# aniketntnu/WordDiffusion

Hardware: AMD Instinct MI355X
Metric: denoised 64x256 word images/sec (1000-step DDPM), whole job (higher is better)
Workload: dtype bf16x3; 1 GPU; BASELINE configs[1]: batch 64 per GPU of 64x256 crops = [64,4,8,32] latents, 1000-step DDPM (999 executed steps), base unet.py UNetModel (320 ch, mult (1,1), 4 heads, 339 writers), random-init synthetic weights; variant=base, batch_per_gpu=64, noise_steps=1000, executed_steps_per_image=999, precision=split-bf16 MFMA x3, fp32 accumulate (<=1e-4 of the fp32 reference), output_finite=True

## Files before the change

### include/wdiff_hip.h

```cpp
#ifndef WDIFF_HIP_H
#define WDIFF_HIP_H

#include <stdint.h>

#ifdef __cplusplus
extern "C" {
#endif

#define WD_OK 0
#define WD_EINVAL (-1)
#define WD_ELAUNCH (-2)
#define WD_ESTATE (-3)

#define WD_ACT_NONE 0
#define WD_ACT_SILU 1
#define WD_ACT_GEGLU 2

typedef uint16_t wd_bf16;

#define WD_MAX_KSPLIT 64

typedef struct wd_src {
    const wd_bf16* hi;
    const wd_bf16* lo;
    const int32_t* gather;
    int32_t ld;
    int32_t c;
    int32_t ntaps;
    int32_t hw_src;
} wd_src;

typedef struct wd_gemm_args {
    wd_src src[2];
    int32_t nsrc;
    int32_t npass;
    const wd_bf16* w_hi;
    const wd_bf16* w_lo;
    int32_t m, n, ktot;
    int32_t hw_out;
    const float* bias;
    const float* rowvec;
    int32_t rowvec_ld;
    const float* resid;
    int32_t resid_ld;
    const int64_t* resid_rows;
    int32_t act;
    float* out_f32;
    int32_t out_ld;
    wd_bf16* out_hi;
    wd_bf16* out_lo;
    int32_t out_pl_ld;
    int32_t tile;
    int32_t w_layout;
    int32_t slab_rows;
    int32_t ksplit;
    float* ws;
    int64_t ws_floats;
    double* stat_part;
    int32_t stat_cpg;
    int32_t dbg;
    int32_t* tickets;
    int32_t ntickets;
    const float* gn_gamma;
    const float* gn_beta;
    float gn_eps;
    int32_t gn_silu;
    int32_t gn_cpg;
    const float* a32;
    int32_t a32_ld;
    const double* a32_part;
    int32_t a32_nchunk;
    int32_t a32_pcpg;
    int32_t a32_cpg;
    const float* a32_gamma;
    const float* a32_beta;
    float a32_eps;
    int32_t a32_silu;
    const float* ln_gamma;
    const float* ln_beta;
    float ln_eps;
    int32_t w_ngroups;
    int64_t w_group_stride;
} wd_gemm_args;

int wd_gemm(const wd_gemm_args* args, void* stream);

int wd_gemm_check(const wd_gemm_args* args, wd_gemm_args* out);
const char* wd_gemm_check_kernel(const wd_gemm_args* args);

int wd_gemm_pack_w(const wd_bf16* hi, const wd_bf16* lo, int n, int ktot, wd_bf16* out_hi, wd_bf16* out_lo, void* stream);

typedef struct wd_ff_args {
    const wd_bf16* x_hi;
    const wd_bf16* x_lo;
    int32_t x_ld;
    int32_t m, c, inner;
    const wd_bf16* w1_hi;
    const wd_bf16* w1_lo;
    const float* b1;
    const wd_bf16* w2_hi;
    const wd_bf16* w2_lo;
    const float* b2;
    const float* resid;
    int32_t resid_ld;
    float* out_f32;
    int32_t out_ld;
    wd_bf16* out_hi;
    wd_bf16* out_lo;
    int32_t out_pl_ld;
    const wd_bf16* w3_hi;
    const wd_bf16* w3_lo;
    const float* b3;
    const float* resid3;
    int32_t resid3_ld;
    double* stat_part;
    int32_t stat_cpg;
    int32_t hw_out;
    int32_t npass;
    const float* x_in;
    int32_t x_in_ld;
    int32_t hw;
    const double* gn_part;
    int32_t gn_nchunk, gn_pcpg, gn_cpg;
    float gn_eps;
    const float* gn_gamma;
    const float* gn_beta;
    const wd_bf16* pi_hi;
    const wd_bf16* pi_lo;
    const float* pi_b;
    const float* ln2_gamma;
    const float* ln2_beta;
    const wd_bf16* mq_a;
    const wd_bf16* mot_a;
    const float* xb_a;
    const wd_bf16* mq_b;
    const wd_bf16* mot_b;
    const float* xb_b;
    const float* ln3_gamma;
    const float* ln3_beta;
    float ln_eps;
    int32_t heads, L;
    float* tok2;
} wd_ff_args;
int wd_ff_fused(const wd_ff_args* args, void* stream);
int wd_ff_supported(int c, int inner);
int wd_ff_args_bytes(void);

int wd_gemm_auto_ksplit(int m, int n, int ktot, int64_t ws_floats);
int wd_gemm_args_bytes(void);
int wd_gemm_experimental(void);

int wd_gn_nchunk(int hw);
int wd_gn_stats(const float* x, int ld, int batch, int hw, int c, int cpg, double* part, void* stream);
int wd_gn_fold_chunks(const double* part, int batch, int nchunk, int ngroups, double* out, void* stream);

int wd_gn_apply(const float* x, int ld, int batch, int hw, int c, int cpg, const double* part, int nchunk, int part_cpg,
                const float* gamma, const float* beta, float eps, int silu,
                wd_bf16* out_hi, wd_bf16* out_lo, int out_ld, int c_off,
                wd_bf16* raw_hi, wd_bf16* raw_lo, void* stream);

int wd_gn_apply2(const float* xa, int lda, int ca, const double* part_a, int nchunk_a, int part_cpg_a, int c_off_a,
                 const float* xb, int ldb, int cb, const double* part_b, int nchunk_b, int part_cpg_b, int c_off_b,
                 int batch, int hw, int cpg, const float* gamma, const float* beta, float eps, int silu,
                 wd_bf16* out_hi, wd_bf16* out_lo, int out_ld, wd_bf16* raw_hi, wd_bf16* raw_lo, const int32_t* perm_a, void* stream);

int wd_gn_conv3x3_few_supported(int c, int w, int oc);
int wd_gn_conv3x3_few(const float* x, int ld, int batch, int h, int w, int c, int cpg, const double* part, int nchunk, int part_cpg,
                      const float* gamma, const float* beta, float eps, int silu, const float* weight, const float* bias, int oc,
                      float* out, void* stream);

int wd_layernorm(const float* x, int ld, int rows, int c, const float* gamma, const float* beta, float eps,
                 wd_bf16* out_hi, wd_bf16* out_lo, int out_ld, void* stream);

int wd_split(const float* x, int ld, int rows, int c, int silu, wd_bf16* out_hi, wd_bf16* out_lo, int out_ld,
             void* stream);

int wd_attention(const float* q, int ldq, const float* k, int ldk, const float* v, int ldv,
                 int batch, int heads, int nq, int nk, int d, float scale,
                 float* out_f32, wd_bf16* out_hi, wd_bf16* out_lo, int out_ld, int out_rows, int out_row0,
                 void* stream);

int64_t wd_attention_packed_elems(int batch, int heads, int nk, int d);
int wd_attention_pack_kv(const float* k, int ldk, const float* v, int ldv, int batch, int heads, int nk, int d,
                         wd_bf16* img, void* stream);
int wd_attention_packed(const float* q, int ldq, const wd_bf16* img, int batch, int heads, int nq, int nk, int d,
                        float scale, float* out_f32, wd_bf16* out_hi, wd_bf16* out_lo, int out_ld, int out_rows,
                        int out_row0, void* stream);

int wd_timestep_embedding(const int64_t* t, int batch, const float* freqs, int half,
                          wd_bf16* out_hi, wd_bf16* out_lo, int out_ld, void* stream);

int wd_xattn_supported(int c, int heads, int L);
int wd_xattn_fold(const float* k, int ldk, const float* v, int ldv, int batch, int heads, int L, int d, float scale,
                  const float* wq, const float* wo, int c, float* mq, float* mo, wd_bf16* mq_pl, wd_bf16* mot_pl, void* stream);
int wd_xattn_fused(const float* x, int ld, int batch, int hw, int c, const float* gamma, const float* beta, float eps,
                   const float* mq, const float* mo, int heads, int L, const float* bias, float* out, int out_ld,
                   const float* gamma2, const float* beta2, float eps2, wd_bf16* n_hi, wd_bf16* n_lo, int n_ld,
                   const wd_bf16* mq_pl, const wd_bf16* mot_pl, void* stream);

int wd_emb_combine(const float* time, const float* label, const int64_t* y, int num_classes, int T, int B, int ted,
                   wd_bf16* out_hi, wd_bf16* out_lo, int out_ld, void* stream);
int wd_select_rows(const float* table, const int32_t* t_dev, int batch, int64_t row_floats, int chunk, float* out,
                   void* stream);

int wd_emb_combine_mix(const float* time, const float* label, const int32_t* pairs, const float* mix, int num_classes, int T, int B,
                       int ted, wd_bf16* out_hi, wd_bf16* out_lo, int out_ld, void* stream);
int wd_label_mix(const float* label, const int32_t* pairs, const float* mix, int num_classes, int B, int ted, float* out,
                 void* stream);

int wd_xattn_pair(const float* x, int ld, int batch, int hw, int c, float eps, int heads, int L, const float* gamma_a,
                  const float* beta_a, const wd_bf16* mq_pl_a, const wd_bf16* mot_pl_a, const float* bias_a, const float* gamma_b,
                  const float* beta_b, const wd_bf16* mq_pl_b, const wd_bf16* mot_pl_b, const float* bias_b, float* out, int out_ld,
                  const float* gamma2, const float* beta2, float eps2, wd_bf16* n_hi, wd_bf16* n_lo, int n_ld, void* stream);

int wd_embed_tokens(const void* ids, int ids_are_i64, int rows, int seq_len, const float* table, int vocab, int c,
                    const float* pe, wd_bf16* out_hi, wd_bf16* out_lo, int out_ld, void* stream);

int wd_im2col3x3(const float* x, int batch, int cin, int h, int w, wd_bf16* out_hi, wd_bf16* out_lo, int kpad,
                 void* stream);

int wd_conv3x3_in_supported(int cin, int h, int w, int cout);
int wd_conv3x3_in_nchunk(int hw);
int wd_conv3x3_in(const float* x, int batch, int cin, int h, int w, const float* weight, const float* bias, int cout, float* out,
                  int ld, double* part, int stat_cpg, void* stream);

int wd_nchw_to_tokens(const float* x, int batch, int c, int hw, float* out, int ld, void* stream);
int wd_tokens_to_nchw(const float* x, int ld, int batch, int c, int hw, float* out, void* stream);

int wd_ddpm_step(float* x, const float* eps, int batch, int n_per_sample, const float* ca, const float* cb,
                 const float* cs, const int32_t* t_dev, const float* noise, uint64_t seed, uint64_t sample_offset,
                 void* stream);

int wd_ddpm_step_cfg(float* x, const float* first, const float* second, float scale, float* eps_out, int batch, int n_per_sample,
                     const float* ca, const float* cb, const float* cs, const int32_t* t_dev, const float* noise, uint64_t seed,
                     uint64_t sample_offset, void* stream);

int wd_advance_timestep(int32_t* t_dev, int delta, int64_t* t64, int batch, void* stream);

int wd_ddim_step(float* x, const float* eps, const float* second, float scale, float* eps_out, int batch, int n_per_sample,
                 const float* c1, const float* c2, const float* c3, const float* c4, const float* c5, const int32_t* k_dev,
                 const int32_t* t_dev, const float* noise, uint64_t seed, uint64_t sample_offset, void* stream);

int wd_next_timestep(int32_t* k_dev, const int32_t* tau, int S, int32_t* t_dev, int64_t* t64, int batch, void* stream);

int wd_randn(float* out, int batch, int n_per_sample, uint64_t seed, uint64_t sample_offset, uint32_t stream_id,
             void* stream);

#define WD_VAE_MAX_LATENT 8
#define WD_STREAM_VAE_POSTERIOR 3
#define WD_STREAM_DROPOUT0 0x100
int wd_vae_posterior(const float* moments_tok, int ld, const float* w, const float* bias, int batch, int L, int hw, float* mean,
                     float* logvar, float* sample, float scale, const float* noise, uint64_t seed, uint64_t sample_offset,
                     void* stream);

int wd_posterior_sample(const float* mean, const float* logvar, int batch, int n_per_sample, float* sample, float scale,
                        const float* noise, uint64_t seed, uint64_t sample_offset, void* stream);

int wd_noise_images(const float* x, const float* eps, const int64_t* t, const float* sqrt_ah, const float* sqrt_1m_ah,
                    int batch, int n_per_sample, float* out, void* stream);

int wd_copy2d(void* dst, int64_t dst_pitch, const void* src, int64_t src_pitch, int64_t width_bytes, int64_t rows,
              void* stream);

int wd_ema_update(float* ema, const float* p, int64_t n, double beta, void* stream);

int wd_adamw_table_entry_bytes(void);
int wd_adamw_chunk(void);
int wd_adamw_multi(const void* table, int ntensor, int64_t total_chunks, double lr, double beta1, double beta2, double eps,
                   double weight_decay, int64_t step, int ema_mode, double ema_beta, void* stream);

int wd_repack_entry_bytes(void);
int wd_repack_tile(void);
int wd_repack_vchunk(void);
int wd_repack_multi(const void* table, int nentries, int64_t total_chunks, void* stream);

int wd_mse_loss(const float* pred, const float* target, int64_t n, float* grad, float* loss, double* scratch,
                int scratch_len, void* stream);


int wd_transpose_planes(const void* in_hi, const void* in_lo, int in_is_f32, int ld, int c, const int32_t* gather, int ntaps,
                        int hw_out, int hw_src, int m, int mpad, int tap_minor, wd_bf16* out_hi, wd_bf16* out_lo,
                        void* stream);

typedef struct wd_dw_item {
    const wd_bf16* d_hi;
    const wd_bf16* d_lo;
    const wd_bf16* x_hi;
    const wd_bf16* x_lo;
    float* grad;
    int32_t d_ld, x_ld, grad_ld, accumulate;
} wd_dw_item;
typedef struct wd_dw_args {
    const wd_bf16* d_hi;
    const wd_bf16* d_lo;
    const wd_bf16* x_hi;
    const wd_bf16* x_lo;
    const int32_t* gather;
    float* grad;
    float* ws;
    int64_t ws_floats;
    int32_t d_ld, x_ld, grad_ld;
    int32_t ntaps, hw_out, hw_src;
    int32_t m, n, c;
    int32_t npass;
    int32_t accumulate;
    int32_t nslice;
    int32_t dbg;
    int32_t reserved;
    void* stamps;
    const wd_dw_item* items;
    int32_t nitems;
    int32_t reserved2;
} wd_dw_args;
int wd_dw(const wd_dw_args* a, void* stream);
int wd_dw_group(const wd_dw_args* a, const wd_dw_item* items_host, const wd_dw_item* items_dev, int nitems, void* stream);
int wd_dw_group_slices(int m, int n, int c, int ntaps, int nitems);
int wd_dw_item_bytes(void);
int wd_dw_supported(int m, int n, int c, int ntaps, int hw_out);
int wd_dw_slices(int m, int n, int c, int ntaps);
int wd_dw_args_bytes(void);

int wd_colsum(const float* x, int ld, int rows, int c, int seg, float* out, int out_ld, int accumulate, float scale,
              float* scratch, int64_t scratch_floats, void* stream);

int wd_gn_bwd_nchunk(int hw);
int wd_gn_bwd_stats(const float* x, int ld, const float* dz, int dz_ld, int dz_off, int batch, int hw, int c, int cpg,
                    const double* part, int nchunk_f, int part_cpg, const float* gamma, const float* beta, int c_off, float eps,
                    int silu, float* sums, void* stream);
int wd_gn_bwd_apply(const float* x, int ld, const float* dz, int dz_ld, int dz_off, int batch, int hw, int c, int cpg,
                    const double* part, int nchunk_f, int part_cpg, const float* gamma, const float* beta, int c_off, float eps,
                    int silu, const float* sums, float* dx, int dx_ld, int accumulate, void* stream);

int wd_gn_bwd_fused_supported(int hw, int c, int cpg);
int wd_gn_bwd_fused(const float* x, int ld, const float* dz, int dz_ld, int dz_off, int batch, int hw, int c, int cpg,
                    const double* part, int nchunk_f, int part_cpg, const float* gamma, const float* beta, int c_off, float eps,
                    int silu, float* sums, float* dx, int dx_ld, int accumulate, void* stream);

typedef struct {
    uint64_t seed;
    uint64_t row_base;
    const uint64_t* row_base_dev;
    uint32_t tag, thr;
    float scale;
} wd_dropout;
int wd_gn_apply_dropout(const float* x, int ld, int batch, int hw, int c, int cpg, const double* part, int nchunk, int part_cpg,
                        const float* gamma, const float* beta, float eps, int silu,
                        wd_bf16* out_hi, wd_bf16* out_lo, int out_ld, int c_off,
                        wd_bf16* raw_hi, wd_bf16* raw_lo, const wd_dropout* d, void* stream);
int wd_gn_bwd_stats_dropout(const float* x, int ld, const float* dz, int dz_ld, int dz_off, int batch, int hw, int c, int cpg,
                            const double* part, int nchunk_f, int part_cpg, const float* gamma, const float* beta, int c_off, float eps,
                            int silu, float* sums, const wd_dropout* d, void* stream);
int wd_gn_bwd_apply_dropout(const float* x, int ld, const float* dz, int dz_ld, int dz_off, int batch, int hw, int c, int cpg,
                            const double* part, int nchunk_f, int part_cpg, const float* gamma, const float* beta, int c_off, float eps,
                            int silu, const float* sums, float* dx, int dx_ld, int accumulate, const wd_dropout* d, void* stream);
int wd_gn_bwd_fused_dropout(const float* x, int ld, const float* dz, int dz_ld, int dz_off, int batch, int hw, int c, int cpg,
                            const double* part, int nchunk_f, int part_cpg, const float* gamma, const float* beta, int c_off, float eps,
                            int silu, float* sums, float* dx, int dx_ld, int accumulate, const wd_dropout* d, void* stream);

int wd_layernorm_bwd_nblk(int rows);
int wd_layernorm_bwd(const float* x, int ld, const float* dy, int dy_ld, int rows, int c, const float* gamma, float eps,
                     float* dx, int dx_ld, int accumulate, float* colpart, void* stream);

int wd_attention_bwd_small_nwg(int heads, int nq, int nk, int d);
int wd_attention_bwd_small(const float* q, int ldq, const float* k, int ldk, const float* v, int ldv, const float* dout,
                           int ldo, int batch, int heads, int nq, int nk, int d, float scale, float* dq, int lddq,
                           float* dkv_part, int* nwg_out, void* stream);
// ... 46 lines not shown
```

### worddiffusion_amd/_native.py

```python
from __future__ import annotations

import ctypes as C
import os
import re

_HERE = os.path.dirname(os.path.abspath(__file__))
LIB_PATH = os.environ.get("WDIFF_LIB") or os.path.join(_HERE, "libwdiff_hip.so")
HEADER_PATH = os.path.join(os.path.dirname(_HERE), "include", "wdiff_hip.h")

WD_OK, WD_EINVAL, WD_ELAUNCH, WD_ESTATE = 0, -1, -2, -3
ACT_NONE, ACT_SILU, ACT_GEGLU = 0, 1, 2
VAE_MAX_LATENT, STREAM_VAE_POSTERIOR = 8, 3
NCLASS = 13
CLASS_NAMES = ("gemm", "gn_stats", "gn_apply", "layernorm", "attention", "other", "gemm_other_tiles", "gemm_splitk_reduce",
               "gemm_two_per_cu", "gemm_weights_to_registers", "feed_forward_fused", "weight_gradient", "gemm_small_maps_whole_k")

_vp = C.c_void_p
_i = C.c_int
_f = C.c_float
_u64 = C.c_uint64


class WdSrc(C.Structure):
    _fields_ = [("hi", _vp), ("lo", _vp), ("gather", _vp), ("ld", C.c_int32), ("c", C.c_int32),
                ("ntaps", C.c_int32), ("hw_src", C.c_int32)]


class WdGemmArgs(C.Structure):
    _fields_ = [("src", WdSrc * 2), ("nsrc", C.c_int32), ("npass", C.c_int32), ("w_hi", _vp), ("w_lo", _vp),
                ("m", C.c_int32), ("n", C.c_int32), ("ktot", C.c_int32), ("hw_out", C.c_int32),
                ("bias", _vp), ("rowvec", _vp), ("rowvec_ld", C.c_int32), ("resid", _vp), ("resid_ld", C.c_int32),
                ("resid_rows", _vp), ("act", C.c_int32), ("out_f32", _vp), ("out_ld", C.c_int32),
                ("out_hi", _vp), ("out_lo", _vp), ("out_pl_ld", C.c_int32), ("tile", C.c_int32),
                ("w_layout", C.c_int32), ("slab_rows", C.c_int32), ("ksplit", C.c_int32), ("ws", _vp),
                ("ws_floats", C.c_int64), ("stat_part", _vp), ("stat_cpg", C.c_int32), ("dbg", C.c_int32),
                ("tickets", _vp), ("ntickets", C.c_int32), ("gn_gamma", _vp), ("gn_beta", _vp), ("gn_eps", C.c_float),
                ("gn_silu", C.c_int32), ("gn_cpg", C.c_int32), ("a32", _vp), ("a32_ld", C.c_int32), ("a32_part", _vp),
                ("a32_nchunk", C.c_int32), ("a32_pcpg", C.c_int32), ("a32_cpg", C.c_int32), ("a32_gamma", _vp), ("a32_beta", _vp),
                ("a32_eps", C.c_float), ("a32_silu", C.c_int32), ("ln_gamma", _vp), ("ln_beta", _vp), ("ln_eps", C.c_float),
                ("w_ngroups", C.c_int32), ("w_group_stride", C.c_int64)]


class WdFfArgs(C.Structure):
    _fields_ = [("x_hi", _vp), ("x_lo", _vp), ("x_ld", C.c_int32), ("m", C.c_int32), ("c", C.c_int32), ("inner", C.c_int32),
                ("w1_hi", _vp), ("w1_lo", _vp), ("b1", _vp), ("w2_hi", _vp), ("w2_lo", _vp), ("b2", _vp), ("resid", _vp),
                ("resid_ld", C.c_int32), ("out_f32", _vp), ("out_ld", C.c_int32), ("out_hi", _vp), ("out_lo", _vp),
                ("out_pl_ld", C.c_int32), ("w3_hi", _vp), ("w3_lo", _vp), ("b3", _vp), ("resid3", _vp), ("resid3_ld", C.c_int32),
                ("stat_part", _vp), ("stat_cpg", C.c_int32), ("hw_out", C.c_int32), ("npass", C.c_int32),
                ("x_in", _vp), ("x_in_ld", C.c_int32), ("hw", C.c_int32), ("gn_part", _vp), ("gn_nchunk", C.c_int32),
                ("gn_pcpg", C.c_int32), ("gn_cpg", C.c_int32), ("gn_eps", C.c_float), ("gn_gamma", _vp), ("gn_beta", _vp),
                ("pi_hi", _vp), ("pi_lo", _vp), ("pi_b", _vp), ("ln2_gamma", _vp), ("ln2_beta", _vp), ("mq_a", _vp), ("mot_a", _vp),
                ("xb_a", _vp), ("mq_b", _vp), ("mot_b", _vp), ("xb_b", _vp), ("ln3_gamma", _vp), ("ln3_beta", _vp),
                ("ln_eps", C.c_float), ("heads", C.c_int32), ("L", C.c_int32), ("tok2", _vp)]


class WdDwArgs(C.Structure):
    _fields_ = [("d_hi", _vp), ("d_lo", _vp), ("x_hi", _vp), ("x_lo", _vp), ("gather", _vp), ("grad", _vp), ("ws", _vp),
                ("ws_floats", C.c_int64), ("d_ld", C.c_int32), ("x_ld", C.c_int32), ("grad_ld", C.c_int32), ("ntaps", C.c_int32),
                ("hw_out", C.c_int32), ("hw_src", C.c_int32), ("m", C.c_int32), ("n", C.c_int32), ("c", C.c_int32),
                ("npass", C.c_int32), ("accumulate", C.c_int32), ("nslice", C.c_int32), ("dbg", C.c_int32), ("reserved", C.c_int32),
                ("stamps", _vp), ("items", _vp), ("nitems", C.c_int32), ("reserved2", C.c_int32)]


class WdDwItem(C.Structure):
    _fields_ = [("d_hi", _vp), ("d_lo", _vp), ("x_hi", _vp), ("x_lo", _vp), ("grad", _vp), ("d_ld", C.c_int32), ("x_ld", C.c_int32),
                ("grad_ld", C.c_int32), ("accumulate", C.c_int32)]


_SIGS = {
    "wd_gemm": (_i, [C.POINTER(WdGemmArgs), _vp]),
    "wd_gemm_check": (_i, [C.POINTER(WdGemmArgs), C.POINTER(WdGemmArgs)]),
    "wd_gemm_check_kernel": (C.c_char_p, [C.POINTER(WdGemmArgs)]),
    "wd_dw": (_i, [C.POINTER(WdDwArgs), _vp]),
    "wd_dw_supported": (_i, [_i, _i, _i, _i, _i]),
    "wd_dw_slices": (_i, [_i, _i, _i, _i]),
    "wd_dw_args_bytes": (_i, []),
    "wd_dw_group": (_i, [C.POINTER(WdDwArgs), _vp, _vp, _i, _vp]),
    "wd_dw_group_slices": (_i, [_i, _i, _i, _i, _i]),
    "wd_dw_item_bytes": (_i, []),
    "wd_gemm_auto_ksplit": (_i, [_i, _i, _i, C.c_int64]),
    "wd_gemm_pack_w": (_i, [_vp, _vp, _i, _i, _vp, _vp, _vp]),
    "wd_ff_fused": (_i, [C.POINTER(WdFfArgs), _vp]),
    "wd_ff_supported": (_i, [_i, _i]),
    "wd_ff_args_bytes": (_i, []),
    "wd_gemm_args_bytes": (_i, []),
    "wd_gemm_experimental": (_i, []),
    "wd_gn_nchunk": (_i, [_i]),
    "wd_gn_stats": (_i, [_vp, _i, _i, _i, _i, _i, _vp, _vp]),
    "wd_gn_fold_chunks": (_i, [_vp, _i, _i, _i, _vp, _vp]),
    "wd_gn_conv3x3_few_supported": (_i, [_i, _i, _i]),
    "wd_gn_conv3x3_few": (_i, [_vp, _i, _i, _i, _i, _i, _i, _vp, _i, _i, _vp, _vp, _f, _i, _vp, _vp, _i, _vp, _vp]),
    "wd_gn_apply": (_i, [_vp, _i, _i, _i, _i, _i, _vp, _i, _i, _vp, _vp, _f, _i, _vp, _vp, _i, _i, _vp, _vp, _vp]),
    "wd_gn_apply_dropout": (_i, [_vp, _i, _i, _i, _i, _i, _vp, _i, _i, _vp, _vp, _f, _i, _vp, _vp, _i, _i, _vp, _vp, _vp, _vp]),
    "wd_gn_apply2": (_i, [_vp, _i, _i, _vp, _i, _i, _i, _vp, _i, _i, _vp, _i, _i, _i, _i, _i, _i, _vp, _vp, _f, _i, _vp, _vp, _i, _vp,
                          _vp, _vp, _vp]),
    "wd_layernorm": (_i, [_vp, _i, _i, _i, _vp, _vp, _f, _vp, _vp, _i, _vp]),
    "wd_split": (_i, [_vp, _i, _i, _i, _i, _vp, _vp, _i, _vp]),
    "wd_attention": (_i, [_vp, _i, _vp, _i, _vp, _i, _i, _i, _i, _i, _i, _f, _vp, _vp, _vp, _i, _i, _i, _vp]),
    "wd_attention_packed_elems": (C.c_int64, [_i, _i, _i, _i]),
    "wd_attention_pack_kv": (_i, [_vp, _i, _vp, _i, _i, _i, _i, _i, _vp, _vp]),
    "wd_attention_packed": (_i, [_vp, _i, _vp, _i, _i, _i, _i, _i, _f, _vp, _vp, _vp, _i, _i, _i, _vp]),
    "wd_timestep_embedding": (_i, [_vp, _i, _vp, _i, _vp, _vp, _i, _vp]),
    "wd_embed_tokens": (_i, [_vp, _i, _i, _i, _vp, _i, _i, _vp, _vp, _vp, _i, _vp]),
    "wd_im2col3x3": (_i, [_vp, _i, _i, _i, _i, _vp, _vp, _i, _vp]),
    "wd_conv3x3_in_supported": (_i, [_i, _i, _i, _i]),
    "wd_conv3x3_in_nchunk": (_i, [_i]),
    "wd_conv3x3_in": (_i, [_vp, _i, _i, _i, _i, _vp, _vp, _i, _vp, _i, _vp, _i, _vp]),
    "wd_nchw_to_tokens": (_i, [_vp, _i, _i, _i, _vp, _i, _vp]),
    "wd_tokens_to_nchw": (_i, [_vp, _i, _i, _i, _i, _vp, _vp]),
    "wd_ddpm_step": (_i, [_vp, _vp, _i, _i, _vp, _vp, _vp, _vp, _vp, _u64, _u64, _vp]),
    "wd_advance_timestep": (_i, [_vp, _i, _vp, _i, _vp]),
    "wd_randn": (_i, [_vp, _i, _i, _u64, _u64, C.c_uint32, _vp]),
    "wd_vae_posterior": (_i, [_vp, _i, _vp, _vp, _i, _i, _i, _vp, _vp, _vp, _f, _vp, _u64, _u64, _vp]),
    "wd_posterior_sample": (_i, [_vp, _vp, _i, _i, _vp, _f, _vp, _u64, _u64, _vp]),
    "wd_noise_images": (_i, [_vp, _vp, _vp, _vp, _vp, _i, _i, _vp, _vp]),
    "wd_copy2d": (_i, [_vp, C.c_int64, _vp, C.c_int64, C.c_int64, C.c_int64, _vp]),
    "wd_ema_update": (_i, [_vp, _vp, C.c_int64, C.c_double, _vp]),
    "wd_adamw_table_entry_bytes": (_i, []),
    "wd_adamw_chunk": (_i, []),
    "wd_adamw_multi": (_i, [_vp, _i, C.c_int64, C.c_double, C.c_double, C.c_double, C.c_double, C.c_double, C.c_int64, _i,
                           C.c_double, _vp]),
    "wd_mse_loss": (_i, [_vp, _vp, C.c_int64, _vp, _vp, _vp, _i, _vp]),
    "wd_transpose_planes": (_i, [_vp, _vp, _i, _i, _i, _vp, _i, _i, _i, _i, _i, _i, _vp, _vp, _vp]),
    "wd_repack_entry_bytes": (_i, []),
    "wd_repack_tile": (_i, []),
    "wd_repack_vchunk": (_i, []),
    "wd_repack_multi": (_i, [_vp, _i, C.c_int64, _vp]),
    "wd_attention_bwd_scratch_floats": (C.c_int64, [_i, _i, _i, _i]),
    "wd_attention_bwd": (_i, [_vp, _i, _vp, _i, _vp, _i, _vp, _i, _i, _i, _i, _i, _i, _f, _vp, _i, _vp, _i, _vp, _i, _vp, C.c_int64, _vp]),
    "wd_xattn_supported": (_i, [_i, _i, _i]),
    "wd_xattn_fold": (_i, [_vp, _i, _vp, _i, _i, _i, _i, _i, _f, _vp, _vp, _i, _vp, _vp, _vp, _vp, _vp]),
    "wd_xattn_fused": (_i, [_vp, _i, _i, _i, _i, _vp, _vp, _f, _vp, _vp, _i, _i, _vp, _vp, _i, _vp, _vp, _f, _vp, _vp, _i, _vp, _vp, _vp]),
    "wd_dout_prep_rows": (_i, []),
    "wd_dout_prep": (_i, [_vp, _i, _i, _i, _i, _i, _vp, _vp, _vp, _vp, _vp, _vp]),
    "wd_dout_prep_geglu": (_i, [_vp, _i, _vp, _i, _i, _i, _i, _vp, _vp, _vp, _vp, _vp, _vp]),
    "wd_colsum_finish": (_i, [_vp, _i, _i, _i, _vp, _i, _i, _f, _vp]),
    "wd_colsum_entry_bytes": (_i, []),
    "wd_colsum_finish_multi": (_i, [_vp, _i, _i, _vp]),
    "wd_emb_combine": (_i, [_vp, _vp, _vp, _i, _i, _i, _i, _vp, _vp, _i, _vp]),
    "wd_select_rows": (_i, [_vp, _vp, _i, C.c_int64, _i, _vp, _vp]),
    "wd_emb_combine_mix": (_i, [_vp, _vp, _vp, _vp, _i, _i, _i, _i, _vp, _vp, _i, _vp]),
    "wd_label_mix": (_i, [_vp, _vp, _vp, _i, _i, _i, _vp, _vp]),
    "wd_ddpm_step_cfg": (_i, [_vp, _vp, _vp, _f, _vp, _i, _i, _vp, _vp, _vp, _vp, _vp, _u64, _u64, _vp]),
    "wd_ddim_step": (_i, [_vp, _vp, _vp, _f, _vp, _i, _i, _vp, _vp, _vp, _vp, _vp, _vp, _vp, _vp, _u64, _u64, _vp]),
    "wd_next_timestep": (_i, [_vp, _vp, _i, _vp, _vp, _i, _vp]),
    "wd_xattn_pair": (_i, [_vp, _i, _i, _i, _i, _f, _i, _i, _vp, _vp, _vp, _vp, _vp, _vp, _vp, _vp, _vp, _vp, _vp, _i, _vp, _vp, _f,
                           _vp, _vp, _i, _vp]),
    "wd_add": (_i, [_vp, _vp, C.c_int64, _vp]),
    "wd_permute_dw": (_i, [_vp, _i, _i, _i, _i, _vp, _vp]),
    "wd_colsum": (_i, [_vp, _i, _i, _i, _i, _vp, _i, _i, _f, _vp, C.c_int64, _vp]),
    "wd_gn_bwd_nchunk": (_i, [_i]),
    "wd_gn_bwd_stats": (_i, [_vp, _i, _vp, _i, _i, _i, _i, _i, _i, _vp, _i, _i, _vp, _vp, _i, _f, _i, _vp, _vp]),
    "wd_gn_bwd_apply": (_i, [_vp, _i, _vp, _i, _i, _i, _i, _i, _i, _vp, _i, _i, _vp, _vp, _i, _f, _i, _vp, _vp, _i, _i, _vp]),
    "wd_gn_bwd_fused_supported": (_i, [_i, _i, _i]),
    "wd_gn_bwd_fused": (_i, [_vp, _i, _vp, _i, _i, _i, _i, _i, _i, _vp, _i, _i, _vp, _vp, _i, _f, _i, _vp, _vp, _i, _i, _vp]),
    "wd_gn_bwd_stats_dropout": (_i, [_vp, _i, _vp, _i, _i, _i, _i, _i, _i, _vp, _i, _i, _vp, _vp, _i, _f, _i, _vp, _vp, _vp]),
    "wd_gn_bwd_apply_dropout": (_i, [_vp, _i, _vp, _i, _i, _i, _i, _i, _i, _vp, _i, _i, _vp, _vp, _i, _f, _i, _vp, _vp, _i, _i, _vp, _vp]),
    "wd_gn_bwd_fused_dropout": (_i, [_vp, _i, _vp, _i, _i, _i, _i, _i, _i, _vp, _i, _i, _vp, _vp, _i, _f, _i, _vp, _vp, _i, _i, _vp, _vp]),
    "wd_layernorm_bwd_nblk": (_i, [_i]),
    "wd_layernorm_bwd": (_i, [_vp, _i, _vp, _i, _i, _i, _vp, _f, _vp, _i, _i, _vp, _vp]),
    "wd_attention_bwd_small_nwg": (_i, [_i, _i, _i, _i]),
    "wd_attention_bwd_small": (_i, [_vp, _i, _vp, _i, _vp, _i, _vp, _i, _i, _i, _i, _i, _i, _f, _vp, _i, _vp,
                                   C.POINTER(_i), _vp]),
    "wd_geglu_fwd": (_i, [_vp, _i, C.c_int64, _i, _vp, _vp, _i, _vp]),
    "wd_geglu_bwd": (_i, [_vp, _i, _vp, _i, C.c_int64, _i, _vp, _i, _vp]),
    "wd_silu_bwd": (_i, [_vp, _vp, C.c_int64, _vp, _vp]),
    "wd_pool2x2_sum": (_i, [_vp, _i, _i, _i, _i, _vp, _vp]),
    "wd_embedding_bwd": (_i, [_vp, _i, _i, _vp, _i, _i, _i, _vp, _i, _vp]),
    "wd_graph_begin": (_i, [_vp]),
    "wd_graph_end": (_i, [_vp, C.POINTER(_vp)]),
    "wd_graph_launch": (_i, [_vp, _vp]),
    "wd_graph_destroy": (_i, [_vp]),
    "wd_prof_enable": (_i, [_i]),
    "wd_prof_collect": (_i, [C.POINTER(C.c_double), C.POINTER(C.c_int64), C.POINTER(C.c_double)]),
    "wd_prof_collect_flops": (_i, [C.POINTER(C.c_double), C.POINTER(C.c_int64), C.POINTER(C.c_double)]),
    "wd_version": (C.c_char_p, []),
    "wd_device_info": (_i, [C.POINTER(_i), C.POINTER(_i), C.c_char_p, _i]),
}


def header_symbols() -> list:
    txt = open(HEADER_PATH).read()
    txt = re.sub(r"/\*.*?\*/", "", txt, flags=re.S)
    return sorted(set(re.findall(r"\b(wd_[a-z0-9_]+)\s*\(", txt)))


class NativeError(RuntimeError):
    pass


_lib = None


def lib() -> C.CDLL:
    global _lib
    if _lib is not None:
        return _lib
    if not os.path.exists(LIB_PATH):
        raise NativeError(f"{LIB_PATH} is missing: build it with `python -m worddiffusion_amd.build` "
                          "(hipcc --offload-arch=gfx950); worddiffusion_amd has no CPU/eager fallback")
    l = C.CDLL(LIB_PATH)
    for name, (res, args) in _SIGS.items():
        fn = getattr(l, name)
        fn.restype = res
        fn.argtypes = args
    if l.wd_gemm_args_bytes() != C.sizeof(WdGemmArgs):
        raise NativeError(f"{LIB_PATH}: wd_gemm_args is {l.wd_gemm_args_bytes()} bytes in the library, {C.sizeof(WdGemmArgs)} in "
                          "worddiffusion_amd/_native.py - rebuild with `python -m worddiffusion_amd.build`")
    if l.wd_ff_args_bytes() != C.sizeof(WdFfArgs):
        raise NativeError(f"{LIB_PATH}: wd_ff_args is {l.wd_ff_args_bytes()} bytes in the library, {C.sizeof(WdFfArgs)} in "
                          "worddiffusion_amd/_native.py - rebuild with `python -m worddiffusion_amd.build`")
    if l.wd_dw_item_bytes() != C.sizeof(WdDwItem):
        raise NativeError(f"{LIB_PATH}: wd_dw_item is {l.wd_dw_item_bytes()} bytes in the library, {C.sizeof(WdDwItem)} in "
                          "worddiffusion_amd/_native.py - rebuild with `python -m worddiffusion_amd.build`")
    if l.wd_dw_args_bytes() != C.sizeof(WdDwArgs):
        raise NativeError(f"{LIB_PATH}: wd_dw_args is {l.wd_dw_args_bytes()} bytes in the library, {C.sizeof(WdDwArgs)} in "
                          "worddiffusion_amd/_native.py - rebuild with `python -m worddiffusion_amd.build`")
    _lib = l
    return l


_ERR = {WD_EINVAL: "invalid argument", WD_ELAUNCH: "HIP launch/runtime error", WD_ESTATE: "bad call order"}


def check(rc: int, what: str) -> None:
    if rc != WD_OK:
        raise NativeError(f"{what} failed: {_ERR.get(rc, rc)}")
```

### worddiffusion_amd/csrc/wd_ff.hip

```cpp
#include "wd_gemm_epi.h"

namespace {

constexpr int FNT = 512;
constexpr int FBM = 64;
constexpr int FC = 320;
constexpr int FCH = 128;
constexpr int FRING = 6;
constexpr int F_MAX_INNER = 2048;
constexpr int FGRP = 30;
constexpr uint32_t F_OOB = 0x80000000u;

typedef __attribute__((ext_vector_type(4))) unsigned f_u32x4;

__device__ __forceinline__ int f_lds_off(int row, int ch) { return row * 128 + ((ch ^ ((row >> 1) & 7)) << 4); }

template <int NPASS, bool PROJ, bool FRONT>
__global__ void __launch_bounds__(FNT, 1) wd_ff_kernel(const wd_ff_args a) {
#if defined(__HIP_DEVICE_COMPILE__)
    static_assert(!FRONT || (NPASS == 3 && PROJ), "the transformer front needs split-bf16 operands and the proj_out tail");
    constexpr int NPL = (NPASS == 1) ? 1 : 2;
    constexpr int SLAB = 2 * FBM * 128;
    constexpr int A_BYTES = 5 * SLAB;
    constexpr int H_BYTES = 2 * SLAB;
    extern __shared__ __attribute__((aligned(16))) char smem[];
    char* s_a = smem;
    char* s_h = smem + A_BYTES;
    float* s_b1 = reinterpret_cast<float*>(smem + A_BYTES + 2 * H_BYTES);

    const int m0 = blockIdx.x * FBM;
    const int tid = threadIdx.x;
    const int lane = tid & 63;
    const int wave = __builtin_amdgcn_readfirstlane(tid >> 6);
    const int kh = wave >> 2, cg = wave & 3;
    const int l15 = lane & 15, lq = lane >> 4;
    const int nchunk = a.inner / FCH;

    auto make_srd = [](const wd_bf16* p) {
        return __builtin_amdgcn_make_buffer_rsrc(const_cast<wd_bf16*>(p), 0, 0x7FFFFFF0, 0x00020000);
    };
    const __amdgpu_buffer_rsrc_t srd1_hi = make_srd(a.w1_hi), srd1_lo = make_srd(a.w1_lo ? a.w1_lo : a.w1_hi);
    const __amdgpu_buffer_rsrc_t srd2_hi = make_srd(a.w2_hi), srd2_lo = make_srd(a.w2_lo ? a.w2_lo : a.w2_hi);
    const __amdgpu_buffer_rsrc_t srd3_hi = make_srd(PROJ ? a.w3_hi : a.w2_hi), srd3_lo = make_srd(PROJ ? (a.w3_lo ? a.w3_lo : a.w3_hi) : a.w2_hi);
    const uint32_t lane16 = lane * 16;
    const int nct1 = (2 * a.inner) >> 4;

    bf16x8 ring[FRING][NPL];
    auto issue = [&](const int slot, const int g, const int j) {
        const bool live = j < nchunk;
        const uint32_t vo = live ? lane16 : F_OOB;
        if (PROJ && g < FRING) {
            const uint32_t so3 = (uint32_t)(((2 * (g / 5) + kh) * (FC / 16) + 5 * cg + g % 5) * 1024);
            const uint32_t so1 = (uint32_t)(((g >> 1) * nct1 + 2 * (j * 8 + wave) + (g & 1)) * 1024);
            const uint32_t so = live ? so1 : so3;
#pragma unroll
            for (int p = 0; p < NPL; ++p) {
                const __amdgpu_buffer_rsrc_t srd = live ? (p ? srd1_lo : srd1_hi) : (p ? srd3_lo : srd3_hi);
                ring[slot][p] = __builtin_bit_cast(bf16x8, __builtin_amdgcn_raw_buffer_load_b128(srd, lane16, so, 0));
            }
        } else if (g < 20) {
            const uint32_t so = (uint32_t)(((g >> 1) * nct1 + 2 * (j * 8 + wave) + (g & 1)) * 1024);
#pragma unroll
            for (int p = 0; p < NPL; ++p)
                ring[slot][p] = __builtin_bit_cast(bf16x8, __builtin_amdgcn_raw_buffer_load_b128(p ? srd1_lo : srd1_hi, vo, live ? so : 0u, 0));
        } else {
            const int q = (g - 20) / 5, t = (g - 20) % 5;
            const uint32_t so = (uint32_t)(((4 * j + 2 * kh + q) * (FC / 16) + 5 * cg + t) * 1024);
#pragma unroll
            for (int p = 0; p < NPL; ++p)
                ring[slot][p] = __builtin_bit_cast(bf16x8, __builtin_amdgcn_raw_buffer_load_b128(p ? srd2_lo : srd2_hi, vo, live ? so : 0u, 0));
        }
    };
    f32x4 acc2[4][5];
    bf16x8 xa[4][NPL];
    auto read_frags = [&](const char* slab_base, const int half) {
        const int ch = half * 4 + lq;
#pragma unroll
        for (int i = 0; i < 4; ++i) {
            const int ao = f_lds_off(i * 16 + l15, ch);
#pragma unroll
            for (int p = 0; p < NPL; ++p) xa[i][p] = *reinterpret_cast<const bf16x8*>(slab_base + p * (FBM * 128) + ao);
        }
    };
    auto mfma12 = [&](f32x4 (&acc)[4], const bf16x8 (&w)[NPL]) {
#pragma unroll
        for (int i = 0; i < 4; ++i) {
            if (NPL == 2) {
                acc[i] = __builtin_amdgcn_mfma_f32_16x16x32_bf16(xa[i][NPL - 1], w[0], acc[i], 0, 0, 0);
                acc[i] = __builtin_amdgcn_mfma_f32_16x16x32_bf16(xa[i][0], w[NPL - 1], acc[i], 0, 0, 0);
            }
            acc[i] = __builtin_amdgcn_mfma_f32_16x16x32_bf16(xa[i][0], w[0], acc[i], 0, 0, 0);
        }
    };
    constexpr int LDE = FC + 4;
    float* ep = reinterpret_cast<float*>(smem);
    auto ksum_to_image = [&]() {
        for (int hh = 0; hh < 2; ++hh) {
            if (kh == hh) {
#pragma unroll
                for (int i = 0; i < 4; ++i)
#pragma unroll
                    for (int t = 0; t < 5; ++t)
#pragma unroll
                        for (int r = 0; r < 4; ++r) {
                            float* pe = ep + (i * 16 + 4 * lq + r) * LDE + cg * 80 + t * 16 + l15;
                            *pe = (hh == 0) ? acc2[i][t][r] : *pe + acc2[i][t][r];
                        }
            }
            __syncthreads();
        }
    };

    if constexpr (FRONT) {
        constexpr int SP = 65, PP = 72, KS32 = FC / 32;
        const int b = m0 / a.hw;
        const int HJ = a.heads * a.L;
        char* fr = s_h + 4096;
        float* s_aff = reinterpret_cast<float*>(fr);
        float* sS = reinterpret_cast<float*>(fr);
        wd_bf16* sP = reinterpret_cast<wd_bf16*>(fr + FBM * SP * 4);
        float* s_vec = reinterpret_cast<float*>(s_h + 40960);
        const float* s_pib = s_vec;
        const float* s_ln2g = s_vec + FC, * s_ln2b = s_vec + 2 * FC, * s_ln3g = s_vec + 3 * FC, * s_ln3b = s_vec + 4 * FC;
        const float* s_xba = s_vec + 5 * FC, * s_xbb = s_vec + 6 * FC;
        const int arow = tid >> 3, ach = tid & 7;
        float4 xv[5][2];
        {
            const float* xrow = a.x_in + (long)(m0 + arow) * a.x_in_ld + ach * 8;
#pragma unroll
            for (int sl = 0; sl < 5; ++sl) {
                xv[sl][0] = *reinterpret_cast<const float4*>(xrow + sl * 64);
                xv[sl][1] = *reinterpret_cast<const float4*>(xrow + sl * 64 + 4);
            }
        }
        const __amdgpu_buffer_rsrc_t srdp_hi = make_srd(a.pi_hi), srdp_lo = make_srd(a.pi_lo);
        auto issue_pi = [&](const int slot, const int g) {
            const uint32_t so = (uint32_t)(((2 * (g / 5) + kh) * (FC / 16) + 5 * cg + g % 5) * 1024);
#pragma unroll
            for (int p = 0; p < NPL; ++p)
                ring[slot][p] = __builtin_bit_cast(bf16x8, __builtin_amdgcn_raw_buffer_load_b128(p ? srdp_lo : srdp_hi, lane16, so, 0));
        };
#pragma unroll
        for (int g = 0; g < FRING; ++g) issue_pi(g, g);
        const int sv = wave < 7 ? wave : 6;
        const float* vsrc = sv == 0 ? a.pi_b : sv == 1 ? a.ln2_gamma : sv == 2 ? a.ln2_beta : sv == 3 ? a.ln3_gamma : sv == 4 ? a.ln3_beta
                            : sv == 5 ? a.xb_a : a.xb_b;
        const float4 vst0 = *reinterpret_cast<const float4*>(vsrc + lane * 4);
        const float4 vst1 = *reinterpret_cast<const float4*>(vsrc + (64 + l15) * 4);
        constexpr int NB1 = 2 * F_MAX_INNER / FNT;
        float b1v[NB1];
        {
            const __amdgpu_buffer_rsrc_t sb1 = __builtin_amdgcn_make_buffer_rsrc(const_cast<float*>(a.b1), 0, a.b1 ? 2 * a.inner * 4 : 0, 0x00020000);
#pragma unroll
            for (int k = 0; k < NB1; ++k)
                b1v[k] = __builtin_bit_cast(float, __builtin_amdgcn_raw_buffer_load_b32(sb1, (uint32_t)(tid + k * FNT) * 4u, 0, 0));
        }
        __builtin_amdgcn_sched_barrier(0);
        for (int e = tid; e < FBM * PP; e += FNT) reinterpret_cast<uint32_t*>(sP)[e] = 0u;
        {
            const int ngp = FC / a.gn_pcpg, ratio = a.gn_cpg / a.gn_pcpg;
            for (int c = tid; c < FC; c += FNT) {
                const int g = c / a.gn_cpg;
                const float gam = a.gn_gamma[c], bet = a.gn_beta[c];
                double su = 0.0, sq = 0.0;
                const int nterm = ratio * a.gn_nchunk;
                int k = 0, ck = 0;
                for (int t0 = 0; t0 < nterm; t0 += 8) {
                    const int k0 = k, ck0 = ck;
                    double2 pv[8];
#pragma unroll
                    for (int u = 0; u < 8; ++u) {
                        const bool live = t0 + u < nterm;
                        const int kk = live ? k : k0, cc = live ? ck : ck0;
                        pv[u] = *reinterpret_cast<const double2*>(a.gn_part + (((long)b * a.gn_nchunk + cc) * ngp + g * ratio + kk) * 2);
                        if (++ck == a.gn_nchunk) {
                            ck = 0;
                            ++k;
                        }
                    }
#pragma unroll
                    for (int u = 0; u < 8; ++u)
                        if (t0 + u < nterm) {
                            su += pv[u].x;
                            sq += pv[u].y;
                        }
                }
                const double n = (double)a.hw * a.gn_cpg;
                const double mu = su / n;
                double var = sq / n - mu * mu;
                if (var < 0.0) var = 0.0;
                const float rstd = (float)(1.0 / sqrt(var + (double)a.gn_eps));
                const float sc = rstd * gam;
                s_aff[2 * c] = sc;
                s_aff[2 * c + 1] = bet - (float)mu * sc;
            }
        }
        __builtin_amdgcn_sched_barrier(0);
        if (wave < 7) {
            *reinterpret_cast<float4*>(s_vec + sv * FC + lane * 4) = vst0;
            *reinterpret_cast<float4*>(s_vec + sv * FC + (64 + l15) * 4) = vst1;
        }
#pragma unroll
        for (int k = 0; k < NB1; ++k)
            if (tid + k * FNT < 2 * a.inner) s_b1[tid + k * FNT] = b1v[k];
        __syncthreads();
#pragma unroll
        for (int sl = 0; sl < 5; ++sl) {
            const float4* tab = reinterpret_cast<const float4*>(s_aff + 2 * (sl * 64 + ach * 8));
            const float4 t0 = tab[0], t1 = tab[1], t2 = tab[2], t3 = tab[3];
            const float4 x0 = xv[sl][0], x1 = xv[sl][1];
            float4 y0, y1;
            y0.x = x0.x * t0.x + t0.y; y0.y = x0.y * t0.z + t0.w; y0.z = x0.z * t1.x + t1.y; y0.w = x0.w * t1.z + t1.w;
            y1.x = x1.x * t2.x + t2.y; y1.y = x1.y * t2.z + t2.w; y1.z = x1.z * t3.x + t3.y; y1.w = x1.w * t3.z + t3.w;
            uint2 h0, l0, h1, l1;
            wd_split4(y0, h0, l0);
            wd_split4(y1, h1, l1);
            char* dst = s_a + sl * SLAB + f_lds_off(arow, ach);
            *reinterpret_cast<f_u32x4*>(dst) = f_u32x4{h0.x, h0.y, h1.x, h1.y};
            *reinterpret_cast<f_u32x4*>(dst + FBM * 128) = f_u32x4{l0.x, l0.y, l1.x, l1.y};
        }
        __syncthreads();
#pragma unroll
        for (int i = 0; i < 4; ++i)
#pragma unroll
            for (int t = 0; t < 5; ++t)
#pragma unroll
                for (int r = 0; r < 4; ++r) acc2[i][t][r] = 0.0f;
#pragma unroll
        for (int g = 0; g < 25; ++g) {
            const int q = g / 5, t = g % 5;
            if (t == 0) read_frags(s_a + q * SLAB, kh);
            {
                f32x4 col[4] = {acc2[0][t], acc2[1][t], acc2[2][t], acc2[3][t]};
                mfma12(col, ring[g % FRING]);
#pragma unroll
                for (int i = 0; i < 4; ++i) acc2[i][t] = col[i];
            }
            if (g + FRING < 25) issue_pi(g % FRING, g + FRING);
            __builtin_amdgcn_sched_barrier(0);
        }
        __syncthreads();
        ksum_to_image();
        float4 xr[2][5];
#pragma unroll
        for (int pp = 0; pp < 2; ++pp)
#pragma unroll
            for (int i = 0; i < 5; ++i) {
                const int n = (l15 + 16 * i) * 4, row = wave * 8 + pp * 4 + lq;
                const float4 v = *reinterpret_cast<const float4*>(ep + row * LDE + n);
                const float4 bx = *reinterpret_cast<const float4*>(s_pib + n);
                xr[pp][i] = make_float4(v.x + bx.x, v.y + bx.y, v.z + bx.z, v.w + bx.w);
            }
        __syncthreads();
        auto ln_rows = [&](const float* gamma, const float* beta) {
#pragma unroll
            for (int pp = 0; pp < 2; ++pp) {
                const int row = wave * 8 + pp * 4 + lq;
                float s = 0.f;
#pragma unroll
                for (int i = 0; i < 5; ++i) s += (xr[pp][i].x + xr[pp][i].y) + (xr[pp][i].z + xr[pp][i].w);
                const float mean = wd_row16_sum(s) / (float)FC;
                float q = 0.f;
#pragma unroll
                for (int i = 0; i < 5; ++i) {
                    const float a0 = xr[pp][i].x - mean, a1 = xr[pp][i].y - mean, a2 = xr[pp][i].z - mean, a3 = xr[pp][i].w - mean;
                    q += (a0 * a0 + a1 * a1) + (a2 * a2 + a3 * a3);
                }
                const float rstd = 1.0f / sqrtf(wd_row16_sum(q) / (float)FC + a.ln_eps);
#pragma unroll
                for (int i = 0; i < 5; ++i) {
                    const int n = (l15 + 16 * i) * 4;
                    const float4 ga = *reinterpret_cast<const float4*>(gamma + n);
                    const float4 be = *reinterpret_cast<const float4*>(beta + n);
                    const float4 x = xr[pp][i];
                    float4 o;
                    o.x = (x.x - mean) * rstd * ga.x + be.x; o.y = (x.y - mean) * rstd * ga.y + be.y;
                    o.z = (x.z - mean) * rstd * ga.z + be.z; o.w = (x.w - mean) * rstd * ga.w + be.w;
                    uint2 hi, lo;
                    wd_split4(o, hi, lo);
                    char* d = s_a + (n >> 6) * SLAB + f_lds_off(row, (n & 63) >> 3) + (n & 7) * 2;
                    *reinterpret_cast<uint2*>(d) = hi;
                    *reinterpret_cast<uint2*>(d + FBM * 128) = lo;
                }
            }
        };
        const int ht = wave & 3, rp = wave >> 2;
        const long pq = 64L * FC;
        bf16x8 bh[KS32], bl[KS32];
        auto issue_mq = [&](const wd_bf16* mq) {
            const __amdgpu_buffer_rsrc_t rq = __builtin_amdgcn_make_buffer_rsrc(const_cast<wd_bf16*>(mq + (long)b * 2 * pq), 0,
                                                                                (int)(2 * pq * 2), 0x00020000);
            const uint32_t vo = ht * 16 + l15 < HJ ? lane16 : F_OOB;
#pragma unroll
            for (int ks = 0; ks < KS32; ++ks) {
                bh[ks] = __builtin_bit_cast(bf16x8, __builtin_amdgcn_raw_buffer_load_b128(rq, vo, (uint32_t)((ht * KS32 + ks) << 10), 0));
                bl[ks] = __builtin_bit_cast(bf16x8, __builtin_amdgcn_raw_buffer_load_b128(rq, vo, (uint32_t)(((ht * KS32 + ks) << 10) + pq * 2), 0));
            }
            __builtin_amdgcn_sched_barrier(0);
        };
        issue_mq(a.mq_a);
#pragma unroll
        for (int ps = 0; ps < 2; ++ps) {
            const wd_bf16* mot = ps == 0 ? a.mot_a : a.mot_b;
            const float* xb = ps == 0 ? s_xba : s_xbb;
            ln_rows(s_ln2g, s_ln2b);
            __syncthreads();
            if (ht * 16 < HJ) {
                f32x4 a_lh[2], a_hl[2], a_hh[2];
#pragma unroll
                for (int ri = 0; ri < 2; ++ri)
#pragma unroll
                    for (int r = 0; r < 4; ++r) a_lh[ri][r] = a_hl[ri][r] = a_hh[ri][r] = 0.f;
#pragma unroll
                for (int ks = 0; ks < KS32; ++ks)
#pragma unroll
                    for (int ri = 0; ri < 2; ++ri) {
                        const char* ap = s_a + (ks >> 1) * SLAB + f_lds_off((2 * rp + ri) * 16 + l15, (ks & 1) * 4 + lq);
                        const bf16x8 ah = *reinterpret_cast<const bf16x8*>(ap);
                        const bf16x8 al = *reinterpret_cast<const bf16x8*>(ap + FBM * 128);
                        a_lh[ri] = __builtin_amdgcn_mfma_f32_16x16x32_bf16(al, bh[ks], a_lh[ri], 0, 0, 0);
                        a_hl[ri] = __builtin_amdgcn_mfma_f32_16x16x32_bf16(ah, bl[ks], a_hl[ri], 0, 0, 0);
                        a_hh[ri] = __builtin_amdgcn_mfma_f32_16x16x32_bf16(ah, bh[ks], a_hh[ri], 0, 0, 0);
                    }
#pragma unroll
                for (int ri = 0; ri < 2; ++ri)
#pragma unroll
                    for (int r = 0; r < 4; ++r)
                        sS[((2 * rp + ri) * 16 + 4 * lq + r) * SP + ht * 16 + l15] = (a_lh[ri][r] + a_hl[ri][r]) + a_hh[ri][r];
            }
            __builtin_amdgcn_sched_barrier(0);
            bf16x8 mh[2][5], ml[2][5];
            {
                const __amdgpu_buffer_rsrc_t rm = __builtin_amdgcn_make_buffer_rsrc(const_cast<wd_bf16*>(mot + (long)b * 2 * pq), 0,
                                                                                    (int)(2 * pq * 2), 0x00020000);
#pragma unroll
                for (int ks = 0; ks < 2; ++ks) {
                    const uint32_t vo = ks * 32 + lq * 8 < HJ ? lane16 : F_OOB;
#pragma unroll
                    for (int t = 0; t < 5; ++t) {
                        const uint32_t so = (uint32_t)((((5 * cg + t) * 2 + ks) << 10));
                        mh[ks][t] = __builtin_bit_cast(bf16x8, __builtin_amdgcn_raw_buffer_load_b128(rm, vo, so, 0));
                        ml[ks][t] = __builtin_bit_cast(bf16x8, __builtin_amdgcn_raw_buffer_load_b128(rm, vo, so + (uint32_t)(pq * 2), 0));
                    }
                }
            }
            __syncthreads();
            for (int idx = tid; idx < FBM * a.heads; idx += FNT) {
                const int t = idx / a.heads, h = idx - t * a.heads;
                const float* pr = sS + t * SP + h * a.L;
                wd_bf16* ph = sP + t * PP + h * a.L;
                float ex[10];
#pragma unroll
                for (int j = 0; j < 10; ++j) ex[j] = pr[j < a.L ? j : a.L - 1];
                float mx = -3.4e38f;
#pragma unroll
                for (int j = 0; j < 10; ++j) mx = fmaxf(mx, ex[j]);
                for (int j = 10; j < a.L; ++j) mx = fmaxf(mx, pr[j]);
                float sum = 0.f;
#pragma unroll
                for (int j = 0; j < 10; ++j) {
                    ex[j] = __expf(ex[j] - mx);
                    sum += j < a.L ? ex[j] : 0.f;
                }
                for (int j = 10; j < a.L; ++j) sum += __expf(pr[j] - mx);
                const float inv = __fdividef(1.f, sum);
#pragma unroll
                for (int j = 0; j < 10; ++j)
                    if (j < a.L) {
                        uint32_t hi, lo;
                        wd_split1(ex[j] * inv, hi, lo);
                        ph[j] = (wd_bf16)hi;
                        ph[FBM * PP + j] = (wd_bf16)lo;
                    }
                for (int j = 10; j < a.L; ++j) {
                    uint32_t hi, lo;
                    wd_split1(__expf(pr[j] - mx) * inv, hi, lo);
                    ph[j] = (wd_bf16)hi;
                    ph[FBM * PP + j] = (wd_bf16)lo;
                }
            }
            __syncthreads();
            {
                f32x4 o[2][5];
#pragma unroll
                for (int ri = 0; ri < 2; ++ri)
#pragma unroll
                    for (int t = 0; t < 5; ++t)
#pragma unroll
                        for (int r = 0; r < 4; ++r) o[ri][t][r] = 0.f;
#pragma unroll
                for (int ks = 0; ks < 2; ++ks)
#pragma unroll
                    for (int ri = 0; ri < 2; ++ri) {
                        const wd_bf16* ap = sP + ((2 * rp + ri) * 16 + l15) * PP + lq * 8 + ks * 32;
                        const bf16x8 ah = *reinterpret_cast<const bf16x8*>(ap);
                        const bf16x8 al = *reinterpret_cast<const bf16x8*>(ap + FBM * PP);
#pragma unroll
                        for (int t = 0; t < 5; ++t) o[ri][t] = __builtin_amdgcn_mfma_f32_16x16x32_bf16(al, mh[ks][t], o[ri][t], 0, 0, 0);
#pragma unroll
                        for (int t = 0; t < 5; ++t) o[ri][t] = __builtin_amdgcn_mfma_f32_16x16x32_bf16(ah, ml[ks][t], o[ri][t], 0, 0, 0);
#pragma unroll
                        for (int t = 0; t < 5; ++t) o[ri][t] = __builtin_amdgcn_mfma_f32_16x16x32_bf16(ah, mh[ks][t], o[ri][t], 0, 0, 0);
                    }
#pragma unroll
                for (int ri = 0; ri < 2; ++ri)
#pragma unroll
                    for (int t = 0; t < 5; ++t)
#pragma unroll
                        for (int r = 0; r < 4; ++r) ep[((2 * rp + ri) * 16 + 4 * lq + r) * LDE + (5 * cg + t) * 16 + l15] = o[ri][t][r];
            }
            if (ps == 0) {
                issue_mq(a.mq_b);
            } else {
#pragma unroll
                for (int g = 0; g < FRING; ++g) issue(g, g, 0);
                __builtin_amdgcn_sched_barrier(0);
            }
            __syncthreads();
#pragma unroll
            for (int pp = 0; pp < 2; ++pp)
#pragma unroll
                for (int i = 0; i < 5; ++i) {
                    const int n = (l15 + 16 * i) * 4, row = wave * 8 + pp * 4 + lq;
                    const float4 bi = *reinterpret_cast<const float4*>(xb + n);
                    const float4 at = *reinterpret_cast<const float4*>(ep + row * LDE + n);
                    const float4 x = xr[pp][i];
                    xr[pp][i] = make_float4(at.x + bi.x + x.x, at.y + bi.y + x.y, at.z + bi.z + x.z, at.w + bi.w + x.w);
                }
            __syncthreads();
        }
#pragma unroll
        for (int pp = 0; pp < 2; ++pp)
#pragma unroll
            for (int i = 0; i < 5; ++i)
                *reinterpret_cast<float4*>(a.tok2 + (long)(m0 + wave * 8 + pp * 4 + lq) * FC + (l15 + 16 * i) * 4) = xr[pp][i];
        ln_rows(s_ln3g, s_ln3b);
    } else {
#pragma unroll
    for (int g = 0; g < FRING; ++g) issue(g, g, 0);

    {
        const __amdgpu_buffer_rsrc_t sx_hi = make_srd(a.x_hi), sx_lo = make_srd(a.x_lo ? a.x_lo : a.x_hi);
        const int arow = tid >> 3, ach = tid & 7;
        const uint32_t vo = (m0 + arow < a.m) ? (uint32_t)(m0 + arow) * (uint32_t)(a.x_ld * 2) + (uint32_t)(ach * 16) : F_OOB;
        f_u32x4 v[5][NPL];
#pragma unroll
        for (int sl = 0; sl < 5; ++sl)
#pragma unroll
            for (int p = 0; p < NPL; ++p) v[sl][p] = __builtin_amdgcn_raw_buffer_load_b128(p ? sx_lo : sx_hi, vo, sl * 128, 0);
        const int dst = f_lds_off(arow, ach);
#pragma unroll
        for (int sl = 0; sl < 5; ++sl)
#pragma unroll
            for (int p = 0; p < NPL; ++p) *reinterpret_cast<f_u32x4*>(s_a + sl * SLAB + p * (FBM * 128) + dst) = v[sl][p];
        for (int i = tid; i < 2 * a.inner; i += FNT) s_b1[i] = a.b1 ? a.b1[i] : 0.0f;
    }
    }
    __syncthreads();

#pragma unroll
    for (int i = 0; i < 4; ++i)
#pragma unroll
        for (int t = 0; t < 5; ++t)
#pragma unroll
            for (int r = 0; r < 4; ++r) acc2[i][t][r] = 0.0f;

    for (int j = 0; j < nchunk; ++j) {
        char* hbuf = s_h + (j & 1) * H_BYTES;
        f32x4 ax[4], ag[4];
#pragma unroll
        for (int i = 0; i < 4; ++i)
#pragma unroll
            for (int r = 0; r < 4; ++r) {
                ax[i][r] = 0.0f;
                ag[i][r] = 0.0f;
            }
#pragma unroll
        for (int g = 0; g < 20; ++g) {
            if ((g & 1) == 0) read_frags(s_a + (g >> 2) * SLAB, (g >> 1) & 1);
            if (g & 1) mfma12(ag, ring[g % FRING]);
            else mfma12(ax, ring[g % FRING]);
            if (g + FRING < FGRP) issue(g % FRING, g + FRING, j);
            else issue(g % FRING, g + FRING - FGRP, j + 1);
            __builtin_amdgcn_sched_barrier(0);
        }
        {
            const int hcol = (j * 8 + wave) * 32 + l15;
            const float bx = s_b1[hcol], bg = s_b1[hcol + 16];
            const int slab = wave >> 2, ch = (wave & 3) * 2 + (l15 >> 3), e = (l15 & 7) * 2;
#pragma unroll
            for (int i = 0; i < 4; ++i)
#pragma unroll
                for (int r = 0; r < 4; ++r) {
                    const float h = (ax[i][r] + bx) * wd_gelu_erf(ag[i][r] + bg);
                    uint32_t hb, lb;
                    wd_split1(h, hb, lb);
                    char* p = hbuf + slab * SLAB + f_lds_off(i * 16 + lq * 4 + r, ch) + e;
                    *reinterpret_cast<unsigned short*>(p) = (unsigned short)hb;
                    if (NPL == 2) *reinterpret_cast<unsigned short*>(p + FBM * 128) = (unsigned short)lb;
                }
        }
        __syncthreads();
#pragma unroll
        for (int g = 20; g < FGRP; ++g) {
            const int q = (g - 20) / 5, t = (g - 20) % 5;
            if (t == 0) read_frags(hbuf + kh * SLAB, q);
            {
                f32x4 col[4] = {acc2[0][t], acc2[1][t], acc2[2][t], acc2[3][t]};
                mfma12(col, ring[g % FRING]);
#pragma unroll
                for (int i = 0; i < 4; ++i) acc2[i][t] = col[i];
            }
            if (g + FRING < FGRP) issue(g % FRING, g + FRING, j);
            else issue(g % FRING, g + FRING - FGRP, j + 1);
            __builtin_amdgcn_sched_barrier(0);
        }
    }

    __syncthreads();
    ksum_to_image();
    wd_gemm_args e = {};
    e.m = a.m;
    e.n = FC;
    e.hw_out = a.hw_out > 0 ? a.hw_out : 1;
    e.act = WD_ACT_NONE;
    e.out_f32 = a.out_f32;
    e.out_ld = a.out_ld;
    e.out_hi = a.out_hi;
    e.out_lo = a.out_lo;
    e.out_pl_ld = a.out_pl_ld;
    e.ksplit = 1;
    e.stat_part = a.stat_part;
    e.stat_cpg = a.stat_cpg;
    if constexpr (!PROJ) {
        e.bias = a.b2;
        e.resid = a.resid;
        e.resid_ld = a.resid_ld;
        wd_epilogue_from_image<FBM, FC, FNT>(e, ep, m0, 0, tid);
    } else {
        constexpr int ROWB = LDE * 4;
        const float* resid = FRONT ? a.tok2 : a.resid;
        const int resid_ld = FRONT ? FC : a.resid_ld;
        if (FRONT) asm volatile("s_waitcnt vmcnt(0)" ::: "memory");
        {
            float4 v[10];
#pragma unroll
            for (int it = 0; it < 10; ++it) {
                const int idx = it * 64 + lane, row = wave * 8 + idx / 80, c = (idx % 80) * 4;
                const int m = m0 + row;
                float4 x = *reinterpret_cast<const float4*>(ep + row * LDE + c);
                if (a.b2) {
                    const float4 q = *reinterpret_cast<const float4*>(a.b2 + c);
                    x.x += q.x; x.y += q.y; x.z += q.z; x.w += q.w;
                }
                if (resid && m < a.m) {
                    const float4 q = *reinterpret_cast<const float4*>(resid + (long)m * resid_ld + c);
                    x.x += q.x; x.y += q.y; x.z += q.z; x.w += q.w;
                }
                v[it] = x;
            }
            asm volatile("s_waitcnt lgkmcnt(0)" ::: "memory");
            __builtin_amdgcn_sched_barrier(0);
#pragma unroll
            for (int it = 0; it < 10; ++it) {
                const int idx = it * 64 + lane, row = wave * 8 + idx / 80, c = (idx % 80) * 4;
                uint2 hh, ll;
                wd_split4(v[it], hh, ll);
                char* rowp = reinterpret_cast<char*>(ep) + row * ROWB;
                *reinterpret_cast<uint2*>(rowp + c * 2) = hh;
                if (NPL == 2) *reinterpret_cast<uint2*>(rowp + 640 + c * 2) = ll;
            }
        }
        __syncthreads();
#pragma unroll
        for (int i = 0; i < 4; ++i)
#pragma unroll
            for (int t = 0; t < 5; ++t)
#pragma unroll
                for (int r = 0; r < 4; ++r) acc2[i][t][r] = 0.0f;
#pragma unroll
        for (int g = 0; g < 25; ++g) {
            const int q = g / 5, t = g % 5;
            if (t == 0) {
                const int ks = 2 * q + kh;
#pragma unroll
                for (int i = 0; i < 4; ++i) {
                    const char* rp = reinterpret_cast<const char*>(ep) + (i * 16 + l15) * ROWB + (ks * 4 + lq) * 16;
#pragma unroll
                    for (int p = 0; p < NPL; ++p) xa[i][p] = *reinterpret_cast<const bf16x8*>(rp + p * 640);
                }
            }
            {
                f32x4 col[4] = {acc2[0][t], acc2[1][t], acc2[2][t], acc2[3][t]};
                mfma12(col, ring[g % FRING]);
#pragma unroll
                for (int i = 0; i < 4; ++i) acc2[i][t] = col[i];
            }
            if (g + FRING < 25) {
                const int g2 = g + FRING;
                const uint32_t so3 = (uint32_t)(((2 * (g2 / 5) + kh) * (FC / 16) + 5 * cg + g2 % 5) * 1024);
#pragma unroll
                for (int p = 0; p < NPL; ++p)
                    ring[g % FRING][p] = __builtin_bit_cast(bf16x8, __builtin_amdgcn_raw_buffer_load_b128(p ? srd3_lo : srd3_hi, lane16, so3, 0));
            }
            __builtin_amdgcn_sched_barrier(0);
        }
        __syncthreads();
        ksum_to_image();
        e.bias = a.b3;
        e.resid = a.resid3;
        e.resid_ld = a.resid3_ld;
        wd_epilogue_from_image<FBM, FC, FNT>(e, ep, m0, 0, tid);
    }
#endif
}

template <int NPASS, bool PROJ, bool FRONT = false>
int launch_ff(const wd_ff_args& a, hipStream_t st) {
    constexpr int max_smem = 5 * 2 * FBM * 128 + 2 * 2 * 2 * FBM * 128 + 2 * F_MAX_INNER * 4;
    constexpr int red_smem = FBM * (FC + 4) * 4 + WD_STAT_SCRATCH;
    static_assert(max_smem <= 160 * 1024 && red_smem <= max_smem, "LDS budget");
    const int loop_smem = max_smem - 2 * (F_MAX_INNER - a.inner) * 4;
    const int smem = loop_smem > red_smem ? loop_smem : red_smem;
    static bool attr_done = false;
    if (!attr_done) {
        if (hipFuncSetAttribute(reinterpret_cast<const void*>(&wd_ff_kernel<NPASS, PROJ, FRONT>), hipFuncAttributeMaxDynamicSharedMemorySize,
                                max_smem) != hipSuccess)
            return WD_ELAUNCH;
        attr_done = true;
    }
    const int nb = (a.m + FBM - 1) / FBM;
    const double fl = 2.0 * (double)a.m * (3.0 * (double)a.inner * FC + (PROJ ? (double)FC * FC : 0.0) +
                                           (FRONT ? (double)FC * FC + 4.0 * a.heads * a.L * FC : 0.0));
    WdLaunchScope scope(WD_CLS_FF, st, fl);
    hipLaunchKernelGGL((wd_ff_kernel<NPASS, PROJ, FRONT>), dim3(nb), dim3(FNT), smem, st, a);
    return wd_check_launch();
}

}

extern "C" int wd_ff_args_bytes(void) { return (int)sizeof(wd_ff_args); }

extern "C" int wd_ff_supported(int c, int inner) { return (c == FC && inner > 0 && inner % FCH == 0 && inner <= F_MAX_INNER) ? 1 : 0; }

extern "C" int wd_ff_fused(const wd_ff_args* pa, void* stream) {
    if (!pa) return WD_EINVAL;
    const wd_ff_args& a = *pa;
    if (!wd_ff_supported(a.c, a.inner) || a.m <= 0 || (a.npass != 1 && a.npass != 3)) return WD_EINVAL;
    const bool front = a.x_in != nullptr;
    if (!a.w1_hi || !a.w2_hi || (a.npass == 3 && (!a.w1_lo || !a.w2_lo))) return WD_EINVAL;
    if (!front && (!a.x_hi || (a.npass == 3 && !a.x_lo) || a.x_ld % 8 || a.x_ld < a.c)) return WD_EINVAL;
    if (!a.out_f32 && !a.out_hi) return WD_EINVAL;
    if ((a.out_ld | a.resid_ld | a.out_pl_ld) & 3) return WD_EINVAL;
    if (a.resid && a.resid_ld <= 0) return WD_EINVAL;
    if ((long)a.m * a.x_ld * 2 >= 0x7FFFFFF0L || (long)2 * a.inner * a.c * 2 >= 0x7FFFFFF0L) return WD_EINVAL;
    const bool proj = a.w3_hi != nullptr;
    if (proj && ((a.npass == 3 && !a.w3_lo) || (a.resid3 && (a.resid3_ld <= 0 || (a.resid3_ld & 3))))) return WD_EINVAL;
    if (a.stat_part && (a.stat_cpg <= 0 || FC % a.stat_cpg || a.hw_out <= 0 || !(a.hw_out % FBM == 0 || FBM % a.hw_out == 0) ||
                        (FBM > a.hw_out && FBM / a.hw_out > WD_STAT_MAXNS)))
        return WD_EINVAL;
    if (front) {
        if (a.npass != 3 || !proj || a.x_in_ld < a.c || a.x_in_ld % 4 || a.hw <= 0 || a.hw % FBM || a.m % a.hw) return WD_EINVAL;
        if (!a.gn_part || a.gn_nchunk <= 0 || a.gn_pcpg <= 0 || a.gn_cpg <= 0 || a.gn_cpg % a.gn_pcpg || FC % a.gn_cpg ||
            !a.gn_gamma || !a.gn_beta)
            return WD_EINVAL;
        if (!a.pi_hi || !a.pi_lo || !a.pi_b || !a.ln2_gamma || !a.ln2_beta || !a.ln3_gamma || !a.ln3_beta || !a.tok2) return WD_EINVAL;
        if (!a.mq_a || !a.mot_a || !a.xb_a || !a.mq_b || !a.mot_b || !a.xb_b || !wd_xattn_supported(a.c, a.heads, a.L)) return WD_EINVAL;
    }
    hipStream_t st = reinterpret_cast<hipStream_t>(stream);
    if (front) return launch_ff<3, true, true>(a, st);
    if (proj) return a.npass == 3 ? launch_ff<3, true>(a, st) : launch_ff<1, true>(a, st);
    return a.npass == 3 ? launch_ff<3, false>(a, st) : launch_ff<1, false>(a, st);
}
```

### worddiffusion_amd/csrc/wd_pack.hip

```cpp
#include "wd_common.h"

namespace {

struct PackRef {
    const float* src0;
    const float* src1;
    void* dst_hi;
    void* dst_lo;
    int32_t N, C, T, mode;
    int32_t npad, ld, g, ntile_c;
    int64_t chunk0;
    int32_t row_off, col_off;
};

constexpr int PT = 32;
constexpr int VCHUNK = 8192;

__device__ __forceinline__ int geglu_perm(int n, int N, int g) {
    if (g <= 0) return n;
    const int inner = N >> 1;
    const int half = n >= inner;
    const int m = half ? n - inner : n;
    return (m / g) * 2 * g + half * g + (m % g);
}

template <int T>
__device__ __forceinline__ void repack_full_tile(const PackRef& e, float* s, const int n0, const int c0, const int tid) {
    constexpr int ROW = PT * T + 1;
    const int C = e.C, N = e.N;
    for (int idx = tid; idx < PT * PT * T; idx += 256) {
        const int nl = idx / (PT * T), rem = idx - nl * (PT * T);
        const int n = n0 + nl;
        s[nl * ROW + rem] = n < N ? e.src0[((int64_t)n * C + c0) * T + rem] : 0.f;
    }
    __syncthreads();
    uint32_t* dh = reinterpret_cast<uint32_t*>(e.dst_hi);
    uint32_t* dl = reinterpret_cast<uint32_t*>(e.dst_lo);
    const int pr = tid & 15, r0 = tid >> 4;
    if (e.mode == 3) {
        const int nct = e.ld >> 4;
        for (int r = r0; r < PT * T; r += 16) {
            const int nl = r / T, t = r - nl * T;
            const int n = n0 + nl;
            if (n >= N) continue;
            uint32_t h0, l0, h1, l1;
            wd_split1(s[nl * ROW + (2 * pr) * T + t], h0, l0);
            wd_split1(s[nl * ROW + (2 * pr + 1) * T + t], h1, l1);
            const int row = geglu_perm(n, N, e.g) + e.row_off;
            const int k = e.col_off + t * C + c0 + 2 * pr;
            const int64_t o = ((((int64_t)(k >> 5) * nct + (row >> 4)) * 64 + (row & 15) + 16 * ((k >> 3) & 3)) * 8 + (k & 7)) >> 1;
            dh[o] = h0 | (h1 << 16);
            if (dl) dl[o] = l0 | (l1 << 16);
        }
    } else if (e.mode == 0) {
        for (int r = r0; r < PT * T; r += 16) {
            const int nl = r / T, t = r - nl * T;
            const int n = n0 + nl;
            if (n >= N) continue;
            uint32_t h0, l0, h1, l1;
            wd_split1(s[nl * ROW + (2 * pr) * T + t], h0, l0);
            wd_split1(s[nl * ROW + (2 * pr + 1) * T + t], h1, l1);
            const int64_t o = ((int64_t)geglu_perm(n, N, e.g) * e.ld + (int64_t)t * C + c0 + 2 * pr) >> 1;
            dh[o] = h0 | (h1 << 16);
            if (dl) dl[o] = l0 | (l1 << 16);
        }
    } else {
        for (int r = r0; r < PT * T; r += 16) {
            const int cl = r / T, t = r - cl * T;
            uint32_t h0, l0, h1, l1;
            wd_split1(s[(2 * pr) * ROW + cl * T + t], h0, l0);
            wd_split1(s[(2 * pr + 1) * ROW + cl * T + t], h1, l1);
            const int64_t o = ((int64_t)(c0 + cl) * e.ld + (int64_t)t * e.npad + n0 + 2 * pr) >> 1;
            dh[o] = h0 | (h1 << 16);
            if (dl) dl[o] = l0 | (l1 << 16);
        }
    }
}

__global__ void __launch_bounds__(256) repack_multi_kernel(const PackRef* __restrict__ tab, int nentries) {
    __shared__ float s[PT * (PT * 9 + 1)];
    int lo = 0, hi = nentries - 1;
    const int64_t ch = blockIdx.x;
    while (lo < hi) {
        const int mid = (lo + hi + 1) >> 1;
        if (tab[mid].chunk0 <= ch) lo = mid;
        else hi = mid - 1;
    }
    const PackRef e = tab[lo];
    const int64_t lc = ch - e.chunk0;
    const int tid = threadIdx.x;
    if (e.mode == 2) {
        float* dst = reinterpret_cast<float*>(e.dst_hi);
        const int64_t base = lc * VCHUNK, end = base + VCHUNK < e.N ? base + VCHUNK : e.N;
        for (int64_t i = base + tid; i < end; i += 256) {
            float v = e.src0[i];
            if (e.src1) v += e.src1[i];
            dst[geglu_perm((int)i, e.N, e.g)] = v;
        }
        return;
    }
    const int T = e.T, C = e.C, N = e.N;
    const int n0 = (int)(lc / e.ntile_c) * PT, c0 = (int)(lc % e.ntile_c) * PT;
    const int nc = min(PT, C - c0);
    const int row = PT * T + 1;
    if (nc == PT && (T == 9 || T == 1) && (e.mode != 1 || e.npad - n0 >= PT) && (C & 1) == 0 && (e.ld & 1) == 0 &&
        (e.npad & 1) == 0 && ((reinterpret_cast<uintptr_t>(e.dst_hi) | reinterpret_cast<uintptr_t>(e.dst_lo)) & 3) == 0) {
        if (T == 9) repack_full_tile<9>(e, s, n0, c0, tid);
        else repack_full_tile<1>(e, s, n0, c0, tid);
        return;
    }
    if (e.mode == 3) return;
    for (int idx = tid; idx < PT * nc * T; idx += 256) {
        const int nl = idx / (nc * T), rem = idx - nl * (nc * T);
        const int n = n0 + nl;
        s[nl * row + rem] = n < N ? e.src0[((int64_t)n * C + c0) * T + rem] : 0.f;
    }
    __syncthreads();
    wd_bf16* dh = reinterpret_cast<wd_bf16*>(e.dst_hi);
    wd_bf16* dl = reinterpret_cast<wd_bf16*>(e.dst_lo);
    if (e.mode == 0) {
        for (int idx = tid; idx < PT * T * nc; idx += 256) {
            const int cl = idx % nc, t = (idx / nc) % T, nl = idx / (nc * T);
            const int n = n0 + nl;
            if (n >= N) continue;
            uint32_t h, l;
            wd_split1(s[nl * row + cl * T + t], h, l);
            const int64_t o = (int64_t)geglu_perm(n, N, e.g) * e.ld + (int64_t)t * C + c0 + cl;
            dh[o] = (wd_bf16)h;
            if (dl) dl[o] = (wd_bf16)l;
        }
    } else {
        const int nn = min(PT, e.npad - n0);
        for (int idx = tid; idx < nc * T * nn; idx += 256) {
            const int nl = idx % nn, t = (idx / nn) % T, cl = idx / (nn * T);
            uint32_t h, l;
            wd_split1(s[nl * row + cl * T + t], h, l);
            const int64_t o = (int64_t)(c0 + cl) * e.ld + (int64_t)t * e.npad + n0 + nl;
            dh[o] = (wd_bf16)h;
            if (dl) dl[o] = (wd_bf16)l;
        }
    }
}

}

extern "C" int wd_repack_entry_bytes(void) { return (int)sizeof(PackRef); }
extern "C" int wd_repack_tile(void) { return PT; }
extern "C" int wd_repack_vchunk(void) { return VCHUNK; }

extern "C" int wd_repack_multi(const void* table, int nentries, int64_t total_chunks, void* stream) {
    if (!table || nentries <= 0 || total_chunks <= 0 || total_chunks > 0x7fffffffLL) return WD_EINVAL;
    hipStream_t st = reinterpret_cast<hipStream_t>(stream);
    WdLaunchScope scope(WD_CLS_OTHER, st);
    hipLaunchKernelGGL(repack_multi_kernel, dim3((unsigned)total_chunks), dim3(256), 0, st,
                       reinterpret_cast<const PackRef*>(table), nentries);
    return wd_check_launch();
}
```

### worddiffusion_amd/csrc/wd_xattn.hip

```cpp
#include "wd_common.h"
#include <stdlib.h>
#include <type_traits>

namespace {

constexpr int XHJ = 64;

__device__ __forceinline__ long xa_mq_index(int hj, int n, int c) {
    return ((long)((hj >> 4) * (c >> 5) + (n >> 5)) << 9) + ((((n >> 3) & 3) * 16 + (hj & 15)) << 3) + (n & 7);
}
__device__ __forceinline__ long xa_mo16_index(int n, int hj) {
    return ((long)((n >> 4) * 2 + (hj >> 5)) << 9) + ((((hj >> 3) & 3) * 16 + (n & 15)) << 3) + (hj & 7);
}

__global__ void __launch_bounds__(256) xattn_fold_kernel(const float* __restrict__ k, int ldk, const float* __restrict__ v,
                                                         int ldv, int heads, int L, int d, float scale,
                                                         const float* __restrict__ wq, const float* __restrict__ wo, int c,
                                                         float* __restrict__ mq, float* __restrict__ mo,
                                                         wd_bf16* __restrict__ mq_pl, wd_bf16* __restrict__ mot_pl) {
    extern __shared__ float s_kv[];
    const int j = blockIdx.x, h = blockIdx.y, b = blockIdx.z;
    const int inner = heads * d;
    const float* kr = k + ((long)b * L + j) * ldk + h * d;
    const float* vr = v + ((long)b * L + j) * ldv + h * d;
// ... 93 lines not shown
        *reinterpret_cast<float4*>(s_m + r * CP + f * 4) = m4;
    }
    __syncthreads();

    const int tp = tid >> 3, g = tid & 7;
    {
        float acc[2][NH];
#pragma unroll
        for (int i = 0; i < NH; ++i) acc[0][i] = acc[1][i] = 0.f;
        const float* xa = s_x + (2 * tp) * CP;
        const float* xb = xa + CP;
        for (int f = 0; f < ((dbg & 2) ? 1 : C4); ++f) {
            const float4 a = *reinterpret_cast<const float4*>(xa + f * 4), c4 = *reinterpret_cast<const float4*>(xb + f * 4);
#pragma unroll
            for (int i = 0; i < NH; ++i) {
                const float4 m4 = *reinterpret_cast<const float4*>(s_m + (g + 8 * i) * CP + f * 4);
                acc[0][i] += (a.x * m4.x + a.y * m4.y) + (a.z * m4.z + a.w * m4.w);
                acc[1][i] += (c4.x * m4.x + c4.y * m4.y) + (c4.z * m4.z + c4.w * m4.w);
            }
        }
#pragma unroll
        for (int i = 0; i < NH; ++i) {
            s_p[(2 * tp) * (HJP + 1) + g + 8 * i] = acc[0][i];
            s_p[(2 * tp + 1) * (HJP + 1) + g + 8 * i] = acc[1][i];
        }
    }
    __syncthreads();
    for (int idx = tid; idx < XT * heads; idx += 256) {
        const int t = idx / heads, h = idx - t * heads;
        float* pr = s_p + t * (HJP + 1) + h * L;
        float mx = -3.4e38f;
        for (int j = 0; j < L; ++j) mx = fmaxf(mx, pr[j]);
        float sum = 0.f;
        for (int j = 0; j < L; ++j) {
            const float e = expf(pr[j] - mx);
            pr[j] = e;
            sum += e;
        }
        const float inv = 1.f / sum;
        for (int j = 0; j < L; ++j) pr[j] *= inv;
    }
    for (int e = tid; e < HJ * C4; e += 256) {
        const int r = e / C4, f = e - r * C4;
        *reinterpret_cast<float4*>(s_m + r * CP + f * 4) = *reinterpret_cast<const float4*>(mob + (long)r * C + f * 4);
    }
    __syncthreads();

    float4 o[2][NI];
#pragma unroll
    for (int i = 0; i < NI; ++i) o[0][i] = o[1][i] = make_float4(0.f, 0.f, 0.f, 0.f);
    {
        const float* pa = s_p + (2 * tp) * (HJP + 1);
        const float* pb = pa + (HJP + 1);
        for (int hj = 0; hj < ((dbg & 4) ? 1 : HJ); ++hj) {
            const float wa = pa[hj], wb = pb[hj];
            const float* mr = s_m + hj * CP + g * 4;
#pragma unroll
            for (int i = 0; i < NI; ++i) {
                const float4 m4 = *reinterpret_cast<const float4*>(mr + i * 32);
                o[0][i].x += wa * m4.x; o[0][i].y += wa * m4.y; o[0][i].z += wa * m4.z; o[0][i].w += wa * m4.w;
                o[1][i].x += wb * m4.x; o[1][i].y += wb * m4.y; o[1][i].z += wb * m4.z; o[1][i].w += wb * m4.w;
            }
        }
    }
#pragma unroll
    for (int u = 0; u < 2; ++u) {
        const int t = 2 * tp + u;
        const bool ok = t < ntok;
        float s = 0.f;
#pragma unroll
        for (int i = 0; i < NI; ++i) {
            const int n = (g + 8 * i) * 4;
            const float4 bi = *reinterpret_cast<const float4*>(bias + n);
            float4 xr = make_float4(0.f, 0.f, 0.f, 0.f);
            if (ok) xr = *reinterpret_cast<const float4*>(x + (row0 + t) * ld + n);
            o[u][i].x += bi.x + xr.x; o[u][i].y += bi.y + xr.y; o[u][i].z += bi.z + xr.z; o[u][i].w += bi.w + xr.w;
            if (ok) *reinterpret_cast<float4*>(out + (row0 + t) * out_ld + n) = o[u][i];
            s += (o[u][i].x + o[u][i].y) + (o[u][i].z + o[u][i].w);
        }
        if (n_hi) {
            s += __shfl_xor(s, 1, 64); s += __shfl_xor(s, 2, 64); s += __shfl_xor(s, 4, 64);
            const float mean = s / (float)C;
            float q = 0.f;
#pragma unroll
            for (int i = 0; i < NI; ++i) {
                const float a0 = o[u][i].x - mean, a1 = o[u][i].y - mean, a2 = o[u][i].z - mean, a3 = o[u][i].w - mean;
                q += (a0 * a0 + a1 * a1) + (a2 * a2 + a3 * a3);
            }
            q += __shfl_xor(q, 1, 64); q += __shfl_xor(q, 2, 64); q += __shfl_xor(q, 4, 64);
            const float rstd = 1.0f / sqrtf(q / (float)C + eps2);
            if (ok) {
#pragma unroll
                for (int i = 0; i < NI; ++i) {
                    const int n = (g + 8 * i) * 4;
                    const float4 ga = *reinterpret_cast<const float4*>(gamma2 + n);
                    const float4 be = *reinterpret_cast<const float4*>(beta2 + n);
                    float4 y;
                    y.x = (o[u][i].x - mean) * rstd * ga.x + be.x; y.y = (o[u][i].y - mean) * rstd * ga.y + be.y;
                    y.z = (o[u][i].z - mean) * rstd * ga.z + be.z; y.w = (o[u][i].w - mean) * rstd * ga.w + be.w;
                    uint2 hi, lo;
                    wd_split4(y, hi, lo);
                    *reinterpret_cast<uint2*>(n_hi + (row0 + t) * n_ld + n) = hi;
                    if (n_lo) *reinterpret_cast<uint2*>(n_lo + (row0 + t) * n_ld + n) = lo;
                }
            }
        }
    }
}

template <int NI, int NH>
int launch_fused(const float* x, int ld, int batch, int hw, const float* gamma, const float* beta, float eps, const float* mq,
                 const float* mo, int heads, int L, const float* bias, float* out, int out_ld, const float* gamma2,
                 const float* beta2, float eps2, wd_bf16* n_hi, wd_bf16* n_lo, int n_ld, hipStream_t st) {
    constexpr int C = NI * 32, CP = C + 4, HJP = NH * 8;
    constexpr size_t smem = (size_t)(XT * CP + HJP * CP + XT * (HJP + 1)) * sizeof(float);
    static_assert(smem <= 160 * 1024, "tile does not fit LDS");
    static bool attr = false;
    if (!attr) {
        if (hipFuncSetAttribute(reinterpret_cast<const void*>(&xattn_fused_kernel<NI, NH>),
                                hipFuncAttributeMaxDynamicSharedMemorySize, (int)smem) != hipSuccess)
            return WD_ELAUNCH;
        attr = true;
    }
    WdLaunchScope scope(WD_CLS_ATTN, st);
    hipLaunchKernelGGL((xattn_fused_kernel<NI, NH>), dim3((hw + XT - 1) / XT, batch), dim3(256), smem, st, x, ld, hw, gamma, beta,
                       eps, mq, mo, heads, L, bias, out, out_ld, gamma2, beta2, eps2, n_hi, n_lo, n_ld,
                       getenv("WDIFF_XATTN_DBG") ? atoi(getenv("WDIFF_XATTN_DBG")) : 0);
    return wd_check_launch();
}


typedef __attribute__((ext_vector_type(8))) __bf16 xa_bf16x8;

struct XaLayer {
    const float* gamma;
    const float* beta;
    const wd_bf16* mq_pl;
    const wd_bf16* mot_pl;
    const float* bias;
};

typedef __attribute__((ext_vector_type(4))) float xa_f32x4;

typedef __attribute__((ext_vector_type(4))) unsigned xa_u32x4;
__device__ __forceinline__ xa_bf16x8 xa_bload(__amdgpu_buffer_rsrc_t r, unsigned voff, unsigned soff) {
    return __builtin_bit_cast(xa_bf16x8, (xa_u32x4)__builtin_amdgcn_raw_buffer_load_b128(r, voff, soff, 0));
}

template <int NI, int NP, int LL>
__global__ void __launch_bounds__(256, 3) xattn16_kernel(const float* __restrict__ x, int ld, int hw, const XaLayer la,
                                                      const XaLayer lb, float eps, int heads, int L, float* __restrict__ out,
                                                      int out_ld, const float* __restrict__ gamma2,
                                                      const float* __restrict__ beta2, float eps2, wd_bf16* __restrict__ n_hi,
                                                      wd_bf16* __restrict__ n_lo, int n_ld) {
    constexpr int XT = 16, NTH = 256;
    constexpr int C = NI * 32, XP = C + 8, OP = C + 4, SP = 65, PP = 72, NT = NI / 2, KS32 = C / 32;
    static_assert(NI % 2 == 0, "column tiles per wave");
    extern __shared__ __attribute__((aligned(16))) char smem[];
    wd_bf16* sX = reinterpret_cast<wd_bf16*>(smem);
    float* sO = reinterpret_cast<float*>(smem);
    constexpr size_t XBYTES = (size_t)2 * XT * XP * 2 > (size_t)XT * OP * 4 ? (size_t)2 * XT * XP * 2 : (size_t)XT * OP * 4;
    float* sS = reinterpret_cast<float*>(smem + XBYTES);
    wd_bf16* sP = reinterpret_cast<wd_bf16*>(smem + XBYTES + (size_t)XT * SP * 4);
    float* sV = reinterpret_cast<float*>(smem + XBYTES + (size_t)XT * SP * 4 + (size_t)2 * XT * PP * 2);
    const int b = blockIdx.x, t0 = blockIdx.y * XT;
    const int tid = threadIdx.x, lane = tid & 63;
    const int wave = __builtin_amdgcn_readfirstlane(tid >> 6);
    const int HJ = heads * L;
    const long row0 = (long)b * hw + t0;
    const int ntok = min(XT, hw - t0);
    constexpr int FI = NI / 2;
    const int qd = lane >> 4, l15 = lane & 15;
    const int trow = wave * 4 + qd;
    const bool ok = trow < ntok;
    float4 xr[FI];
#pragma unroll
    for (int i = 0; i < FI; ++i) {
        xr[i] = make_float4(0.f, 0.f, 0.f, 0.f);
        if (ok) xr[i] = *reinterpret_cast<const float4*>(x + (row0 + trow) * ld + (l15 + 16 * i) * 4);
    }
    const bool row_live = wave * 16 + l15 < HJ;
    const long pq = (long)XHJ * C;
    xa_bf16x8 bh[KS32], bl[KS32];
    auto request_scores = [&](const XaLayer& ly) {
        const __amdgpu_buffer_rsrc_t rq = __builtin_amdgcn_make_buffer_rsrc(const_cast<wd_bf16*>(ly.mq_pl + (long)b * 2 * pq), 0,
                                                                            (int)(2 * pq * 2), 0x00020000);
        const unsigned vo = row_live ? lane * 16u : 0x80000000u;
#pragma unroll
        for (int ks = 0; ks < KS32; ++ks) {
            bh[ks] = xa_bload(rq, vo, (unsigned)((wave * KS32 + ks) << 10));
            bl[ks] = xa_bload(rq, vo, (unsigned)(((wave * KS32 + ks) << 10) + pq * 2));
        }
    };
    for (int e = tid; e < 2 * XT * PP / 2; e += NTH) reinterpret_cast<uint32_t*>(sP)[e] = 0u;
    for (int e = tid; e < 6 * (C / 4); e += NTH) {
        const int v = e / (C / 4), i = e - v * (C / 4);
        const float* src = v == 0 ? la.bias : v == 1 ? lb.gamma : v == 2 ? lb.beta : v == 3 ? lb.bias : v == 4 ? gamma2 : beta2;
        if (src) reinterpret_cast<float4*>(sV)[e] = reinterpret_cast<const float4*>(src)[i];
    }
#pragma unroll
    for (int ps = 0; ps < NP; ++ps) {
    const XaLayer& ly = ps == 0 ? la : lb;
    const float* gamma = ps == 0 ? la.gamma : sV + C;
    const float* beta = ps == 0 ? la.beta : sV + 2 * C;
    const float* bias = ps == 0 ? sV : sV + 3 * C;
    const bool last = ps == NP - 1;
    {
        float s = 0.f;
#pragma unroll
        for (int i = 0; i < FI; ++i) s += (xr[i].x + xr[i].y) + (xr[i].z + xr[i].w);
        const float mean = wd_row16_sum(s) / (float)C;
        float q = 0.f;
#pragma unroll
        for (int i = 0; i < FI; ++i) {
            const float a0 = xr[i].x - mean, a1 = xr[i].y - mean, a2 = xr[i].z - mean, a3 = xr[i].w - mean;
            q += (a0 * a0 + a1 * a1) + (a2 * a2 + a3 * a3);
        }
        const float rstd = 1.0f / sqrtf(wd_row16_sum(q) / (float)C + eps);
#pragma unroll
        for (int i = 0; i < FI; ++i) {
            const float4 ga = *reinterpret_cast<const float4*>(gamma + (l15 + 16 * i) * 4);
            const float4 be = *reinterpret_cast<const float4*>(beta + (l15 + 16 * i) * 4);
            float4 o;
            o.x = (xr[i].x - mean) * rstd * ga.x + be.x; o.y = (xr[i].y - mean) * rstd * ga.y + be.y;
            o.z = (xr[i].z - mean) * rstd * ga.z + be.z; o.w = (xr[i].w - mean) * rstd * ga.w + be.w;
            uint2 hi, lo;
            wd_split4(o, hi, lo);
            *reinterpret_cast<uint2*>(sX + (long)trow * XP + (l15 + 16 * i) * 4) = hi;
            *reinterpret_cast<uint2*>(sX + (long)(XT + trow) * XP + (l15 + 16 * i) * 4) = lo;
        }
    }
    __builtin_amdgcn_sched_barrier(0);
    request_scores(ly);
    __syncthreads();

    if (wave * 16 < HJ) {
        xa_f32x4 a_lh = {0.f, 0.f, 0.f, 0.f}, a_hl = a_lh, a_hh = a_lh;
        const wd_bf16* ax = sX + (long)l15 * XP + qd * 8;
#pragma unroll
        for (int ks = 0; ks < KS32; ++ks) {
            const xa_bf16x8 ah = *reinterpret_cast<const xa_bf16x8*>(ax + ks * 32);
            const xa_bf16x8 al = *reinterpret_cast<const xa_bf16x8*>(ax + (long)XT * XP + ks * 32);
            a_lh = __builtin_amdgcn_mfma_f32_16x16x32_bf16(al, bh[ks], a_lh, 0, 0, 0);
            a_hl = __builtin_amdgcn_mfma_f32_16x16x32_bf16(ah, bl[ks], a_hl, 0, 0, 0);
            a_hh = __builtin_amdgcn_mfma_f32_16x16x32_bf16(ah, bh[ks], a_hh, 0, 0, 0);
        }
#pragma unroll
        for (int r = 0; r < 4; ++r) sS[(4 * qd + r) * SP + wave * 16 + l15] = (a_lh[r] + a_hl[r]) + a_hh[r];
    }
    __builtin_amdgcn_sched_barrier(0);
    xa_bf16x8 mh[2][NT], ml[2][NT];
    {
        const __amdgpu_buffer_rsrc_t rm = __builtin_amdgcn_make_buffer_rsrc(const_cast<wd_bf16*>(ly.mot_pl + (long)b * 2 * pq), 0,
                                                                            (int)(2 * pq * 2), 0x00020000);
#pragma unroll
        for (int ks = 0; ks < 2; ++ks) {
            const unsigned vo = ks * 32 + qd * 8 < HJ ? lane * 16u : 0x80000000u;
#pragma unroll
            for (int t = 0; t < NT; ++t) {
                mh[ks][t] = xa_bload(rm, vo, (unsigned)((((wave * NT + t) * 2 + ks) << 10)));
                ml[ks][t] = xa_bload(rm, vo, (unsigned)((((wave * NT + t) * 2 + ks) << 10) + pq * 2));
            }
        }
    }
    __syncthreads();
    for (int idx = tid; idx < XT * heads; idx += NTH) {
        const int t = idx / heads, h = idx - t * heads;
        const float* pr = sS + t * SP + h * L;
        wd_bf16* ph = sP + (long)t * PP + h * L;
        if (LL > 0) {
            constexpr int LN_ = LL > 0 ? LL : 1;
            float v[LN_];
#pragma unroll
            for (int j = 0; j < LN_; ++j) v[j] = pr[j];
            float mx = v[0];
#pragma unroll
            for (int j = 1; j < LN_; ++j) mx = fmaxf(mx, v[j]);
            float sum = 0.f;
#pragma unroll
            for (int j = 0; j < LN_; ++j) {
                v[j] = __expf(v[j] - mx);
                sum += v[j];
            }
            const float inv = __fdividef(1.f, sum);
#pragma unroll
            for (int j = 0; j < LN_; ++j) {
                uint32_t hi, lo;
                wd_split1(v[j] * inv, hi, lo);
                ph[j] = (wd_bf16)hi;
                ph[(long)XT * PP + j] = (wd_bf16)lo;
            }
        } else {
            float mx = -3.4e38f;
            for (int j = 0; j < L; ++j) mx = fmaxf(mx, pr[j]);
            float sum = 0.f;
            for (int j = 0; j < L; ++j) sum += __expf(pr[j] - mx);
            const float inv = __fdividef(1.f, sum);
            for (int j = 0; j < L; ++j) {
                uint32_t hi, lo;
                wd_split1(__expf(pr[j] - mx) * inv, hi, lo);
                ph[j] = (wd_bf16)hi;
                ph[(long)XT * PP + j] = (wd_bf16)lo;
            }
        }
    }
    __syncthreads();
    {
        xa_f32x4 o[NT];
#pragma unroll
        for (int t = 0; t < NT; ++t) o[t] = xa_f32x4{0.f, 0.f, 0.f, 0.f};
        const wd_bf16* ap = sP + (long)l15 * PP + qd * 8;
#pragma unroll
        for (int ks = 0; ks < 2; ++ks) {
            const xa_bf16x8 ah = *reinterpret_cast<const xa_bf16x8*>(ap + ks * 32);
            const xa_bf16x8 al = *reinterpret_cast<const xa_bf16x8*>(ap + (long)XT * PP + ks * 32);
#pragma unroll
            for (int t = 0; t < NT; ++t) o[t] = __builtin_amdgcn_mfma_f32_16x16x32_bf16(al, mh[ks][t], o[t], 0, 0, 0);
#pragma unroll
            for (int t = 0; t < NT; ++t) o[t] = __builtin_amdgcn_mfma_f32_16x16x32_bf16(ah, ml[ks][t], o[t], 0, 0, 0);
#pragma unroll
            for (int t = 0; t < NT; ++t) o[t] = __builtin_amdgcn_mfma_f32_16x16x32_bf16(ah, mh[ks][t], o[t], 0, 0, 0);
        }
#pragma unroll
        for (int t = 0; t < NT; ++t)
#pragma unroll
            for (int r = 0; r < 4; ++r) sO[(4 * qd + r) * OP + (wave * NT + t) * 16 + l15] = o[t][r];
    }
    __syncthreads();
    {
        float s = 0.f;
#pragma unroll
        for (int i = 0; i < FI; ++i) {
            const int n = (l15 + 16 * i) * 4;
            const float4 bi = *reinterpret_cast<const float4*>(bias + n);
            const float4 at = *reinterpret_cast<const float4*>(sO + trow * OP + n);
            xr[i] = make_float4(at.x + bi.x + xr[i].x, at.y + bi.y + xr[i].y, at.z + bi.z + xr[i].z, at.w + bi.w + xr[i].w);
            if (ok && last) *reinterpret_cast<float4*>(out + (row0 + trow) * out_ld + n) = xr[i];
            s += (xr[i].x + xr[i].y) + (xr[i].z + xr[i].w);
        }
        if (n_hi && last) {
            const float mean = wd_row16_sum(s) / (float)C;
            float q = 0.f;
#pragma unroll
            for (int i = 0; i < FI; ++i) {
                const float a0 = xr[i].x - mean, a1 = xr[i].y - mean, a2 = xr[i].z - mean, a3 = xr[i].w - mean;
                q += (a0 * a0 + a1 * a1) + (a2 * a2 + a3 * a3);
            }
            const float rstd = 1.0f / sqrtf(wd_row16_sum(q) / (float)C + eps2);
            if (ok) {
#pragma unroll
                for (int i = 0; i < FI; ++i) {
                    const int n = (l15 + 16 * i) * 4;
                    const float4 g2 = *reinterpret_cast<const float4*>(sV + 4 * C + n);
                    const float4 b2 = *reinterpret_cast<const float4*>(sV + 5 * C + n);
                    float4 y;
                    y.x = (xr[i].x - mean) * rstd * g2.x + b2.x; y.y = (xr[i].y - mean) * rstd * g2.y + b2.y;
                    y.z = (xr[i].z - mean) * rstd * g2.z + b2.z; y.w = (xr[i].w - mean) * rstd * g2.w + b2.w;
                    uint2 hi, lo;
                    wd_split4(y, hi, lo);
                    *reinterpret_cast<uint2*>(n_hi + (row0 + trow) * n_ld + n) = hi;
                    if (n_lo) *reinterpret_cast<uint2*>(n_lo + (row0 + trow) * n_ld + n) = lo;
                }
            }
        }
    }
    if (!last) __syncthreads();
    }
}

template <int NI, int NP>
int launch16(const float* x, int ld, int batch, int hw, const XaLayer& la, const XaLayer& lb, float eps, int heads, int L,
             float* out, int out_ld, const float* gamma2, const float* beta2, float eps2, wd_bf16* n_hi, wd_bf16* n_lo, int n_ld,
             hipStream_t st) {
    constexpr int C = NI * 32, XTM = 16;
    constexpr size_t xb = (size_t)2 * XTM * (C + 8) * 2 > (size_t)XTM * (C + 4) * 4 ? (size_t)2 * XTM * (C + 8) * 2 : (size_t)XTM * (C + 4) * 4;
    constexpr size_t smem = xb + (size_t)XTM * 65 * 4 + (size_t)2 * XTM * 72 * 2 + (size_t)6 * C * 4;
    static_assert(smem <= 48 * 1024, "static LDS limit");
    WdLaunchScope scope(WD_CLS_ATTN, st);
    const dim3 grid(batch, (hw + XTM - 1) / XTM);
    if (L == 10)
        hipLaunchKernelGGL((xattn16_kernel<NI, NP, 10>), grid, dim3(256), smem, st, x, ld, hw, la, lb, eps, heads, L, out, out_ld,
                           gamma2, beta2, eps2, n_hi, n_lo, n_ld);
    else
        hipLaunchKernelGGL((xattn16_kernel<NI, NP, 0>), grid, dim3(256), smem, st, x, ld, hw, la, lb, eps, heads, L, out, out_ld,
                           gamma2, beta2, eps2, n_hi, n_lo, n_ld);
    return wd_check_launch();
}

}

extern "C" int wd_xattn_supported(int c, int heads, int L) {
    return (c == 64 || c == 320) && heads > 0 && L > 0 && heads * L <= 40 && c % heads == 0;
}

extern "C" int wd_xattn_fold(const float* k, int ldk, const float* v, int ldv, int batch, int heads, int L, int d, float scale,
                             const float* wq, const float* wo, int c, float* mq, float* mo, wd_bf16* mq_pl, wd_bf16* mot_pl,
                             void* stream) {
    if (!k || !v || !wq || !wo || !mq || !mo || batch <= 0 || heads <= 0 || L <= 0 || d <= 0 || c <= 0) return WD_EINVAL;
    if ((mq_pl != nullptr) != (mot_pl != nullptr) || (mq_pl && heads * L > XHJ)) return WD_EINVAL;
    hipStream_t st = reinterpret_cast<hipStream_t>(stream);
    WdLaunchScope scope(WD_CLS_OTHER, st);
    hipLaunchKernelGGL(xattn_fold_kernel, dim3(L, heads, batch), dim3(256), 2 * d * sizeof(float), st, k, ldk, v, ldv, heads, L, d,
                       scale, wq, wo, c, mq, mo, mq_pl, mot_pl);
    return wd_check_launch();
}

extern "C" int wd_xattn_fused(const float* x, int ld, int batch, int hw, int c, const float* gamma, const float* beta, float eps,
                              const float* mq, const float* mo, int heads, int L, const float* bias, float* out, int out_ld,
                              const float* gamma2, const float* beta2, float eps2, wd_bf16* n_hi, wd_bf16* n_lo, int n_ld,
                              const wd_bf16* mq_pl, const wd_bf16* mot_pl, void* stream) {
    if (!x || !gamma || !beta || !mq || !mo || !bias || !out || batch <= 0 || hw <= 0) return WD_EINVAL;
    if (!wd_xattn_supported(c, heads, L) || ld % 4 || out_ld % 4 || (n_hi && (n_ld % 4 || !gamma2 || !beta2))) return WD_EINVAL;
    hipStream_t st = reinterpret_cast<hipStream_t>(stream);
    if (mq_pl && mot_pl && !getenv("WDIFF_XATTN_VALU")) {
        const XaLayer la = {gamma, beta, mq_pl, mot_pl, bias};
        if (c == 320)
            return launch16<10, 1>(x, ld, batch, hw, la, la, eps, heads, L, out, out_ld, gamma2, beta2, eps2, n_hi, n_lo, n_ld, st);
        return launch16<2, 1>(x, ld, batch, hw, la, la, eps, heads, L, out, out_ld, gamma2, beta2, eps2, n_hi, n_lo, n_ld, st);
    }
    const int nh = (heads * L + 7) / 8;
#define WD_XA(NI_, NH_)                                                                                                     \
    return launch_fused<NI_, NH_>(x, ld, batch, hw, gamma, beta, eps, mq, mo, heads, L, bias, out, out_ld, gamma2, beta2, eps2, \
                                  n_hi, n_lo, n_ld, st)
    if (c == 320) {
        switch (nh) {
            case 1: WD_XA(10, 1);
            case 2: WD_XA(10, 2);
            case 3: WD_XA(10, 3);
            case 4: WD_XA(10, 4);
            case 5: WD_XA(10, 5);
        }
    } else {
        switch (nh) {
            case 1: WD_XA(2, 1);
            case 2: WD_XA(2, 2);
            case 3: WD_XA(2, 3);
            case 4: WD_XA(2, 4);
            case 5: WD_XA(2, 5);
        }
    }
#undef WD_XA
    return WD_EINVAL;
}

extern "C" int wd_xattn_pair(const float* x, int ld, int batch, int hw, int c, float eps, int heads, int L, const float* gamma_a,
                             const float* beta_a, const wd_bf16* mq_pl_a, const wd_bf16* mot_pl_a, const float* bias_a,
                             const float* gamma_b, const float* beta_b, const wd_bf16* mq_pl_b, const wd_bf16* mot_pl_b,
                             const float* bias_b, float* out, int out_ld, const float* gamma2, const float* beta2, float eps2,
                             wd_bf16* n_hi, wd_bf16* n_lo, int n_ld, void* stream) {
    if (!x || !out || !gamma_a || !beta_a || !mq_pl_a || !mot_pl_a || !bias_a || !gamma_b || !beta_b || !mq_pl_b || !mot_pl_b ||
        !bias_b || batch <= 0 || hw <= 0)
        return WD_EINVAL;
    if (!wd_xattn_supported(c, heads, L) || ld % 4 || out_ld % 4 || (n_hi && (n_ld % 4 || !gamma2 || !beta2))) return WD_EINVAL;
    hipStream_t st = reinterpret_cast<hipStream_t>(stream);
    const XaLayer la = {gamma_a, beta_a, mq_pl_a, mot_pl_a, bias_a}, lb = {gamma_b, beta_b, mq_pl_b, mot_pl_b, bias_b};
    if (c == 320)
        return launch16<10, 2>(x, ld, batch, hw, la, lb, eps, heads, L, out, out_ld, gamma2, beta2, eps2, n_hi, n_lo, n_ld, st);
    return launch16<2, 2>(x, ld, batch, hw, la, lb, eps, heads, L, out, out_ld, gamma2, beta2, eps2, n_hi, n_lo, n_ld, st);
}
```

### worddiffusion_amd/engine.py

```python
from __future__ import annotations

import ctypes as C
import math
import os
from typing import Dict, List, Optional, Tuple

import numpy as np
import torch

from . import _native as N
from .layers import (DownsampleParams, ResBlockParams, SpatialTransformerParams, UpsampleParams)


def conv_gather_table(h: int, w: int, mode: str) -> Tuple[np.ndarray, int, int]:
    if mode == "same":
        ho, wo = h, w
    elif mode == "down":
        ho, wo = (h + 2 - 3) // 2 + 1, (w + 2 - 3) // 2 + 1
    elif mode == "up":
        ho, wo = 2 * h, 2 * w
    elif mode == "down_rb":
        ho, wo = (h - 2) // 2 + 1, (w - 2) // 2 + 1
    else:
        raise ValueError(mode)
# ... 114 lines not shown
    def __init__(self, name, planes, rows=0, cols=0, shape=None):
        self.name, self.planes, self.rows, self.cols, self.shape, self.pieces = name, planes, rows, cols, shape, []

    @staticmethod
    def _nct(w):
        return w.shape[0], w.shape[1], (w.shape[2] * w.shape[3] if w.dim() == 4 else 1)

    def fwd(self, w, row_off=0, col_off=0, g=0):
        n, c, t = self._nct(w)
        assert row_off + n <= self.rows and col_off + t * c <= self.cols, self.name
        self.pieces.append((0, w, None, n, c, t, row_off, col_off, 0, g))
        return self

    def bwd(self, w, col_off=0, npad=None):
        n, c, t = self._nct(w)
        npad = n if npad is None else npad
        assert c <= self.rows and col_off + t * npad <= self.cols, self.name
        self.pieces.append((1, w, None, n, c, t, 0, col_off, npad, 0))
        return self

    def vec(self, p, p2=None, off=0, g=0):
        self.pieces.append((2, p, p2, p.numel(), 1, 1, 0, off, 0, g))
        return self

    def host(self) -> torch.Tensor:
        first = self.pieces[0][1]
        out = torch.zeros((self.rows, self.cols) if self.planes else (int(torch.tensor(self.shape).prod()),),
                          dtype=torch.float32, device=first.device)
        for (mode, p, p2, n, c, t, row_off, col_off, npad, g) in self.pieces:
            src = p.detach().float()
            if mode == 2:
                v = src.reshape(-1) + (p2.detach().float().reshape(-1) if p2 is not None else 0)
                out[col_off:col_off + n] = geglu_interleave(v, g) if g else v
                continue
            w3 = src.reshape(n, c, t)
            if mode == 0:
                blk = w3.permute(0, 2, 1).reshape(n, t * c)
                out[row_off:row_off + n, col_off:col_off + t * c] = geglu_interleave(blk, g) if g else blk
            else:
                blk = torch.zeros(c, t, npad, dtype=torch.float32, device=first.device)
                blk[:, :, :n] = w3.permute(1, 2, 0)
                out[:c, col_off:col_off + t * npad] = blk.reshape(c, t * npad)
        return out if self.planes else out.reshape(self.shape)


class RecipeBook(dict):

    def matrix(self, name, rows, cols) -> _Recipe:
        self[name] = _Recipe(name, True, rows, cols)
        return self[name]

    def vector(self, name, p, p2=None, g=0) -> _Recipe:
        self[name] = _Recipe(name, False, shape=tuple(p.shape)).vec(p, p2, 0, g)
        return self[name]

    def vector_cat(self, name, ps) -> _Recipe:
        r = _Recipe(name, False, shape=(sum(p.numel() for p in ps),))
        off = 0
        for p in ps:
            r.vec(p, None, off)
            off += p.numel()
        self[name] = r
        return r

    def linear(self, name, lin):
        self.matrix(name + ".w", lin.weight.shape[0], lin.weight.shape[1]).fwd(lin.weight)
        if lin.bias is not None:
            self.vector(name + ".b", lin.bias)

    @staticmethod
    def frag_ok(r) -> bool:
        return r.planes and r.rows % 16 == 0 and r.cols % 32 == 0 and all(
            mode == 0 and c % 32 == 0 and t in (1, 9) and col_off % 2 == 0 and row_off >= 0
            for (mode, p, p2, n, c, t, row_off, col_off, npad, g) in r.pieces)

    def device_table(self, lib, dst: Dict[str, torch.Tensor], dev, frag: Optional[Dict[str, torch.Tensor]] = None):
        import struct
        assert lib.wd_repack_entry_bytes() == 80
        tile, vchunk = lib.wd_repack_tile(), lib.wd_repack_vchunk()
        recs, c0 = [], 0
        for name, r in self.items():
            d = dst[name]
            for (mode, p, p2, n, c, t, row_off, col_off, npad, g) in r.pieces:
                assert p.is_cuda and p.dtype == torch.float32 and p.is_contiguous(), name
                if mode == 2:
                    hi, lo, ld, ntc = d.data_ptr() + 4 * col_off, 0, 0, 1
                    nch = (n + vchunk - 1) // vchunk
                else:
                    ld = r.cols
                    o = 2 * (row_off * ld + col_off)
                    hi, lo = d[0].data_ptr() + o, d[1].data_ptr() + o
                    ntc = (c + tile - 1) // tile
                    nch = (((npad if mode == 1 else n) + tile - 1) // tile) * ntc
                recs.append(struct.pack("<QQQQiiiiiiiiqii", p.data_ptr(), p2.data_ptr() if p2 is not None else 0, hi, lo, n, c, t,
                                        mode, npad, ld, g, ntc, c0, 0, 0))
                c0 += nch
                if frag is not None and name in frag and self.frag_ok(r):
                    f = frag[name]
                    recs.append(struct.pack("<QQQQiiiiiiiiqii", p.data_ptr(), 0, f[0].data_ptr(), f[1].data_ptr(), n, c, t, 3, 0,
                                            r.rows, g, ntc, c0, row_off, col_off))
                    c0 += nch
        raw = torch.frombuffer(bytearray(b"".join(recs)), dtype=torch.uint8).to(dev)
        return raw, c0, len(recs)


class Act:
    __slots__ = ("t", "c", "h", "w", "stats", "prod", "perm")

    def __init__(self, t, c, h, w, stats=None, prod=None, perm=None):
        self.t, self.c, self.h, self.w = t, c, h, w
        self.perm = perm
        self.stats = stats
        self.prod = prod


class Plan:
    def __init__(self):
        self.cond: List[tuple] = []
        self.step: List[tuple] = []
        self.keep: List[object] = []
        self.out: Optional[torch.Tensor] = None

    @staticmethod
    def _run(ops, stream):
        for fn, args, what in ops:
            rc = fn(*args, stream)
            if rc != 0:
                N.check(rc, what)

    def run_cond(self, stream):
        self._run(self.cond, stream)

    def run_film(self, stream):
        self._run(getattr(self, "film", []), stream)
        self.film_loaded = -1

    @staticmethod
    def film_prepare(t, stream):
        return False

    def run_step(self, stream):
        self._run(self.step, stream)

    def run_step1(self, stream):
        self._run(self.step1, stream)


def _ptr(t: Optional[torch.Tensor], byte_off: int = 0):
    return None if t is None else t.data_ptr() + byte_off


class UNetEngine:

    def __init__(self, model, variant: str):
        self.model = model
        self.variant = variant
        self.lib = N.lib()
        self.npass = 3
        self._sig = None
        self._ps, self._ps_gen = None, -1
        self._pack = None
        self._w: Dict[str, torch.Tensor] = {}
        self._w3: Dict[str, torch.Tensor] = {}
        self._w3_meta: Dict[str, tuple] = {}
        self._wf: Dict[str, torch.Tensor] = {}
        self.use_wdirect = os.environ.get("WDIFF_GEMM_WDIRECT", "1") != "0"
        self.use_up_phases = os.environ.get("WDIFF_UPSAMPLE_PHASES", "1") != "0"
        self._derived: Dict[str, tuple] = {}
        self.use_smallmap = os.environ.get("WDIFF_GEMM_SMALLMAP", "1") != "0"
        self.fuse_ff = os.environ.get("WDIFF_FUSE_FF", "1") != "0"
        self.fuse_proj = os.environ.get("WDIFF_FUSE_PROJ", "1") != "0"
        self.fuse_ln = os.environ.get("WDIFF_FUSE_LN", "1") != "0"
        self.fuse_gn_in = int(os.environ.get("WDIFF_FUSE_GN_IN", "1"))
        self.use_slab = os.environ.get("WDIFF_SLAB", "0") != "0"
        self.fuse_stats = os.environ.get("WDIFF_FUSE_STATS", "1") != "0"
        self.fuse_xattn = os.environ.get("WDIFF_FUSE_XATTN", "1") != "0"
        self.use_conv3 = os.environ.get("WDIFF_CONV3", "0") != "0"
        if (self.use_slab or self.use_conv3) and not self.lib.wd_gemm_experimental():
            raise N.NativeError("WDIFF_SLAB / WDIFF_CONV3 need a library built with WDIFF_EXPERIMENTAL=1 "
                                "(python -m worddiffusion_amd.build --force)")
        self.fuse_xattn_pair = os.environ.get("WDIFF_FUSE_XATTN_PAIR", "1") != "0"
        self.fuse_st = os.environ.get("WDIFF_FUSE_ST", "1") != "0"
        self.fuse_out = os.environ.get("WDIFF_FUSE_OUT", "1") != "0"
        self.fuse_in = os.environ.get("WDIFF_FUSE_IN", "1") != "0"
        self.pack_kv = os.environ.get("WDIFF_PACK_KV", "1") != "0"
        self.fuse_gn2 = os.environ.get("WDIFF_FUSE_GN2", "1") != "0"
        self.fuse_gn = os.environ.get("WDIFF_FUSE_GN", "1") != "0"
        self.fuse_split = os.environ.get("WDIFF_FUSE_SPLIT", "1") != "0"
        self._plans: Dict[tuple, Plan] = {}
        self._tabs: Dict[tuple, torch.Tensor] = {}
        self._tab_np: Dict[int, np.ndarray] = {}
        self._same_w: Dict[int, int] = {}
        self._down_w: Dict[int, int] = {}
        self._ws = None
        self.device = None

    def set_precision(self, mode: str):
        npass = {"bf16x3": 3, "fp32": 3, "bf16": 1}[mode]
        if npass != self.npass:
            self.npass = npass
            self._plans.clear()

    def _recipes(self) -> "RecipeBook":
        m = self.model
        R = RecipeBook()
        film_w = []
        self.film_off = {}
        off = 0
        cin_conv = m.input_blocks[0][0]
        self.kpad_in = ((9 * cin_conv.in_channels + 31) // 32) * 32
        R.matrix("in.w", cin_conv.out_channels, self.kpad_in).fwd(cin_conv.weight)
        R.vector("in.b", cin_conv.bias)
        R.vector("in.w.f32", cin_conv.weight)
        R.linear("te0", m.time_embed[0])
        R.linear("te2", m.time_embed[2])
        if m.num_classes is not None:
            R.vector("label", m.label_emb.weight)
        we = m.word_emb
        cd = we.embedding.weight.shape[1]
        R.vector("we.table", we.embedding.weight)
        qkv = (we.attention.linear_query, we.attention.linear_key, we.attention.linear_value)
        R.matrix("we.qkv.w", 3 * cd, cd)
        R.vector_cat("we.qkv.b", [l.bias for l in qkv])
        for i, l in enumerate(qkv):
            R["we.qkv.w"].fwd(l.weight, row_off=i * cd)
        kv_w = []
        self.kv_off = {}
        kvo = 0
        for name, mod in self._walk():
            if isinstance(mod, ResBlockParams):
                R.vector(name + ".gn1.g", mod.in_layers[0].weight)
                R.vector(name + ".gn1.b", mod.in_layers[0].bias)
                R.matrix(name + ".c1.w", mod.cout, 9 * mod.cin).fwd(mod.in_layers[2].weight)
                R.vector(name + ".c1.b", mod.in_layers[2].bias)
                R.vector(name + ".gn2.g", mod.out_layers[0].weight)
                R.vector(name + ".gn2.b", mod.out_layers[0].bias)
                if mod.cin != mod.cout:
                    R.matrix(name + ".c2.w", mod.cout, 9 * mod.cout + mod.cin).fwd(mod.out_layers[3].weight) \
                        .fwd(mod.skip_connection.weight, col_off=9 * mod.cout)
                    R.vector(name + ".c2.b", mod.out_layers[3].bias, mod.skip_connection.bias)
                else:
                    R.matrix(name + ".c2.w", mod.cout, 9 * mod.cout).fwd(mod.out_layers[3].weight)
                    R.vector(name + ".c2.b", mod.out_layers[3].bias)
                film_w.append(mod.emb_layers[1])
                self.film_off[name] = off
                off += mod.cout
            elif isinstance(mod, (DownsampleParams, UpsampleParams)):
                conv = mod.op if isinstance(mod, DownsampleParams) else mod.conv
                R.matrix(name + ".w", mod.cout, 9 * mod.cin).fwd(conv.weight)
                R.vector(name + ".b", conv.bias)
                if isinstance(mod, UpsampleParams) and self._up_phases_ok(mod):
                    key = name + ".wph"
                    if key not in self._derived or self._derived[key][0].device != conv.weight.device:
                        self._derived[key] = (torch.empty((4, 4, mod.cout, mod.cin), dtype=torch.float32, device=conv.weight.device),
                                              (lambda cv=conv: upsample_phase_weights(cv.weight)))
                    wph = self._derived[key][0]
                    for ph in range(4):
                        r = R.matrix(f"{name}.wph{ph}", mod.cout, 4 * mod.cin)
                        for t in range(4):
                            r.fwd(wph[ph, t], col_off=t * mod.cin)
            elif isinstance(mod, SpatialTransformerParams):
                inner = mod.heads * mod.d_head
                R.vector(name + ".gn.g", mod.norm.weight)
                R.vector(name + ".gn.b", mod.norm.bias)
                R.matrix(name + ".pi.w", inner, mod.ch).fwd(mod.proj_in.weight)
                R.vector(name + ".pi.b", mod.proj_in.bias)
                R.matrix(name + ".po.w", mod.ch, inner).fwd(mod.proj_out.weight)
                R.vector(name + ".po.b", mod.proj_out.bias)
                for d, tb in enumerate(mod.transformer_blocks):
                    p = f"{name}.tb{d}"
                    for ln in ("norm1", "norm2", "norm3"):
                        R.vector(f"{p}.{ln}.g", getattr(tb, ln).weight)
                        R.vector(f"{p}.{ln}.b", getattr(tb, ln).bias)
                    if self.variant == "phosc":
                        R.matrix(p + ".a1.qkv.w", 3 * inner, inner)
                        for i, l in enumerate((tb.attn1.to_q, tb.attn1.to_k, tb.attn1.to_v)):
                            R[p + ".a1.qkv.w"].fwd(l.weight, row_off=i * inner)
                        cross = [("a2", tb.attn2)]
                    else:
                        R.matrix(p + ".a1.q.w", inner, inner).fwd(tb.attn1.to_q.weight)
                        cross = [("a1", tb.attn1), ("a2", tb.attn2)]
                    R.matrix(p + ".a2.q.w", inner, inner).fwd(tb.attn2.to_q.weight)
                    for tag, at in cross:
                        kv_w.append(at)
                        self.kv_off[f"{p}.{tag}"] = kvo
                        kvo += 2 * at.to_k.weight.shape[0]
                        R.vector(f"{p}.{tag}.q.f32", at.to_q.weight)
                        R.vector(f"{p}.{tag}.o.f32", at.to_out[0].weight)
                    for tag, at in (("a1", tb.attn1), ("a2", tb.attn2)):
                        R.linear(f"{p}.{tag}.o", at.to_out[0])
                    ffi = tb.ff.net[2].in_features
                    g = geglu_tile(ffi) % 1000 // 2
                    R.matrix(p + ".ff1.w", 2 * ffi, inner).fwd(tb.ff.net[0].proj.weight, g=g)
                    R.vector(p + ".ff1.b", tb.ff.net[0].proj.bias, g=g)
                    R.linear(p + ".ff2", tb.ff.net[2])
                    if N.lib().wd_ff_supported(inner, ffi):
                        R.matrix(p + ".ff1f.w", 2 * ffi, inner).fwd(tb.ff.net[0].proj.weight, g=16)
                        R.vector(p + ".ff1f.b", tb.ff.net[0].proj.bias, g=16)
        self.film_total = off
        self.kv_total = kvo
        ted = m.time_embed[2].out_features
        R.matrix("film.w", off, ted)
        R.vector_cat("film.b", [l.bias for l in film_w])
        r0 = 0
        for l in film_w:
            R["film.w"].fwd(l.weight, row_off=r0)
            r0 += l.weight.shape[0]
        if kv_w:
            R.matrix("kv.w", kvo, kv_w[0].to_k.weight.shape[1])
            r0 = 0
            for at in kv_w:
                for l in (at.to_k, at.to_v):
                    R["kv.w"].fwd(l.weight, row_off=r0)
                    r0 += l.weight.shape[0]
        self._film_mods, self._kv_mods = film_w, kv_w
        R.vector("out.gn.g", m.out[0].weight)
        R.vector("out.gn.b", m.out[0].bias)
        R.matrix("out.w", m.out[2].out_channels, 9 * m.out[2].in_channels).fwd(m.out[2].weight)
        R.vector("out.b", m.out[2].bias)
        R.vector("out.w.f32", m.out[2].weight)
        return R

    def _walk(self):
        m = self.model
        for i, blk in enumerate(m.input_blocks):
            for j, mod in enumerate(blk):
                yield f"in{i}.{j}", mod
        for j, mod in enumerate(m.middle_block):
            yield f"mid.{j}", mod
        for i, blk in enumerate(m.output_blocks):
            for j, mod in enumerate(blk):
                yield f"out{i}.{j}", mod

    def _signature(self):
        if self._ps is None or self._ps_gen != _PARAM_GEN[0]:
            self._ps, self._ps_gen = list(self.model.parameters()), _PARAM_GEN[0]
        ps = self._ps
        return (sum(p._version for p in ps) + (_NATIVE_WRITES[0] << 32), hash(tuple(p.data_ptr() for p in ps)), str(ps[0].device))

    def refresh_weights(self, force: bool = False):
        sig = self._signature()
        if not force and sig == self._sig:
            return
        dev = next(self.model.parameters()).device
        if dev.type != "cuda":
            raise N.NativeError("worddiffusion_amd runs on an MI355X only: move the model to cuda "
                                "(there is no CPU / eager fallback)")
        if self.device is not None and dev != self.device:
            self._w.clear()
            self._w3.clear()
            self._wf.clear()
            self._w3_meta.clear()
            self._plans.clear()
            self._tabs.clear()
            self._tab_np.clear()
            self._ws = None
            self._pack = None
        self.device = dev
        if self._pack is None or self._pack[0] != sig[1:]:
            book = self._recipes()
            for p in self.model.parameters():
                if p.dtype != torch.float32 or not p.is_contiguous():
                    raise N.NativeError("parameters must be contiguous fp32 (the reference never retypes them, unet.py:415)")
            for name, r in book.items():
                if name not in self._w:
                    self._w[name] = (torch.zeros((2, r.rows, r.cols), dtype=torch.bfloat16, device=dev) if r.planes
                                     else torch.zeros(r.shape, dtype=torch.float32, device=dev))
            table, chunks, n = book.device_table(self.lib, self._w, dev, self._wf)
            self._pack = (sig[1:], table, chunks, n, [k for k in self._wf if k not in book or not book.frag_ok(book[k])])
        _, table, chunks, n, wf_left = self._pack
        stream = torch.cuda.current_stream(dev).cuda_stream
        with torch.no_grad():
            for buf, fn in self._derived.values():
                buf.copy_(fn())
        N.check(self.lib.wd_repack_multi(table.data_ptr(), n, chunks, stream), "wd_repack_multi")
        for name in wf_left:
            self._pack_wf(name, self._wf[name], stream)
        with torch.no_grad():
            for name, meta in self._w3_meta.items():
                self._w3[name].copy_(slab_order(self._w[name], *meta))
            if "freqs" not in self._w and hasattr(self.model, "word_emb"):
                half = self.model.model_channels // 2
                freqs = torch.exp(-math.log(10000) * torch.arange(0, half, dtype=torch.float32) / half)
                self._w["freqs"] = freqs.to(dev)
                self._w["pe"] = self.model.word_emb.positional_encoding.to(dev).contiguous()
        self._sig = sig

    def _pack_wf(self, name, wf, stream):
        wp = self._w[name]
        N.check(self.lib.wd_gemm_pack_w(wp[0].data_ptr(), wp[1].data_ptr(), wp.shape[1], wp.shape[2], wf[0].data_ptr(),
                                        wf[1].data_ptr(), stream), "wd_gemm_pack_w")

    def _table(self, h, w, mode):
        key = (h, w, mode)
        if key not in self._tabs:
            tab, ho, wo = conv_gather_table(h, w, mode)
            dt = torch.from_numpy(tab).to(self.device)
            self._tabs[key] = (dt, ho, wo)
            self._tab_np[dt.data_ptr()] = tab
            if mode == "down":
                self._down_w[dt.data_ptr()] = wo
            if mode == "same":
                self._same_w[dt.data_ptr()] = w
        return self._tabs[key]

    def _f32(self, P: Plan, *shape):
        t = torch.empty(shape, dtype=torch.float32, device=self.device)
        P.keep.append(t)
        return t

    def _planes(self, P: Plan, rows, ld):
        t = torch.zeros((2, rows, ld), dtype=torch.bfloat16, device=self.device)
        P.keep.append(t)
        return t

    def _hilo(self, planes: Optional[torch.Tensor], byte_off: int = 0):
        if planes is None:
            return None, None
        return planes[0].data_ptr() + byte_off, (planes[1].data_ptr() + byte_off if self.npass == 3 else None)

    def _src(self, planes: torch.Tensor, c: int, ntaps: int = 1, gather: Optional[torch.Tensor] = None,
             hw_src: int = 0, col_off: int = 0) -> N.WdSrc:
        s = N.WdSrc()
        s._tab_np = self._tab_np.get(gather.data_ptr()) if gather is not None else None
        s._same_w = self._same_w.get(gather.data_ptr(), 0) if gather is not None else 0
        s._down_w = self._down_w.get(gather.data_ptr(), 0) if gather is not None else 0
        ld = planes.shape[2]
        s.hi = planes[0].data_ptr() + 2 * col_off
        s.lo = planes[1].data_ptr() + 2 * col_off
        s.gather = _ptr(gather)
        s.ld, s.c, s.ntaps, s.hw_src = ld, c, ntaps, hw_src
        return s

    def _gemm(self, ops, what, srcs, wname, m, hw_out, bias=None, rowvec=None, rowvec_ld=0, resid=None,
              resid_ld=0, resid_rows=None, act=N.ACT_NONE, out_f32=None, out_ld=0, out_pl=None, n=None, tile=0,
              w_row_off=0, want_stats=False, a32=None, ln=None, w_groups=None):
        a = N.WdGemmArgs()
        for i, s in enumerate(srcs):
            a.src[i] = s
        a.nsrc = len(srcs)
        a.npass = self.npass
        wp = self._w[wname]
        ktot = wp.shape[2]
        assert ktot == sum(s.ntaps * s.c for s in srcs), (what, ktot, [(s.ntaps, s.c) for s in srcs])
        nrows = wp.shape[1] if n is None else n
        a.w_hi = wp[0].data_ptr() + 2 * w_row_off * ktot
        a.w_lo = wp[1].data_ptr() + 2 * w_row_off * ktot
        a.m, a.n, a.ktot, a.hw_out = m, nrows, ktot, hw_out
        a.bias = _ptr(bias)
        a.rowvec, a.rowvec_ld = rowvec, rowvec_ld
        a.resid, a.resid_ld, a.resid_rows = resid, resid_ld, resid_rows
        a.act = act
        a.out_f32, a.out_ld = _ptr(out_f32), out_ld
        if out_pl is not None:
            a.out_hi, a.out_lo, a.out_pl_ld = out_pl[0].data_ptr(), out_pl[1].data_ptr(), out_pl.shape[2]
        if a32 is not None:
            self._set_a32(a, *a32)
        if w_groups is not None:
            a.w_ngroups, a.w_group_stride = w_groups
        a.tile = tile
        if self._ws is None:
            self._ws = torch.empty(128 * 128 * 160 * 8, dtype=torch.float32, device=self.device)
        a.ksplit, a.ws, a.ws_floats = 0, self._ws.data_ptr(), self._ws.numel()
        self._give_tickets(a, m, nrows)
        span = 0
        if self.use_slab and w_row_off == 0 and (len(srcs) == 1 or (srcs[1].ntaps == 1 and not srcs[1].gather)):
            tabnp = getattr(srcs[0], "_tab_np", None)
            span = slab_span(tabnp, hw_out, srcs[0].hw_src, m)
            if span > 192 or ((m + 127) // 128) * max(1, nrows // 160) < 96:
                span = 0
        s0 = srcs[0]
        frag = not span and not self.use_conv3 and w_row_off == 0 and n is None and act == N.ACT_NONE and tile == 0
        width = (getattr(s0, "_down_w", 0) or getattr(s0, "_same_w", 0)) if s0.ntaps == 9 else 0
        wdirect = (frag and self.use_wdirect and wdirect_fills_chip(m, nrows) and
                   self._legal(a, w_layout=3, tile=64320, slab_rows=getattr(s0, "_same_w", 0) if s0.ntaps == 9 else 0))
        smallmap = (frag and not wdirect and self.use_smallmap and hw_out == 64 and 128 <= (m // 64) * (nrows // 80) <= 512 and
                    self._legal(a, w_layout=3, tile=64080, slab_rows=width))
        assert (a32 is None and w_groups is None) or wdirect, what
        if wdirect or smallmap:
            wf = self._wfrag(wname)
            a.w_hi, a.w_lo = wf[0].data_ptr(), wf[1].data_ptr()
        elif span:
            meta = (srcs[0].ntaps, srcs[0].c, srcs[1].c if len(srcs) > 1 else 0)
            if wname not in self._w3:
                self._w3[wname] = slab_order(wp, *meta)
                self._w3_meta[wname] = meta
            assert self._w3_meta[wname] == meta, wname
            w3 = self._w3[wname]
            a.w_hi, a.w_lo = w3[0].data_ptr(), w3[1].data_ptr()
            a.w_layout, a.slab_rows = 1, span
        else:
            same_w = getattr(srcs[0], "_same_w", 0)
            if (same_w and srcs[0].ntaps == 9 and srcs[0].c % 64 == 0 and act == N.ACT_NONE and tile == 0 and
                    (len(srcs) == 1 or (srcs[1].ntaps == 1 and not srcs[1].gather and srcs[1].c % 64 == 0))):
                a.w_layout, a.slab_rows = 2, same_w
        a._ln_pl = None
        if ln is not None and self.fuse_ln and not self.use_slab:
            pl = torch.zeros((2, m, nrows), dtype=torch.bfloat16, device=self.device)
            if self._legal(a, out_hi=pl[0].data_ptr(), out_lo=pl[1].data_ptr(), out_pl_ld=nrows, ln_gamma=self._w[ln + ".g"].data_ptr(),
                           ln_beta=self._w[ln + ".b"].data_ptr(), ln_eps=1e-5):
                self._cur_plan.keep.append(pl)
                a._ln_pl = pl
        stats = None
        if want_stats and self.fuse_stats and nrows % 32 == 0 and (hw_out % 128 == 0 or hw_out == 64) and not span:
            cpg = nrows // 32
            r = self._resolved(a, stat_part=a.ws, stat_cpg=cpg)
            if r is not None:
                nchunk = max(1, hw_out // (r.tile // 1000))
                part = torch.zeros((m // hw_out, nchunk, 32, 2), dtype=torch.float64, device=self.device)
                self._cur_plan.keep.append(part)
                a.stat_part, a.stat_cpg = part.data_ptr(), cpg
                stats = (part, nchunk, cpg)
        a._stats = stats
        self._cur_plan.keep.append(a)
        ops.append((self.lib.wd_gemm, (C.byref(a),), what))
        return a

    def _resolved(self, a, **fields) -> Optional[N.WdGemmArgs]:
        b = N.WdGemmArgs.from_buffer_copy(a)
        for k, v in fields.items():
            setattr(b, k, v)
        out = N.WdGemmArgs()
        return out if self.lib.wd_gemm_check(C.byref(b), C.byref(out)) == N.WD_OK else None

    def _legal(self, a, apply=True, **fields) -> bool:
        if self._resolved(a, **fields) is None:
            return False
# ... 123 lines not shown
        s.hi, s.lo, s.gather = None, None, _ptr(gather)
        s.ld, s.c, s.ntaps, s.hw_src = x.c, x.c, ntaps, hw_src
        return s

    def _gn_in_combine(self, s: Act, raw, gam, bet, eps, silu, cpg, pl, coff) -> bool:
        pr = s.prod
        if pr is None or not isinstance(pr, N.WdGemmArgs) or not self.fuse_gn or raw is not None or self.use_conv3:
            return False
        if pr.out_f32 != s.t.data_ptr() or pr.out_hi or pr.gn_gamma or pr.n != s.c:
            return False
        hi, lo = self._hilo(pl, 2 * coff)
        return self._legal(pr, gn_gamma=gam.data_ptr() + 4 * coff, gn_beta=bet.data_ptr() + 4 * coff, gn_eps=float(eps),
                           gn_silu=int(silu), gn_cpg=cpg, out_hi=hi, out_lo=lo, out_pl_ld=pl.shape[2])

    def _ln(self, P, ops, what, x: torch.Tensor, rows, c, name):
        pl = self._planes(P, rows, c)
        ops.append((self.lib.wd_layernorm,
                    (x.data_ptr(), c, rows, c, self._w[name + ".g"].data_ptr(), self._w[name + ".b"].data_ptr(), 1e-5,
                     *self._hilo(pl), c), what))
        return pl

    def _resblock(self, P, name, mod: ResBlockParams, srcs: List[Act]) -> Act:
        ops = P.step
        B = self._B
        h, w = srcs[0].h, srcs[0].w
        hw, M = h * w, B * h * w
        cin, cout = mod.cin, mod.cout
        assert cin == sum(s.c for s in srcs)
        tab, _, _ = self._table(h, w, "same")
        need_raw = cin != cout
        h1 = self._f32(P, M, cout)
        if self._gn_in_consumer(P, ops, name + ".gn1", srcs, need_raw, M, hw, cout, taps=9, gather=tab):
            s1, in1 = self._src32(srcs[0], 9, tab, hw), (srcs[0], name + ".gn1", 1e-5, True)
            raw = None
        else:
            a1, raw = self._gn(P, ops, name + ".gn1", srcs, name + ".gn1", 1e-5, True, want_raw=need_raw)
            s1, in1 = self._src(a1, cin, 9, tab, hw), None
        g1 = self._gemm(ops, name + ".conv1", [s1], name + ".c1.w", M, hw,
                        bias=self._w[name + ".c1.b"], rowvec=self._film.data_ptr() + 4 * self.film_off[name],
                        rowvec_ld=self.film_total, out_f32=h1, out_ld=cout, want_stats=True, a32=in1)
        h1a = Act(h1, cout, h, w, g1._stats, prod=g1)
        if self._gn_in_consumer(P, ops, name + ".gn2", [h1a], False, M, hw, cout, taps=9, gather=tab):
            s2, in2 = self._src32(h1a, 9, tab, hw), (h1a, name + ".gn2", 1e-5, True)
        else:
            a2, _ = self._gn(P, ops, name + ".gn2", [h1a], name + ".gn2", 1e-5, True)
            s2, in2 = self._src(a2, cout, 9, tab, hw), None
        out = self._f32(P, M, cout)
        if need_raw:
            g2 = self._gemm(ops, name + ".conv2+skip", [s2, self._src(raw, cin)],
                            name + ".c2.w", M, hw, bias=self._w[name + ".c2.b"], out_f32=out, out_ld=cout,
                            want_stats=True, a32=in2)
        else:
            g2 = self._gemm(ops, name + ".conv2", [s2], name + ".c2.w", M, hw,
                            bias=self._w[name + ".c2.b"], resid=srcs[0].t.data_ptr(), resid_ld=cout, out_f32=out,
                            out_ld=cout, want_stats=True, a32=in2)
        return Act(out, cout, h, w, g2._stats, prod=g2)

    def _up_phases_ok(self, mod) -> bool:
        return (getattr(self, "use_up_phases", False) and self.use_wdirect and self.fuse_gn2 and self.npass == 3 and not self.use_slab and
                not self.use_conv3)

    def _resample(self, P, name, mod, x: Act, mode: str, tile: int = 0) -> Act:
        ops = P.step
        B = self._B
        assert x.perm is None, name
        tab, ho, wo = self._table(x.h, x.w, mode)
        pl = self._planes(P, B * x.h * x.w, x.c)
        pr = x.prod
        if (pr is not None and self.fuse_split and not pr.out_hi and pr.out_f32 == x.t.data_ptr() and
                (pr.n if isinstance(pr, N.WdGemmArgs) else pr.c) == x.c):
            pr.out_hi, pr.out_lo = self._hilo(pl)
            pr.out_pl_ld = x.c
        else:
            ops.append((self.lib.wd_split, (x.t.data_ptr(), x.c, B * x.h * x.w, x.c, 0, *self._hilo(pl), x.c), name + ":split"))
        out = self._f32(P, B * ho * wo, mod.cout)
        hw = x.h * x.w
        src4 = None
        if mode == "up" and tile == 0 and (name + ".wph0") in self._w and self._up_phases_ok(mod) and wdirect_fills_chip(B * 4 * hw, mod.cout):
            key = (x.h, x.w, "up4")
            if key not in self._tabs:
                t4, pm = upsample_phase_tables(x.h, x.w)
                dt, dp = torch.from_numpy(t4).to(self.device), torch.from_numpy(pm).to(self.device)
                self._tabs[key] = (dt, dp)
                self._tab_np[dt.data_ptr()] = t4
            tab4, perm = self._tabs[key]
            src4 = self._src(pl, x.c, 4, tab4, hw)
            groups = (4, mod.cout * 4 * x.c)
            if not self._wdirect_ok([src4], B * 4 * hw, mod.cout, 4 * hw, w_ngroups=groups[0], w_group_stride=groups[1]):
                src4 = None
        if src4 is not None:
            if (name + ".wph0") not in self._wf:
                grp = torch.empty((2, 4, mod.cout, 4 * x.c), dtype=torch.bfloat16, device=self.device)
                st = torch.cuda.current_stream(self.device).cuda_stream
                for ph in range(4):
                    self._wf[f"{name}.wph{ph}"] = grp[:, ph]
                    self._pack_wf(f"{name}.wph{ph}", grp[:, ph], st)
                self._pack = None
            gg = self._gemm(ops, name + ".conv (4 phases)", [src4], name + ".wph0", B * 4 * hw, 4 * hw,
                            bias=self._w[name + ".b"], out_f32=out, out_ld=mod.cout, want_stats=True, w_groups=groups)
            return Act(out, mod.cout, ho, wo, gg._stats, prod=None, perm=perm)
        gg = self._gemm(ops, name + ".conv", [self._src(pl, x.c, 9, tab, x.h * x.w)], name + ".w", B * ho * wo, ho * wo,
                        bias=self._w[name + ".b"], out_f32=out, out_ld=mod.cout, want_stats=True, tile=tile)
        return Act(out, mod.cout, ho, wo, gg._stats, prod=gg)

    def _attention(self, ops, what, q, ldq, k, ldk, v, ldv, heads, nq, nk, d, scale, out_pl, out_f32=None,
                   out_rows=None, out_row0=0):
        B = self._B
        ops.append((self.lib.wd_attention,
                    (q, ldq, k, ldk, v, ldv, B, heads, nq, nk, d, float(scale), _ptr(out_f32), *self._hilo(out_pl),
                     out_pl.shape[2] if out_pl is not None else out_f32.shape[-1],
                     nq if out_rows is None else out_rows, out_row0), what))

    def _xattn_fold(self, P, at, heads, d):
        B, L, inner = self._B, self._ctx_len, heads * d
        ko = self.kv_off[at]
        mq = self._f32(P, B, heads * L, inner)
        mo = self._f32(P, B, heads * L, inner)
        mq_pl = torch.zeros((B, 2, 64, inner), dtype=torch.bfloat16, device=self.device)
        mot_pl = torch.zeros((B, 2, inner, 64), dtype=torch.bfloat16, device=self.device)
        P.keep += [mq_pl, mot_pl]
        P.cond.append((self.lib.wd_xattn_fold,
                       (self._kv.data_ptr() + 4 * ko, self.kv_total, self._kv.data_ptr() + 4 * (ko + inner), self.kv_total, B,
                        heads, L, d, float(d ** -0.5), self._w[at + ".q.f32"].data_ptr(), self._w[at + ".o.f32"].data_ptr(), inner,
                        mq.data_ptr(), mo.data_ptr(), mq_pl.data_ptr(), mot_pl.data_ptr()), at + ":fold"))
        return mq, mo, mq_pl, mot_pl

    def _transformer(self, P, name, mod: SpatialTransformerParams, x: Act) -> Act:
        ops = P.step
        B = self._B
        h, w, c = x.h, x.w, x.c
        hw, M = h * w, B * h * w
        heads, d = mod.heads, mod.d_head
        inner = heads * d
        L = self._ctx_len
        if (self.fuse_st and self.variant != "phosc" and len(mod.transformer_blocks) == 1 and inner == c == 320 and
                self.npass == 3 and self.fuse_xattn and self.fuse_xattn_pair and self.fuse_ff and self.fuse_proj and
                bool(self.lib.wd_xattn_supported(inner, heads, L)) and (M + 63) // 64 >= 192 and hw % 64 == 0 and
                (name + ".tb0.ff1f.w") in self._w and
                self._gn_in_consumer(P, ops, name + ".gn", [x], False, M, hw, inner)):
            return self._transformer_fused(P, name, mod, x)
        tok = self._f32(P, M, inner)
        ln1 = f"{name}.tb0.norm1" if self.variant == "phosc" else None
        if self._gn_in_consumer(P, ops, name + ".gn", [x], False, M, hw, inner):
            g_in = self._gemm(ops, name + ".proj_in", [self._src32(x, hw_src=hw)], name + ".pi.w", M, hw, bias=self._w[name + ".pi.b"],
                              out_f32=tok, out_ld=inner, a32=(x, name + ".gn", 1e-6, False), ln=ln1)
        else:
            g, _ = self._gn(P, ops, name + ".gn", [x], name + ".gn", 1e-6, False)
            g_in = self._gemm(ops, name + ".proj_in", [self._src(g, c)], name + ".pi.w", M, hw, bias=self._w[name + ".pi.b"],
                              out_f32=tok, out_ld=inner, ln=ln1)
        n1_pre = g_in._ln_pl
        xpl = None
        fuse = self.fuse_xattn and bool(self.lib.wd_xattn_supported(inner, heads, L))

        def folded(tag, p, x_in, x_out, ln_name, next_ln=None):
            mq, mo, mq_pl, mot_pl = self._xattn_fold(P, f"{p}.{tag}", heads, d)
            npl = self._planes(P, M, inner) if next_ln else None
            ops.append((self.lib.wd_xattn_fused,
                        (x_in.data_ptr(), inner, B, hw, inner, self._w[f"{p}.{ln_name}.g"].data_ptr(),
                         self._w[f"{p}.{ln_name}.b"].data_ptr(), 1e-5, mq.data_ptr(), mo.data_ptr(), heads, L,
                         self._w[f"{p}.{tag}.o.b"].data_ptr(), x_out.data_ptr(), inner,
                         self._w[f"{p}.{next_ln}.g"].data_ptr() if next_ln else None,
                         self._w[f"{p}.{next_ln}.b"].data_ptr() if next_ln else None, 1e-5, *self._hilo(npl), inner,
                         mq_pl.data_ptr(), mot_pl.data_ptr()),
                        f"{p}.{tag}:folded"))
            return npl

        def folded_pair(p, x_in, x_out):
            _, _, qa, oa = self._xattn_fold(P, p + ".a1", heads, d)
            _, _, qb, ob = self._xattn_fold(P, p + ".a2", heads, d)
            npl = self._planes(P, M, inner)
            g2, b2 = self._w[f"{p}.norm2.g"].data_ptr(), self._w[f"{p}.norm2.b"].data_ptr()
            ops.append((self.lib.wd_xattn_pair,
                        (x_in.data_ptr(), inner, B, hw, inner, 1e-5, heads, L, g2, b2, qa.data_ptr(), oa.data_ptr(),
                         self._w[f"{p}.a1.o.b"].data_ptr(), g2, b2, qb.data_ptr(), ob.data_ptr(),
                         self._w[f"{p}.a2.o.b"].data_ptr(), x_out.data_ptr(), inner, self._w[f"{p}.norm3.g"].data_ptr(),
                         self._w[f"{p}.norm3.b"].data_ptr(), 1e-5, *self._hilo(npl), inner), f"{p}.a1+a2:folded"))
            return npl

        for di, tb in enumerate(mod.transformer_blocks):
            p = f"{name}.tb{di}"
            scale = d ** -0.5
            n3 = None
            if fuse and self.variant != "phosc" and self.fuse_xattn_pair:
                tok2 = self._f32(P, M, inner)
                n3 = folded_pair(p, tok, tok2)
            tok1 = self._f32(P, M, inner) if n3 is None else None
            if n3 is not None:
                pass
            elif self.variant == "phosc":
                n1 = n1_pre if (di == 0 and n1_pre is not None) else self._ln(P, ops, p + ".norm1", tok, M, inner, p + ".norm1")
                qkv = self._f32(P, M, 3 * inner)
                self._gemm(ops, p + ".a1.qkv", [self._src(n1, inner)], p + ".a1.qkv.w", M, hw, out_f32=qkv,
                           out_ld=3 * inner)
                o1 = self._planes(P, M, inner)
                self._attention(ops, p + ".a1", qkv.data_ptr(), 3 * inner, qkv.data_ptr() + 4 * inner, 3 * inner,
                                qkv.data_ptr() + 8 * inner, 3 * inner, heads, hw, hw, d, scale, o1)
                n2_pre = self._gemm(ops, p + ".a1.out", [self._src(o1, inner)], p + ".a1.o.w", M, hw, bias=self._w[p + ".a1.o.b"],
                                    resid=tok.data_ptr(), resid_ld=inner, out_f32=tok1, out_ld=inner,
                                    ln=None if fuse else p + ".norm2")._ln_pl
            elif fuse:
                folded("a1", p, tok, tok1, "norm2")
            else:
                n1 = self._ln(P, ops, p + ".norm2a", tok, M, inner, p + ".norm2")
                q1 = self._f32(P, M, inner)
                self._gemm(ops, p + ".a1.q", [self._src(n1, inner)], p + ".a1.q.w", M, hw, out_f32=q1, out_ld=inner)
                ko = self.kv_off[p + ".a1"]
                o1 = self._planes(P, M, inner)
                self._attention(ops, p + ".a1", q1.data_ptr(), inner, self._kv.data_ptr() + 4 * ko, self.kv_total,
                                self._kv.data_ptr() + 4 * (ko + inner), self.kv_total, heads, hw, L, d, scale, o1)
                self._gemm(ops, p + ".a1.out", [self._src(o1, inner)], p + ".a1.o.w", M, hw, bias=self._w[p + ".a1.o.b"],
                           resid=tok.data_ptr(), resid_ld=inner, out_f32=tok1, out_ld=inner)
            if n3 is not None:
                pass
            elif fuse:
                tok2 = self._f32(P, M, inner)
                n3 = folded("a2", p, tok1, tok2, "norm2", next_ln="norm3")
            else:
                tok2 = self._f32(P, M, inner)
                n2 = n2_pre if (self.variant == "phosc" and n2_pre is not None) else \
                    self._ln(P, ops, p + ".norm2", tok1, M, inner, p + ".norm2")
                q2 = self._f32(P, M, inner)
                self._gemm(ops, p + ".a2.q", [self._src(n2, inner)], p + ".a2.q.w", M, hw, out_f32=q2, out_ld=inner)
                ko = self.kv_off[p + ".a2"]
                o2 = self._planes(P, M, inner)
                kp, vp = self._kv.data_ptr() + 4 * ko, self._kv.data_ptr() + 4 * (ko + inner)
                nimg = self.lib.wd_attention_packed_elems(B, heads, L, d) if self.pack_kv else 0
                if nimg > 0:
                    img = torch.empty(nimg, dtype=torch.bfloat16, device=self.device)
                    P.keep.append(img)
                    P.cond.append((self.lib.wd_attention_pack_kv,
                                   (kp, self.kv_total, vp, self.kv_total, B, heads, L, d, img.data_ptr()), p + ".a2:pack kv"))
                    ops.append((self.lib.wd_attention_packed,
                                (q2.data_ptr(), inner, img.data_ptr(), B, heads, hw, L, d, float(scale), None, *self._hilo(o2), inner,
                                 hw, 0), p + ".a2"))
                else:
                    self._attention(ops, p + ".a2", q2.data_ptr(), inner, kp, self.kv_total, vp, self.kv_total, heads, hw, L, d,
                                    scale, o2)
                n3 = self._gemm(ops, p + ".a2.out", [self._src(o2, inner)], p + ".a2.o.w", M, hw, bias=self._w[p + ".a2.o.b"],
                                resid=tok1.data_ptr(), resid_ld=inner, out_f32=tok2, out_ld=inner, ln=p + ".norm3")._ln_pl
            if n3 is None:
                n3 = self._ln(P, ops, p + ".norm3", tok2, M, inner, p + ".norm3")
            last = di == len(mod.transformer_blocks) - 1
            tok = self._f32(P, M, inner)
            xpl = self._planes(P, M, inner) if last else None
            ffi = tb.ff.net[2].in_features
            if self.fuse_ff and (p + ".ff1f.w") in self._w and (M + 63) // 64 >= 192:
                if last and self.fuse_proj and inner == c:
                    out = self._f32(P, M, c)
                    fa = self._ff_fused(ops, p, n3, tok2, M, inner, ffi, out, None,
                                        proj=(name + ".po.w", self._w[name + ".po.b"], x.t, hw))
                    return Act(out, c, h, w, fa._stats, prod=fa)
                self._ff_fused(ops, p, n3, tok2, M, inner, ffi, None if last else tok, xpl)
            else:
                ffh = self._planes(P, M, ffi)
                self._gemm(ops, p + ".ff1", [self._src(n3, inner)], p + ".ff1.w", M, hw, bias=self._w[p + ".ff1.b"],
                           act=N.ACT_GEGLU, out_pl=ffh, tile=geglu_tile(ffi))
                self._gemm(ops, p + ".ff2", [self._src(ffh, ffi)], p + ".ff2.w", M, hw, bias=self._w[p + ".ff2.b"],
                           resid=tok2.data_ptr(), resid_ld=inner, out_f32=None if last else tok, out_ld=inner,
                           out_pl=xpl)
        out = self._f32(P, M, c)
        gg = self._gemm(ops, name + ".proj_out", [self._src(xpl, inner)], name + ".po.w", M, hw,
                        bias=self._w[name + ".po.b"], resid=x.t.data_ptr(), resid_ld=c, out_f32=out, out_ld=c,
                        want_stats=True)
        return Act(out, c, h, w, gg._stats, prod=gg)

    def _transformer_fused(self, P, name, mod: SpatialTransformerParams, x: Act) -> Act:
        M, hw, c = self._B * x.h * x.w, x.h * x.w, x.c
        heads, d, L = mod.heads, mod.d_head, self._ctx_len
        p = name + ".tb0"
        folds = [self._xattn_fold(P, f"{p}.{tag}", heads, d)[2:] for tag in ("a1", "a2")]
        tok2 = self._f32(P, M, c)
        out = self._f32(P, M, c)
        part, nchunk, pc = x.stats
        pw = self._wfrag(name + ".pi.w")
        front = dict(x_in=x.t.data_ptr(), x_in_ld=c, hw=hw, gn_part=part.data_ptr(), gn_nchunk=nchunk, gn_pcpg=pc, gn_cpg=c // 32,
                     gn_eps=1e-6, gn_gamma=self._w[name + ".gn.g"].data_ptr(), gn_beta=self._w[name + ".gn.b"].data_ptr(),
                     pi_hi=pw[0].data_ptr(), pi_lo=pw[1].data_ptr(), pi_b=self._w[name + ".pi.b"].data_ptr(),
                     ln2_gamma=self._w[p + ".norm2.g"].data_ptr(), ln2_beta=self._w[p + ".norm2.b"].data_ptr(),
                     mq_a=folds[0][0].data_ptr(), mot_a=folds[0][1].data_ptr(), xb_a=self._w[p + ".a1.o.b"].data_ptr(),
                     mq_b=folds[1][0].data_ptr(), mot_b=folds[1][1].data_ptr(), xb_b=self._w[p + ".a2.o.b"].data_ptr(),
                     ln3_gamma=self._w[p + ".norm3.g"].data_ptr(), ln3_beta=self._w[p + ".norm3.b"].data_ptr(), ln_eps=1e-5,
                     heads=heads, L=L, tok2=tok2.data_ptr())
        ffi = mod.transformer_blocks[0].ff.net[2].in_features
        fa = self._ff_fused(P.step, p, None, tok2, M, c, ffi, out, None, proj=(name + ".po.w", self._w[name + ".po.b"], x.t, hw),
                            front=front)
        return Act(out, c, x.h, x.w, fa._stats, prod=fa)

    def _wfrag(self, wname):
        if wname not in self._wf:
            self._wf[wname] = torch.empty_like(self._w[wname])
            self._pack_wf(wname, self._wf[wname], torch.cuda.current_stream(self.device).cuda_stream)
            self._pack = None
        return self._wf[wname]

    def _ff_fused(self, ops, p, n3, resid, M, inner, ffi, out_f32, out_pl, proj=None, front=None):
        a = N.WdFfArgs()
        if front is None:
            (a.x_hi, a.x_lo), a.x_ld = self._hilo(n3), n3.shape[2]
        else:
            for k, v in front.items():
                setattr(a, k, v)
        a.m, a.c, a.inner = M, inner, ffi
        w1, w2 = self._wfrag(p + ".ff1f.w"), self._wfrag(p + ".ff2.w")
        a.w1_hi, a.w1_lo, a.b1 = w1[0].data_ptr(), w1[1].data_ptr(), self._w[p + ".ff1f.b"].data_ptr()
        a.w2_hi, a.w2_lo, a.b2 = w2[0].data_ptr(), w2[1].data_ptr(), self._w[p + ".ff2.b"].data_ptr()
        a.resid, a.resid_ld = resid.data_ptr(), inner
        if out_f32 is not None:
            a.out_f32, a.out_ld = out_f32.data_ptr(), inner
        if out_pl is not None:
            (a.out_hi, a.out_lo), a.out_pl_ld = self._hilo(out_pl), out_pl.shape[2]
        a.hw_out, a.npass = 1, self.npass
        stats = None
        if proj is not None:
            wname, b3, x_in, hw = proj
            w3 = self._wfrag(wname)
            a.w3_hi, a.w3_lo, a.b3 = w3[0].data_ptr(), w3[1].data_ptr(), b3.data_ptr()
            a.resid3, a.resid3_ld = x_in.data_ptr(), inner
            if self.fuse_stats and inner % 32 == 0 and hw % 64 == 0:
                nchunk = hw // 64
                part = torch.zeros((M // hw, nchunk, 32, 2), dtype=torch.float64, device=self.device)
                self._cur_plan.keep.append(part)
                a.stat_part, a.stat_cpg, a.hw_out = part.data_ptr(), inner // 32, hw
                stats = (part, nchunk, inner // 32)
        self._cur_plan.keep.append(a)
        what = ".ff (fused)" if proj is None else ".ff + proj_out (fused)" if front is None else ": gn + proj_in + a1 + a2 + ff + proj_out (fused)"
        ops.append((self.lib.wd_ff_fused, (C.byref(a),), p + what))
        a._stats = stats
        return a

    @staticmethod
    def _cached_plan(plans: Dict[tuple, Plan], key, room: int = 0) -> Optional[Plan]:
        if key in plans:
            plans[key] = plans.pop(key)
            return plans[key]
        while room and len(plans) >= room:
            plans.pop(next(iter(plans)))
        return None

    def _begin_plan(self, P: Plan, B: int) -> Plan:
        self._cur_plan = P
        self._B = B
        return P

    def _inputs(self, P: Plan, H, W, ctx_len, phosc_len):
        m, B, dev = self.model, self._B, self.device
        P.x_in = torch.zeros((B, m.in_channels, H, W), dtype=torch.float32, device=dev)
        P.t_in = torch.zeros((B,), dtype=torch.int64, device=dev)
        P.y_in = torch.zeros((B,), dtype=torch.int64, device=dev)
        P.ctx_in = torch.zeros((B, max(ctx_len, 1)), dtype=torch.int64, device=dev)
        P.phosc_in = torch.zeros((B, max(phosc_len, 1)), dtype=torch.int32, device=dev)

    def _conditioning(self, P: Plan, ops, ctx_len, phosc_len) -> List[tuple]:
        m, lib, B = self.model, self.lib, self._B
        cd = m.context_dim
        msl = m.max_seq_len
        L = self._ctx_len = ctx_len + phosc_len
        P.ctx_pl = self._planes(P, B * L, cd)
        groups = []
        for (ids, n_tok, row0, i64) in ((P.ctx_in, ctx_len, 0, 1), (P.phosc_in, phosc_len, ctx_len, 0)):
            if n_tok == 0:
                continue
            use_pe = (self.variant == "base") or (n_tok <= msl)
            if use_pe and n_tok > msl:
                raise ValueError(f"context length {n_tok} exceeds max_seq_len {msl} (the reference fails too)")
            e = self._planes(P, B * n_tok, cd)
            ops.append((lib.wd_embed_tokens,
                        (ids.data_ptr(), i64, B * n_tok, n_tok, self._w["we.table"].data_ptr(), self._w["we.table"].shape[0], cd,
                         self._w["pe"].data_ptr() if use_pe else None, *self._hilo(e), cd), "word_emb.embedding"))
            qkv = self._f32(P, B * n_tok, 3 * cd)
            self._gemm(ops, "word_emb.qkv", [self._src(e, cd)], "we.qkv.w", B * n_tok, n_tok, bias=self._w["we.qkv.b"],
                       out_f32=qkv, out_ld=3 * cd)
            self._attention(ops, "word_emb.attention", qkv.data_ptr(), 3 * cd, qkv.data_ptr() + 4 * cd, 3 * cd,
                            qkv.data_ptr() + 8 * cd, 3 * cd, 1, n_tok, n_tok, cd, 1.0, P.ctx_pl, out_rows=L, out_row0=row0)
            groups.append((ids, n_tok, row0, i64, e, qkv))
        if self.kv_total:
            self._kv = self._f32(P, B * L, self.kv_total)
            self._gemm(ops, "cross.kv", [self._src(P.ctx_pl, cd)], "kv.w", B * L, L, out_f32=self._kv, out_ld=self.kv_total)
        return groups

    def _head_gemm(self, P: Plan, ops, what, x: torch.Tensor, w: str, label="im2col", want_stats=True, tile=0):
        B, cin, H, W = x.shape
        xin = self._planes(P, B * H * W, self.kpad_in)
        ops.append((self.lib.wd_im2col3x3, (x.data_ptr(), B, cin, H, W, *self._hilo(xin), self.kpad_in), label))
        cout = self._w[w + ".w"].shape[1]
        h0 = self._f32(P, B * H * W, cout)
        g0 = self._gemm(ops, what, [self._src(xin, self.kpad_in)], w + ".w", B * H * W, H * W, bias=self._w[w + ".b"], out_f32=h0,
                        out_ld=cout, want_stats=want_stats, tile=tile)
        return Act(h0, cout, H, W, g0._stats), xin

    def _trunk(self, P: Plan, cur: Act) -> Act:
        m = self.model
        hs = [cur]

        def run_layers(prefix, blk, cur, extra=None):
            for j, mod in enumerate(blk):
                name = f"{prefix}.{j}"
                if isinstance(mod, ResBlockParams):
                    cur = self._resblock(P, name, mod, [cur] + ([extra] if (extra is not None and j == 0) else []))
                elif isinstance(mod, SpatialTransformerParams):
                    cur = self._transformer(P, name, mod, cur)
                elif isinstance(mod, DownsampleParams):
                    cur = self._resample(P, name, mod, cur, "down")
                elif isinstance(mod, UpsampleParams):
                    cur = self._resample(P, name, mod, cur, "up")
                else:
                    raise TypeError(type(mod))
            return cur

        for i, blk in enumerate(m.input_blocks):
            if i == 0:
                continue
            cur = run_layers(f"in{i}", blk, cur)
            hs.append(cur)
        cur = run_layers("mid", m.middle_block, cur)
        for i, blk in enumerate(m.output_blocks):
            cur = run_layers(f"out{i}", blk, cur, extra=hs.pop())
        return cur

    def _tail_gemm(self, P: Plan, ops, what, x: Act, eps, nchw: Optional[torch.Tensor] = None):
        B, hw = self._B, x.h * x.w
        g, _ = self._gn(P, ops, "out.gn", [x], "out.gn", eps, True)
        tab, _, _ = self._table(x.h, x.w, "same")
        oc = self._w["out.w"].shape[1]
        otok = self._f32(P, B * hw, oc)
        self._gemm(ops, what, [self._src(g, x.c, 9, tab, hw)], "out.w", B * hw, hw, bias=self._w["out.b"], out_f32=otok, out_ld=oc)
        if nchw is not None:
            ops.append((self.lib.wd_tokens_to_nchw, (otok.data_ptr(), oc, B, oc, hw, nchw.data_ptr()), "tokens_to_nchw"))
        return g, otok

    def plan(self, B: int, H: int, W: int, ctx_len: int, phosc_len: int, film_steps: int = 0, mix: int = 0,
             film_timesteps: Optional[tuple] = None) -> Plan:
        key = (B, H, W, ctx_len, phosc_len, self.npass, film_steps) + ((("mix", mix),) if mix else ())
        if film_timesteps is not None:
            film_timesteps = tuple(int(t) for t in film_timesteps)
            if not film_steps or not film_timesteps or min(film_timesteps) < 0 or max(film_timesteps) >= film_steps:
                raise ValueError("film_timesteps needs film_steps = T and timesteps in [0, T)")
            key += (("tau", film_timesteps),)
        P = self._cached_plan(self._plans, key, room=max(1, PLAN_CACHE_SIZE))
        if P is not None:
            return P
        m = self.model
        lib = self.lib
        if ctx_len + phosc_len == 0:
            raise NotImplementedError("context=None: every reference script conditions on the word (unet.py:1605)")
        P = self._begin_plan(Plan(), B)
        dev = self.device
        mc = m.model_channels
        ted = 4 * mc
        self._inputs(P, H, W, ctx_len, phosc_len)
        self._conditioning(P, P.cond, ctx_len, phosc_len)

        step = P.step
        has_lab = m.num_classes is not None
        if mix and not has_lab:
            raise ValueError("writer-style interpolation needs a class-conditional model (num_classes)")
        if mix not in (0, 1, 2) or (mix == 2 and not film_steps):
            raise ValueError(f"mix = {mix}: 1 or 2 forwards per step with the table, 1 without")
        P.mix = mix
        if mix:
            P.mix_m = torch.zeros((B,), dtype=torch.float32, device=dev)
        self._film = self._f32(P, B, self.film_total)
        P.t_dev = torch.zeros((1,), dtype=torch.int32, device=dev)
        P.k_dev = torch.zeros((1,), dtype=torch.int32, device=dev)
        P.film = []
        if film_steps:
            T = film_steps if film_timesteps is None else len(film_timesteps)
            nf = max(1, mix)
            chunk = min(T, max(8 if film_timesteps is None else 1, FILM_CHUNK_ROWS // (B * nf)))
            nchunks = (T + chunk - 1) // chunk
            Tp = nchunks * chunk
# ... 177 lines not shown
```

### worddiffusion_amd/train_engine.py

```python
from __future__ import annotations

import ctypes as C
from typing import Dict, List, Optional

import os

import torch

from . import _native as N
from . import dropout as DO
from .backward import conv_bwd_table
from .engine import Act, Plan, UNetEngine, _ptr
from .layers import DownsampleParams, ResBlockParams, SpatialTransformerParams, UpsampleParams


class TAct(Act):
    __slots__ = ("g", "gw")

    def __init__(self, t, c, h, w, stats=None):
        super().__init__(t, c, h, w, stats)
        self.g, self.gw = None, False


class TrainPlan(Plan):
    def __init__(self):
        super().__init__()
        self.bwd: List[tuple] = []
        self.dout: Optional[torch.Tensor] = None
        self.dropouts: List[DO.WdDropout] = []
        self.row_base: Optional[torch.Tensor] = None

    def set_dropout_seed(self, seed: int):
        for d in self.dropouts:
            d.seed = int(seed) & 0xFFFFFFFFFFFFFFFF

    def set_row_base(self, row_base: int):
        if self.dropouts:
            v = int(row_base) & 0xFFFFFFFFFFFFFFFF
            self.row_base.fill_(v - (1 << 64) if v >= (1 << 63) else v)

    def run_bwd(self, stream, begin: int = 0, end: Optional[int] = None):
        self._run(self.bwd[begin:end], stream)


def _rup(x: int, m: int) -> int:
    return (x + m - 1) // m * m


class TrainEngine(UNetEngine):
    def __init__(self, model, variant: str):
        super().__init__(model, variant)
        self.use_wdirect = os.environ.get("WDIFF_TRAIN_WDIRECT", "0") != "0"
        self.use_smallmap = os.environ.get("WDIFF_TRAIN_SMALLMAP", "1") != "0"
        self.fuse_ff = self.fuse_proj = False
        self.use_up_phases = False
        self.fuse_gn_in = 0
        self.use_dw = os.environ.get("WDIFF_TRAIN_DW", "1") != "0"
        self.fuse_geglu_bwd = os.environ.get("WDIFF_FUSE_GEGLU_BWD", "1") != "0"
        self.fuse_gn_bwd = os.environ.get("WDIFF_FUSE_GN_BWD", "1") != "0"
        self.dw_group_max = int(os.environ.get("WDIFF_DW_GROUP", "8"))
        self._dw_pending: Dict[tuple, list] = {}
        self._tplans: Dict[tuple, TrainPlan] = {}
        self._grad: Dict[int, torch.Tensor] = {}
        self._params: Dict[int, torch.nn.Parameter] = {}
        self._btabs: Dict[tuple, torch.Tensor] = {}
        self._scr: Dict[str, torch.Tensor] = {}
        self._arena = None
        self._arena_used = 0
        self.defer_bias_sums = os.environ.get("WDIFF_DEFER_BIAS", "1") != "0"
        self._deferred, self._deferred_outs = [], {}
        self.nbuckets = int(os.environ.get("WDIFF_GRAD_BUCKETS", "3"))
        self._carve_order: List[tuple] = []
        self._done_at: Dict[int, int] = {}
        self._closure = 0
        self._cut_closures: Optional[List[int]] = None
        self.dropout_seed = 0
        self.dropout_row_base = 0
        self._layer_of: Optional[Dict[int, int]] = None

    def set_precision(self, mode: str):
        old = self.npass
        super().set_precision(mode)
        if self.npass != old and self._tplans:
            self._tplans.clear()
            self._scr = {k: v for k, v in self._scr.items() if isinstance(k, tuple)}

    def _recipes(self):
        R = super()._recipes()
        m = self.model
        we = m.word_emb
        cd = we.embedding.weight.shape[1]
        R.matrix("B:we.qkv.w", cd, 3 * cd)
        for i, l in enumerate((we.attention.linear_query, we.attention.linear_key, we.attention.linear_value)):
            R["B:we.qkv.w"].bwd(l.weight, col_off=i * cd)
        for name, mod in self._walk():
            if isinstance(mod, ResBlockParams):
                R.matrix("B:" + name + ".c1.w", mod.cin, 9 * mod.cout).bwd(mod.in_layers[2].weight)
                R.matrix("B:" + name + ".c2.w", mod.cout, 9 * mod.cout).bwd(mod.out_layers[3].weight)
                if mod.cin != mod.cout:
                    R.matrix("B:" + name + ".skip.w", mod.cin, mod.cout).bwd(mod.skip_connection.weight)
            elif isinstance(mod, (DownsampleParams, UpsampleParams)):
                conv = mod.op if isinstance(mod, DownsampleParams) else mod.conv
                R.matrix("B:" + name + ".w", mod.cin, 9 * mod.cout).bwd(conv.weight)
            elif isinstance(mod, SpatialTransformerParams):
                inner = mod.heads * mod.d_head
                R.matrix("B:" + name + ".pi.w", mod.ch, inner).bwd(mod.proj_in.weight)
                R.matrix("B:" + name + ".po.w", inner, mod.ch).bwd(mod.proj_out.weight)
                for d, tb in enumerate(mod.transformer_blocks):
                    p = f"{name}.tb{d}"
                    for tag, at in (("a1", tb.attn1), ("a2", tb.attn2)):
                        if tag == "a1" and self.variant == "phosc":
                            R.matrix(f"B:{p}.a1.qkv.w", inner, 3 * inner)
                            for i, l in enumerate((at.to_q, at.to_k, at.to_v)):
                                R[f"B:{p}.a1.qkv.w"].bwd(l.weight, col_off=i * inner)
                        else:
                            R.matrix(f"B:{p}.{tag}.q.w", inner, inner).bwd(at.to_q.weight)
                        R.matrix(f"B:{p}.{tag}.o.w", inner, inner).bwd(at.to_out[0].weight)
                    ffi = tb.ff.net[2].in_features
                    R.linear(p + ".ff1u", tb.ff.net[0].proj)
                    R.matrix("B:" + p + ".ff1.w", inner, 2 * ffi).bwd(tb.ff.net[0].proj.weight)
                    R.matrix("B:" + p + ".ff2.w", ffi, inner).bwd(tb.ff.net[2].weight)
        ted = m.time_embed[2].out_features
        R.matrix("B:film.w", ted, self.film_total)
        c0 = 0
        for l in self._film_mods:
            R["B:film.w"].bwd(l.weight, col_off=c0)
            c0 += l.weight.shape[0]
        R.matrix("B:kv.w", cd, self.kv_total)
        c0 = 0
        for at in self._kv_mods:
            for l in (at.to_k, at.to_v):
                R["B:kv.w"].bwd(l.weight, col_off=c0)
                c0 += l.weight.shape[0]
        R.matrix("B:te2.w", ted, ted).bwd(m.time_embed[2].weight)
        R.matrix("B:out.w", m.out[2].in_channels, 9 * 32).bwd(m.out[2].weight, npad=32)
        return R

    def _carve(self, shape) -> torch.Tensor:
        if self._arena is None:
            total = sum(_rup(p.numel(), 64) for p in self.model.parameters())
            self._arena = torch.zeros(total, dtype=torch.float32, device=self.device)
            self._arena_used = 0
        n = 1
        for d in shape:
            n *= int(d)
        out = self._arena[self._arena_used:self._arena_used + n].view(shape)
        self._carve_order.append((out.data_ptr(), self._arena_used, _rup(n, 64)))
        self._arena_used += _rup(n, 64)
        assert self._arena_used <= self._arena.numel()
        return out

    def _pgrad(self, p: torch.nn.Parameter) -> torch.Tensor:
        if id(p) not in self._grad:
            self._grad[id(p)] = self._carve(tuple(p.shape))
            self._params[id(p)] = p
        return self._grad[id(p)]

    def _pgroup(self, params: List[torch.nn.Parameter]) -> torch.Tensor:
        key = ("group",) + tuple(id(p) for p in params)
        if key not in self._scr:
            tail = tuple(params[0].shape[1:])
            rows = sum(p.shape[0] for p in params)
            buf = self._carve((rows,) + tail)
            r0 = 0
            for p in params:
                self._grad[id(p)] = buf[r0:r0 + p.shape[0]]
                self._params[id(p)] = p
                r0 += p.shape[0]
            self._scr[key] = buf
        return self._scr[key]

    def _ppair(self, p0: torch.nn.Parameter, p1: torch.nn.Parameter) -> torch.Tensor:
        key = ("pair", id(p0), id(p1))
        if key not in self._scr:
            buf = self._carve((2,) + tuple(p0.shape))
            for i, p in enumerate((p0, p1)):
                self._grad[id(p)] = buf[i]
                self._params[id(p)] = p
            self._scr[key] = buf
        return self._scr[key]

    def grad_arena(self) -> torch.Tensor:
        return self._arena[: self._arena_used]

    def _bias_finish(self, ops, what, colpart, nblk, n, b):
        self._param_colsum(ops, what, colpart.data_ptr(), n, nblk, n, b.data_ptr(), self._pacc(b), key=b.data_ptr())

    def _param_colsum(self, ops, what, src_ptr, ld, rows, c, out_ptr, acc, key=None):
        key = out_ptr if key is None else key
        rnd = self._deferred_outs.get(key, 0)
        if not self.defer_bias_sums or rows > 1024 or (acc and rnd == 0):
            self._colsum(ops, what, src_ptr, ld, rows, c, rows, out_ptr, c, acc)
            return
        self._deferred_outs[key] = rnd + 1
        while len(self._deferred) <= rnd:
            self._deferred.append([])
        self._deferred[rnd].append((src_ptr, out_ptr, rows, c, ld, 1 if (rnd or acc) else 0, 1.0, 0))

    def _flush_deferred(self, P):
        import struct
        for rnd, entries in enumerate(self._deferred):
            if not entries:
                continue
            rec = self.lib.wd_colsum_entry_bytes()
            assert rec == 40, rec
            blob = b"".join(struct.pack("<QQiiiifi", *e) for e in entries)
            table = torch.frombuffer(bytearray(blob), dtype=torch.uint8).to(self.device)
# ... 802 lines not shown
```

Baseline: 35.62 images/s.

## Fold ff2 weights into proj_out to collapse the transformer tail into one GEMM

Precomputes W32 = W_proj_out · W_ff2 and a combined bias on device, so the feed-forward second linear and proj_out become a single GEMM over [ffh, tok2] planes. The fused FF kernel gains a FOLD variant that first multiplies the residual tokens by W_proj_out in-register, then accumulates the folded ff2 product. The xattn kernel gains a variant that also emits split-bf16 planes of the residual. This removes one chained GEMM and the intermediate fp32 token round-trip at the cost of more kernel complexity, extra LDS and different rounding.

```diff
diff --git a/include/wdiff_hip.h b/include/wdiff_hip.h
--- a/include/wdiff_hip.h
+++ b/include/wdiff_hip.h
@@ -141,6 +141,9 @@
     float ln_eps;
     int32_t heads, L;
     float* tok2;
+    const wd_bf16* w32_hi;
+    const wd_bf16* w32_lo;
+    const float* b32;
 } wd_ff_args;
 int wd_ff_fused(const wd_ff_args* args, void* stream);
 int wd_ff_supported(int c, int inner);
@@ -212,6 +215,15 @@
                   const float* beta_a, const wd_bf16* mq_pl_a, const wd_bf16* mot_pl_a, const float* bias_a, const float* gamma_b,
                   const float* beta_b, const wd_bf16* mq_pl_b, const wd_bf16* mot_pl_b, const float* bias_b, float* out, int out_ld,
                   const float* gamma2, const float* beta2, float eps2, wd_bf16* n_hi, wd_bf16* n_lo, int n_ld, void* stream);
+
+int wd_xattn_planes(const float* x, int ld, int batch, int hw, int c, float eps, int heads, int L, const float* gamma_a,
+                    const float* beta_a, const wd_bf16* mq_pl_a, const wd_bf16* mot_pl_a, const float* bias_a, const float* gamma_b,
+                    const float* beta_b, const wd_bf16* mq_pl_b, const wd_bf16* mot_pl_b, const float* bias_b, float* out, int out_ld,
+                    const float* gamma2, const float* beta2, float eps2, wd_bf16* n_hi, wd_bf16* n_lo, int n_ld, wd_bf16* r_hi,
+                    wd_bf16* r_lo, int r_ld, void* stream);
+
+int wd_linear_fold(const float* w3, const float* w2, const float* b2, const float* b3, int c, int inner, int ffi, float* w32,
+                   float* b32, void* stream);
 
 int wd_embed_tokens(const void* ids, int ids_are_i64, int rows, int seq_len, const float* table, int vocab, int c,
                     const float* pe, wd_bf16* out_hi, wd_bf16* out_lo, int out_ld, void* stream);
diff --git a/worddiffusion_amd/_native.py b/worddiffusion_amd/_native.py
--- a/worddiffusion_amd/_native.py
+++ b/worddiffusion_amd/_native.py
@@ -51,7 +51,8 @@
                 ("gn_pcpg", C.c_int32), ("gn_cpg", C.c_int32), ("gn_eps", C.c_float), ("gn_gamma", _vp), ("gn_beta", _vp),
                 ("pi_hi", _vp), ("pi_lo", _vp), ("pi_b", _vp), ("ln2_gamma", _vp), ("ln2_beta", _vp), ("mq_a", _vp), ("mot_a", _vp),
                 ("xb_a", _vp), ("mq_b", _vp), ("mot_b", _vp), ("xb_b", _vp), ("ln3_gamma", _vp), ("ln3_beta", _vp),
-                ("ln_eps", C.c_float), ("heads", C.c_int32), ("L", C.c_int32), ("tok2", _vp)]
+                ("ln_eps", C.c_float), ("heads", C.c_int32), ("L", C.c_int32), ("tok2", _vp),
+                ("w32_hi", _vp), ("w32_lo", _vp), ("b32", _vp)]
 
 
 class WdDwArgs(C.Structure):
@@ -146,6 +147,9 @@
     "wd_next_timestep": (_i, [_vp, _vp, _i, _vp, _vp, _i, _vp]),
     "wd_xattn_pair": (_i, [_vp, _i, _i, _i, _i, _f, _i, _i, _vp, _vp, _vp, _vp, _vp, _vp, _vp, _vp, _vp, _vp, _vp, _i, _vp, _vp, _f,
                            _vp, _vp, _i, _vp]),
+    "wd_xattn_planes": (_i, [_vp, _i, _i, _i, _i, _f, _i, _i, _vp, _vp, _vp, _vp, _vp, _vp, _vp, _vp, _vp, _vp, _vp, _i, _vp, _vp, _f,
+                             _vp, _vp, _i, _vp, _vp, _i, _vp]),
+    "wd_linear_fold": (_i, [_vp, _vp, _vp, _vp, _i, _i, _i, _vp, _vp, _vp]),
     "wd_add": (_i, [_vp, _vp, C.c_int64, _vp]),
     "wd_permute_dw": (_i, [_vp, _i, _i, _i, _i, _vp, _vp]),
     "wd_colsum": (_i, [_vp, _i, _i, _i, _i, _vp, _i, _i, _f, _vp, C.c_int64, _vp]),
diff --git a/worddiffusion_amd/csrc/wd_ff.hip b/worddiffusion_amd/csrc/wd_ff.hip
--- a/worddiffusion_amd/csrc/wd_ff.hip
+++ b/worddiffusion_amd/csrc/wd_ff.hip
@@ -15,10 +15,11 @@
 
 __device__ __forceinline__ int f_lds_off(int row, int ch) { return row * 128 + ((ch ^ ((row >> 1) & 7)) << 4); }
 
-template <int NPASS, bool PROJ, bool FRONT>
+template <int NPASS, bool PROJ, bool FRONT, bool FOLD>
 __global__ void __launch_bounds__(FNT, 1) wd_ff_kernel(const wd_ff_args a) {
 #if defined(__HIP_DEVICE_COMPILE__)
     static_assert(!FRONT || (NPASS == 3 && PROJ), "the transformer front needs split-bf16 operands and the proj_out tail");
+    static_assert(!FOLD || (NPASS == 3 && PROJ), "the folded tail is the proj_out tail in split-bf16");
     constexpr int NPL = (NPASS == 1) ? 1 : 2;
     constexpr int SLAB = 2 * FBM * 128;
     constexpr int A_BYTES = 5 * SLAB;
@@ -40,7 +41,8 @@
         return __builtin_amdgcn_make_buffer_rsrc(const_cast<wd_bf16*>(p), 0, 0x7FFFFFF0, 0x00020000);
     };
     const __amdgpu_buffer_rsrc_t srd1_hi = make_srd(a.w1_hi), srd1_lo = make_srd(a.w1_lo ? a.w1_lo : a.w1_hi);
-    const __amdgpu_buffer_rsrc_t srd2_hi = make_srd(a.w2_hi), srd2_lo = make_srd(a.w2_lo ? a.w2_lo : a.w2_hi);
+    const __amdgpu_buffer_rsrc_t srd2_hi = make_srd(FOLD ? a.w32_hi : a.w2_hi),
+                                 srd2_lo = make_srd(FOLD ? a.w32_lo : a.w2_lo ? a.w2_lo : a.w2_hi);
     const __amdgpu_buffer_rsrc_t srd3_hi = make_srd(PROJ ? a.w3_hi : a.w2_hi), srd3_lo = make_srd(PROJ ? (a.w3_lo ? a.w3_lo : a.w3_hi) : a.w2_hi);
     const uint32_t lane16 = lane * 16;
     const int nct1 = (2 * a.inner) >> 4;
@@ -49,7 +51,7 @@
     auto issue = [&](const int slot, const int g, const int j) {
         const bool live = j < nchunk;
         const uint32_t vo = live ? lane16 : F_OOB;
-        if (PROJ && g < FRING) {
+        if (PROJ && !FOLD && g < FRING) {
             const uint32_t so3 = (uint32_t)(((2 * (g / 5) + kh) * (FC / 16) + 5 * cg + g % 5) * 1024);
             const uint32_t so1 = (uint32_t)(((g >> 1) * nct1 + 2 * (j * 8 + wave) + (g & 1)) * 1024);
             const uint32_t so = live ? so1 : so3;
@@ -108,6 +110,38 @@
                         }
             }
             __syncthreads();
+        }
+    };
+
+    auto issue_w3 = [&](const int slot, const int g) {
+        const uint32_t so = (uint32_t)(((2 * (g / 5) + kh) * (FC / 16) + 5 * cg + g % 5) * 1024);
+#pragma unroll
+        for (int p = 0; p < NPL; ++p)
+            ring[slot][p] = __builtin_bit_cast(bf16x8, __builtin_amdgcn_raw_buffer_load_b128(p ? srd3_lo : srd3_hi, lane16, so, 0));
+    };
+    auto fold_product = [&](const int q0, const int q1, const char* slabs) {
+        if (q0 == 0) {
+#pragma unroll
+            for (int i = 0; i < 4; ++i)
+#pragma unroll
+                for (int t = 0; t < 5; ++t)
+#pragma unroll
+                    for (int r = 0; r < 4; ++r) acc2[i][t][r] = 0.0f;
+        }
+#pragma unroll
+        for (int g = 0; g < 25; ++g) {
+            const int q = g / 5, t = g % 5;
+            if (q < q0 || q >= q1) continue;
+            if (t == 0) read_frags(slabs + (q - q0) * SLAB, kh);
+            {
+                f32x4 col[4] = {acc2[0][t], acc2[1][t], acc2[2][t], acc2[3][t]};
+                mfma12(col, ring[(g + 5) % FRING]);
+#pragma unroll
+                for (int i = 0; i < 4; ++i) acc2[i][t] = col[i];
+            }
+            if (g + FRING < 25) issue_w3((g + 5) % FRING, g + FRING);
+            else issue((g + 5) % FRING, g + FRING - 25, 0);
+            __builtin_amdgcn_sched_barrier(0);
         }
     };
 
@@ -119,7 +153,7 @@
         float* s_aff = reinterpret_cast<float*>(fr);
         float* sS = reinterpret_cast<float*>(fr);
         wd_bf16* sP = reinterpret_cast<wd_bf16*>(fr + FBM * SP * 4);
-        float* s_vec = reinterpret_cast<float*>(s_h + 40960);
+        float* s_vec = reinterpret_cast<float*>(s_h + (FOLD ? 49152 : 40960));
         const float* s_pib = s_vec;
         const float* s_ln2g = s_vec + FC, * s_ln2b = s_vec + 2 * FC, * s_ln3g = s_vec + 3 * FC, * s_ln3b = s_vec + 4 * FC;
         const float* s_xba = s_vec + 5 * FC, * s_xbb = s_vec + 6 * FC;
@@ -413,7 +447,10 @@
                 issue_mq(a.mq_b);
             } else {
 #pragma unroll
-                for (int g = 0; g < FRING; ++g) issue(g, g, 0);
+                for (int g = 0; g < FRING; ++g) {
+                    if (FOLD) issue_w3((g + 5) % FRING, g);
+                    else issue(g, g, 0);
+                }
                 __builtin_amdgcn_sched_barrier(0);
             }
             __syncthreads();
@@ -429,15 +466,81 @@
                 }
             __syncthreads();
         }
-#pragma unroll
-        for (int pp = 0; pp < 2; ++pp)
-#pragma unroll
-            for (int i = 0; i < 5; ++i)
-                *reinterpret_cast<float4*>(a.tok2 + (long)(m0 + wave * 8 + pp * 4 + lq) * FC + (l15 + 16 * i) * 4) = xr[pp][i];
+        if constexpr (!FOLD) {
+#pragma unroll
+            for (int pp = 0; pp < 2; ++pp)
+#pragma unroll
+                for (int i = 0; i < 5; ++i)
+                    *reinterpret_cast<float4*>(a.tok2 + (long)(m0 + wave * 8 + pp * 4 + lq) * FC + (l15 + 16 * i) * 4) = xr[pp][i];
+        } else {
+            const __amdgpu_buffer_rsrc_t st2 = __builtin_amdgcn_make_buffer_rsrc(a.tok2, 0, a.tok2 ? 0x7FFFFFF0 : 0, 0x00020000);
+            float4* park = reinterpret_cast<float4*>(s_a);
+            auto planes = [&](const int pp, const int i, const int i0) {
+                const int n = (l15 + 16 * i) * 4, row = wave * 8 + pp * 4 + lq;
+                uint2 hi, lo;
+                wd_split4(xr[pp][i], hi, lo);
+                char* d = s_h + (i - i0) * SLAB + f_lds_off(row, (n & 63) >> 3) + (n & 7) * 2;
+                *reinterpret_cast<uint2*>(d) = hi;
+                *reinterpret_cast<uint2*>(d + FBM * 128) = lo;
+            };
+#pragma unroll
+            for (int pp = 0; pp < 2; ++pp)
+#pragma unroll
+                for (int i = 0; i < 5; ++i) {
+                    const int n = (l15 + 16 * i) * 4, row = wave * 8 + pp * 4 + lq;
+                    __builtin_amdgcn_raw_buffer_store_b128(__builtin_bit_cast(f_u32x4, xr[pp][i]), st2, (uint32_t)(((m0 + row) * FC + n) * 4), 0, 0);
+                    park[(pp * 5 + i) * FNT + tid] = xr[pp][i];
+                    if (i < 3) planes(pp, i, 0);
+                }
+            __syncthreads();
+            fold_product(0, 3, s_h);
+            __syncthreads();
+#pragma unroll
+            for (int pp = 0; pp < 2; ++pp)
+#pragma unroll
+                for (int i = 3; i < 5; ++i) {
+                    xr[pp][i] = park[(pp * 5 + i) * FNT + tid];
+                    planes(pp, i, 3);
+                }
+            __syncthreads();
+            fold_product(3, 5, s_h);
+#pragma unroll
+            for (int pp = 0; pp < 2; ++pp)
+#pragma unroll
+                for (int i = 0; i < 5; ++i) xr[pp][i] = park[(pp * 5 + i) * FNT + tid];
+            __syncthreads();
+        }
         ln_rows(s_ln3g, s_ln3b);
     } else {
 #pragma unroll
-    for (int g = 0; g < FRING; ++g) issue(g, g, 0);
+    for (int g = 0; g < FRING; ++g) {
+        if (FOLD) issue_w3((g + 5) % FRING, g);
+        else issue(g, g, 0);
+    }
+    if constexpr (FOLD) {
+        const int arow = tid >> 3, ach = tid & 7;
+        const bool rok = m0 + arow < a.m;
+        const float* xrow = a.resid + (long)(rok ? m0 + arow : 0) * a.resid_ld + ach * 8;
+        float4 xv[5][2];
+#pragma unroll
+        for (int sl = 0; sl < 5; ++sl) {
+            xv[sl][0] = *reinterpret_cast<const float4*>(xrow + sl * 64);
+            xv[sl][1] = *reinterpret_cast<const float4*>(xrow + sl * 64 + 4);
+        }
+#pragma unroll
+        for (int sl = 0; sl < 5; ++sl) {
+            const float4 z = make_float4(0.f, 0.f, 0.f, 0.f);
+            uint2 h0, l0, h1, l1;
+            wd_split4(rok ? xv[sl][0] : z, h0, l0);
+            wd_split4(rok ? xv[sl][1] : z, h1, l1);
+            char* dst = s_a + sl * SLAB + f_lds_off(arow, ach);
+            *reinterpret_cast<f_u32x4*>(dst) = f_u32x4{h0.x, h0.y, h1.x, h1.y};
+            *reinterpret_cast<f_u32x4*>(dst + FBM * 128) = f_u32x4{l0.x, l0.y, l1.x, l1.y};
+        }
+        __syncthreads();
+        fold_product(0, 5, s_a);
+        __syncthreads();
+    }
 
     {
         const __amdgpu_buffer_rsrc_t sx_hi = make_srd(a.x_hi), sx_lo = make_srd(a.x_lo ? a.x_lo : a.x_hi);
@@ -458,12 +561,14 @@
     }
     __syncthreads();
 
-#pragma unroll
-    for (int i = 0; i < 4; ++i)
-#pragma unroll
-        for (int t = 0; t < 5; ++t)
-#pragma unroll
-            for (int r = 0; r < 4; ++r) acc2[i][t][r] = 0.0f;
+    if constexpr (!FOLD) {
+#pragma unroll
+        for (int i = 0; i < 4; ++i)
+#pragma unroll
+            for (int t = 0; t < 5; ++t)
+#pragma unroll
+                for (int r = 0; r < 4; ++r) acc2[i][t][r] = 0.0f;
+    }
 
     for (int j = 0; j < nchunk; ++j) {
         char* hbuf = s_h + (j & 1) * H_BYTES;
@@ -537,6 +642,11 @@
         e.resid = a.resid;
         e.resid_ld = a.resid_ld;
         wd_epilogue_from_image<FBM, FC, FNT>(e, ep, m0, 0, tid);
+    } else if constexpr (FOLD) {
+        e.bias = a.b32;
+        e.resid = a.resid3;
+        e.resid_ld = a.resid3_ld;
+        wd_epilogue_from_image<FBM, FC, FNT>(e, ep, m0, 0, tid);
     } else {
         constexpr int ROWB = LDE * 4;
         const float* resid = FRONT ? a.tok2 : a.resid;
@@ -615,7 +725,7 @@
 #endif
 }
 
-template <int NPASS, bool PROJ, bool FRONT = false>
+template <int NPASS, bool PROJ, bool FRONT = false, bool FOLD = false>
 int launch_ff(const wd_ff_args& a, hipStream_t st) {
     constexpr int max_smem = 5 * 2 * FBM * 128 + 2 * 2 * 2 * FBM * 128 + 2 * F_MAX_INNER * 4;
     constexpr int red_smem = FBM * (FC + 4) * 4 + WD_STAT_SCRATCH;
@@ -624,7 +734,7 @@
     const int smem = loop_smem > red_smem ? loop_smem : red_smem;
     static bool attr_done = false;
     if (!attr_done) {
-        if (hipFuncSetAttribute(reinterpret_cast<const void*>(&wd_ff_kernel<NPASS, PROJ, FRONT>), hipFuncAttributeMaxDynamicSharedMemorySize,
+        if (hipFuncSetAttribute(reinterpret_cast<const void*>(&wd_ff_kernel<NPASS, PROJ, FRONT, FOLD>), hipFuncAttributeMaxDynamicSharedMemorySize,
                                 max_smem) != hipSuccess)
             return WD_ELAUNCH;
         attr_done = true;
@@ -633,7 +743,7 @@
     const double fl = 2.0 * (double)a.m * (3.0 * (double)a.inner * FC + (PROJ ? (double)FC * FC : 0.0) +
                                            (FRONT ? (double)FC * FC + 4.0 * a.heads * a.L * FC : 0.0));
     WdLaunchScope scope(WD_CLS_FF, st, fl);
-    hipLaunchKernelGGL((wd_ff_kernel<NPASS, PROJ, FRONT>), dim3(nb), dim3(FNT), smem, st, a);
+    hipLaunchKernelGGL((wd_ff_kernel<NPASS, PROJ, FRONT, FOLD>), dim3(nb), dim3(FNT), smem, st, a);
     return wd_check_launch();
 }
 
@@ -655,6 +765,9 @@
     if (a.resid && a.resid_ld <= 0) return WD_EINVAL;
     if ((long)a.m * a.x_ld * 2 >= 0x7FFFFFF0L || (long)2 * a.inner * a.c * 2 >= 0x7FFFFFF0L) return WD_EINVAL;
     const bool proj = a.w3_hi != nullptr;
+    const bool fold = a.w32_hi != nullptr;
+    if (fold && (!proj || a.npass != 3 || !a.w32_lo || !a.b32 || (!front && !a.resid) || (long)a.m * FC * 4 >= 0x7FFFFFF0L))
+        return WD_EINVAL;
     if (proj && ((a.npass == 3 && !a.w3_lo) || (a.resid3 && (a.resid3_ld <= 0 || (a.resid3_ld & 3))))) return WD_EINVAL;
     if (a.stat_part && (a.stat_cpg <= 0 || FC % a.stat_cpg || a.hw_out <= 0 || !(a.hw_out % FBM == 0 || FBM % a.hw_out == 0) ||
                         (FBM > a.hw_out && FBM / a.hw_out > WD_STAT_MAXNS)))
@@ -664,10 +777,11 @@
         if (!a.gn_part || a.gn_nchunk <= 0 || a.gn_pcpg <= 0 || a.gn_cpg <= 0 || a.gn_cpg % a.gn_pcpg || FC % a.gn_cpg ||
             !a.gn_gamma || !a.gn_beta)
             return WD_EINVAL;
-        if (!a.pi_hi || !a.pi_lo || !a.pi_b || !a.ln2_gamma || !a.ln2_beta || !a.ln3_gamma || !a.ln3_beta || !a.tok2) return WD_EINVAL;
+        if (!a.pi_hi || !a.pi_lo || !a.pi_b || !a.ln2_gamma || !a.ln2_beta || !a.ln3_gamma || !a.ln3_beta || (!a.tok2 && !fold)) return WD_EINVAL;
         if (!a.mq_a || !a.mot_a || !a.xb_a || !a.mq_b || !a.mot_b || !a.xb_b || !wd_xattn_supported(a.c, a.heads, a.L)) return WD_EINVAL;
     }
     hipStream_t st = reinterpret_cast<hipStream_t>(stream);
+    if (fold) return front ? launch_ff<3, true, true, true>(a, st) : launch_ff<3, true, false, true>(a, st);
     if (front) return launch_ff<3, true, true>(a, st);
     if (proj) return a.npass == 3 ? launch_ff<3, true>(a, st) : launch_ff<1, true>(a, st);
     return a.npass == 3 ? launch_ff<3, false>(a, st) : launch_ff<1, false>(a, st);
diff --git a/worddiffusion_amd/csrc/wd_pack.hip b/worddiffusion_amd/csrc/wd_pack.hip
--- a/worddiffusion_amd/csrc/wd_pack.hip
+++ b/worddiffusion_amd/csrc/wd_pack.hip
@@ -142,6 +142,36 @@
     }
 }
 
+__global__ void __launch_bounds__(256) linear_fold_kernel(const float* __restrict__ w3, const float* __restrict__ w2,
+                                                          const float* __restrict__ b2, const float* __restrict__ b3, int c, int inner,
+                                                          int ffi, float* __restrict__ w32, float* __restrict__ b32) {
+    const int j = blockIdx.x * 256 + threadIdx.x, n = blockIdx.y;
+    if (n == c) {
+        if (j >= c) return;
+        double acc = 0.0;
+        if (b2)
+            for (int k = 0; k < inner; ++k) acc += (double)w3[(int64_t)j * inner + k] * (double)b2[k];
+        if (b3) acc += (double)b3[j];
+        b32[j] = (float)acc;
+        return;
+    }
+    if (j >= ffi) return;
+    const float* row = w3 + (int64_t)n * inner;
+    double acc = 0.0;
+    for (int k = 0; k < inner; ++k) acc += (double)row[k] * (double)w2[(int64_t)k * ffi + j];
+    w32[(int64_t)n * ffi + j] = (float)acc;
+}
+
+}
+
+extern "C" int wd_linear_fold(const float* w3, const float* w2, const float* b2, const float* b3, int c, int inner, int ffi,
+                              float* w32, float* b32, void* stream) {
+    if (!w3 || !w2 || !w32 || !b32 || c <= 0 || inner <= 0 || ffi <= 0 || c > 65534) return WD_EINVAL;
+    hipStream_t st = reinterpret_cast<hipStream_t>(stream);
+    WdLaunchScope scope(WD_CLS_OTHER, st);
+    const int nx = ((ffi > c ? ffi : c) + 255) / 256;
+    hipLaunchKernelGGL(linear_fold_kernel, dim3(nx, c + 1), dim3(256), 0, st, w3, w2, b2, b3, c, inner, ffi, w32, b32);
+    return wd_check_launch();
 }
 
 extern "C" int wd_repack_entry_bytes(void) { return (int)sizeof(PackRef); }
diff --git a/worddiffusion_amd/csrc/wd_xattn.hip b/worddiffusion_amd/csrc/wd_xattn.hip
--- a/worddiffusion_amd/csrc/wd_xattn.hip
+++ b/worddiffusion_amd/csrc/wd_xattn.hip
@@ -269,7 +269,8 @@
                                                       const XaLayer lb, float eps, int heads, int L, float* __restrict__ out,
                                                       int out_ld, const float* __restrict__ gamma2,
                                                       const float* __restrict__ beta2, float eps2, wd_bf16* __restrict__ n_hi,
-                                                      wd_bf16* __restrict__ n_lo, int n_ld) {
+                                                      wd_bf16* __restrict__ n_lo, int n_ld, wd_bf16* __restrict__ r_hi,
+                                                      wd_bf16* __restrict__ r_lo, int r_ld) {
     constexpr int XT = 16, NTH = 256;
     constexpr int C = NI * 32, XP = C + 8, OP = C + 4, SP = 65, PP = 72, NT = NI / 2, KS32 = C / 32;
     static_assert(NI % 2 == 0, "column tiles per wave");
@@ -455,6 +456,16 @@
             if (ok && last) *reinterpret_cast<float4*>(out + (row0 + trow) * out_ld + n) = xr[i];
             s += (xr[i].x + xr[i].y) + (xr[i].z + xr[i].w);
         }
+        if (r_hi && last && ok) {
+#pragma unroll
+            for (int i = 0; i < FI; ++i) {
+                const int n = (l15 + 16 * i) * 4;
+                uint2 hi, lo;
+                wd_split4(xr[i], hi, lo);
+                *reinterpret_cast<uint2*>(r_hi + (row0 + trow) * r_ld + n) = hi;
+                if (r_lo) *reinterpret_cast<uint2*>(r_lo + (row0 + trow) * r_ld + n) = lo;
+            }
+        }
         if (n_hi && last) {
             const float mean = wd_row16_sum(s) / (float)C;
             float q = 0.f;
@@ -488,7 +499,7 @@
 template <int NI, int NP>
 int launch16(const float* x, int ld, int batch, int hw, const XaLayer& la, const XaLayer& lb, float eps, int heads, int L,
              float* out, int out_ld, const float* gamma2, const float* beta2, float eps2, wd_bf16* n_hi, wd_bf16* n_lo, int n_ld,
-             hipStream_t st) {
+             hipStream_t st, wd_bf16* r_hi = nullptr, wd_bf16* r_lo = nullptr, int r_ld = 0) {
     constexpr int C = NI * 32, XTM = 16;
     constexpr size_t xb = (size_t)2 * XTM * (C + 8) * 2 > (size_t)XTM * (C + 4) * 4 ? (size_t)2 * XTM * (C + 8) * 2 : (size_t)XTM * (C + 4) * 4;
     constexpr size_t smem = xb + (size_t)XTM * 65 * 4 + (size_t)2 * XTM * 72 * 2 + (size_t)6 * C * 4;
@@ -497,10 +508,10 @@
     const dim3 grid(batch, (hw + XTM - 1) / XTM);
     if (L == 10)
         hipLaunchKernelGGL((xattn16_kernel<NI, NP, 10>), grid, dim3(256), smem, st, x, ld, hw, la, lb, eps, heads, L, out, out_ld,
-                           gamma2, beta2, eps2, n_hi, n_lo, n_ld);
+                           gamma2, beta2, eps2, n_hi, n_lo, n_ld, r_hi, r_lo, r_ld);
     else
         hipLaunchKernelGGL((xattn16_kernel<NI, NP, 0>), grid, dim3(256), smem, st, x, ld, hw, la, lb, eps, heads, L, out, out_ld,
-                           gamma2, beta2, eps2, n_hi, n_lo, n_ld);
+                           gamma2, beta2, eps2, n_hi, n_lo, n_ld, r_hi, r_lo, r_ld);
     return wd_check_launch();
 }
 
@@ -560,18 +571,37 @@
     return WD_EINVAL;
 }
 
+extern "C" int wd_xattn_planes(const float* x, int ld, int batch, int hw, int c, float eps, int heads, int L, const float* gamma_a,
+                               const float* beta_a, const wd_bf16* mq_pl_a, const wd_bf16* mot_pl_a, const float* bias_a,
+                               const float* gamma_b, const float* beta_b, const wd_bf16* mq_pl_b, const wd_bf16* mot_pl_b,
+                               const float* bias_b, float* out, int out_ld, const float* gamma2, const float* beta2, float eps2,
+                               wd_bf16* n_hi, wd_bf16* n_lo, int n_ld, wd_bf16* r_hi, wd_bf16* r_lo, int r_ld, void* stream) {
+    if (!x || !out || !gamma_a || !beta_a || !mq_pl_a || !mot_pl_a || !bias_a || batch <= 0 || hw <= 0) return WD_EINVAL;
+    const bool pair = mq_pl_b != nullptr;
+    if (pair && (!gamma_b || !beta_b || !mot_pl_b || !bias_b)) return WD_EINVAL;
+    if (!wd_xattn_supported(c, heads, L) || ld % 4 || out_ld % 4 || (n_hi && (n_ld % 4 || !gamma2 || !beta2)) ||
+        (r_hi && r_ld % 4) || (r_lo && !r_hi))
+        return WD_EINVAL;
+    hipStream_t st = reinterpret_cast<hipStream_t>(stream);
+    const XaLayer la = {gamma_a, beta_a, mq_pl_a, mot_pl_a, bias_a};
+    const XaLayer lb = pair ? XaLayer{gamma_b, beta_b, mq_pl_b, mot_pl_b, bias_b} : la;
+#define WD_XP(NI_, NP_) \
+    return launch16<NI_, NP_>(x, ld, batch, hw, la, lb, eps, heads, L, out, out_ld, gamma2, beta2, eps2, n_hi, n_lo, n_ld, st, r_hi, r_lo, r_ld)
+    if (c == 320) {
+        if (pair) WD_XP(10, 2);
+        WD_XP(10, 1);
+    }
+    if (pair) WD_XP(2, 2);
+    WD_XP(2, 1);
+#undef WD_XP
+}
+
 extern "C" int wd_xattn_pair(const float* x, int ld, int batch, int hw, int c, float eps, int heads, int L, const float* gamma_a,
                              const float* beta_a, const wd_bf16* mq_pl_a, const wd_bf16* mot_pl_a, const float* bias_a,
                              const float* gamma_b, const float* beta_b, const wd_bf16* mq_pl_b, const wd_bf16* mot_pl_b,
                              const float* bias_b, float* out, int out_ld, const float* gamma2, const float* beta2, float eps2,
                              wd_bf16* n_hi, wd_bf16* n_lo, int n_ld, void* stream) {
-    if (!x || !out || !gamma_a || !beta_a || !mq_pl_a || !mot_pl_a || !bias_a || !gamma_b || !beta_b || !mq_pl_b || !mot_pl_b ||
-        !bias_b || batch <= 0 || hw <= 0)
-        return WD_EINVAL;
-    if (!wd_xattn_supported(c, heads, L) || ld % 4 || out_ld % 4 || (n_hi && (n_ld % 4 || !gamma2 || !beta2))) return WD_EINVAL;
-    hipStream_t st = reinterpret_cast<hipStream_t>(stream);
-    const XaLayer la = {gamma_a, beta_a, mq_pl_a, mot_pl_a, bias_a}, lb = {gamma_b, beta_b, mq_pl_b, mot_pl_b, bias_b};
-    if (c == 320)
-        return launch16<10, 2>(x, ld, batch, hw, la, lb, eps, heads, L, out, out_ld, gamma2, beta2, eps2, n_hi, n_lo, n_ld, st);
-    return launch16<2, 2>(x, ld, batch, hw, la, lb, eps, heads, L, out, out_ld, gamma2, beta2, eps2, n_hi, n_lo, n_ld, st);
-}
+    if (!mq_pl_b) return WD_EINVAL;
+    return wd_xattn_planes(x, ld, batch, hw, c, eps, heads, L, gamma_a, beta_a, mq_pl_a, mot_pl_a, bias_a, gamma_b, beta_b, mq_pl_b,
+                           mot_pl_b, bias_b, out, out_ld, gamma2, beta2, eps2, n_hi, n_lo, n_ld, nullptr, nullptr, 0, stream);
+}
diff --git a/worddiffusion_amd/engine.py b/worddiffusion_amd/engine.py
--- a/worddiffusion_amd/engine.py
+++ b/worddiffusion_amd/engine.py
@@ -290,6 +290,8 @@
 
 class UNetEngine:
 
+    fold_proj = False
+
     def __init__(self, model, variant: str):
         self.model = model
         self.variant = variant
@@ -319,6 +321,7 @@
                                 "(python -m worddiffusion_amd.build --force)")
         self.fuse_xattn_pair = os.environ.get("WDIFF_FUSE_XATTN_PAIR", "1") != "0"
         self.fuse_st = os.environ.get("WDIFF_FUSE_ST", "1") != "0"
+        self.fold_proj = os.environ.get("WDIFF_FOLD_PROJ", "1") != "0"
         self.fuse_out = os.environ.get("WDIFF_FUSE_OUT", "1") != "0"
         self.fuse_in = os.environ.get("WDIFF_FUSE_IN", "1") != "0"
         self.pack_kv = os.environ.get("WDIFF_PACK_KV", "1") != "0"
@@ -435,6 +438,27 @@
                     if N.lib().wd_ff_supported(inner, ffi):
                         R.matrix(p + ".ff1f.w", 2 * ffi, inner).fwd(tb.ff.net[0].proj.weight, g=16)
                         R.vector(p + ".ff1f.b", tb.ff.net[0].proj.bias, g=16)
+                if self.fold_proj:
+                    tb = mod.transformer_blocks[-1]
+                    lin, po = tb.ff.net[2], mod.proj_out
+                    ffi, dev = lin.in_features, po.weight.device
+                    key = name + ".w32"
+                    if key not in self._derived or self._derived[key][0].device != dev:
+                        w32 = torch.empty((mod.ch, ffi), dtype=torch.float32, device=dev)
+                        b32 = torch.empty((mod.ch,), dtype=torch.float32, device=dev)
+
+                        def fold(lin=lin, po=po, w32=w32, b32=b32, rows=mod.ch, k=inner, cols=ffi):
+                            st = torch.cuda.current_stream(w32.device).cuda_stream
+                            N.check(self.lib.wd_linear_fold(po.weight.data_ptr(), lin.weight.data_ptr(), _ptr(lin.bias), _ptr(po.bias),
+                                                            rows, k, cols, w32.data_ptr(), b32.data_ptr(), st), "wd_linear_fold")
+
+                        self._derived[key] = (w32, fold)
+                        self._derived[name + ".b32"] = (b32, None)
+                    w32, b32 = self._derived[key][0], self._derived[name + ".b32"][0]
+                    R.matrix(name + ".po32.w", mod.ch, ffi + inner).fwd(w32).fwd(po.weight, col_off=ffi)
+                    R.vector(name + ".b32", b32)
+                    if inner == mod.ch and N.lib().wd_ff_supported(inner, ffi):
+                        R.matrix(name + ".w32.w", mod.ch, ffi).fwd(w32)
         self.film_total = off
         self.kv_total = kvo
         ted = m.time_embed[2].out_features
@@ -510,7 +534,9 @@
         stream = torch.cuda.current_stream(dev).cuda_stream
         with torch.no_grad():
             for buf, fn in self._derived.values():
-                buf.copy_(fn())
+                r = fn() if fn is not None else None
+                if r is not None:
+                    buf.copy_(r)
         N.check(self.lib.wd_repack_multi(table.data_ptr(), n, chunks, stream), "wd_repack_multi")
         for name in wf_left:
             self._pack_wf(name, self._wf[name], stream)
@@ -940,9 +966,18 @@
         xpl = None
         fuse = self.fuse_xattn and bool(self.lib.wd_xattn_supported(inner, heads, L))
 
-        def folded(tag, p, x_in, x_out, ln_name, next_ln=None):
+        def folded(tag, p, x_in, x_out, ln_name, next_ln=None, raw=None):
             mq, mo, mq_pl, mot_pl = self._xattn_fold(P, f"{p}.{tag}", heads, d)
             npl = self._planes(P, M, inner) if next_ln else None
+            if raw is not None:
+                ops.append((self.lib.wd_xattn_planes,
+                            (x_in.data_ptr(), inner, B, hw, inner, 1e-5, heads, L, self._w[f"{p}.{ln_name}.g"].data_ptr(),
+                             self._w[f"{p}.{ln_name}.b"].data_ptr(), mq_pl.data_ptr(), mot_pl.data_ptr(),
+                             self._w[f"{p}.{tag}.o.b"].data_ptr(), None, None, None, None, None, x_out.data_ptr(), inner,
+                             self._w[f"{p}.{next_ln}.g"].data_ptr() if next_ln else None,
+                             self._w[f"{p}.{next_ln}.b"].data_ptr() if next_ln else None, 1e-5, *self._hilo(npl), inner,
+                             *self._hilo(raw), inner), f"{p}.{tag}:folded + planes"))
+                return npl
             ops.append((self.lib.wd_xattn_fused,
                         (x_in.data_ptr(), inner, B, hw, inner, self._w[f"{p}.{ln_name}.g"].data_ptr(),
                          self._w[f"{p}.{ln_name}.b"].data_ptr(), 1e-5, mq.data_ptr(), mo.data_ptr(), heads, L,
@@ -953,25 +988,35 @@
                         f"{p}.{tag}:folded"))
             return npl
 
-        def folded_pair(p, x_in, x_out):
+        def folded_pair(p, x_in, x_out, raw=None):
             _, _, qa, oa = self._xattn_fold(P, p + ".a1", heads, d)
             _, _, qb, ob = self._xattn_fold(P, p + ".a2", heads, d)
             npl = self._planes(P, M, inner)
             g2, b2 = self._w[f"{p}.norm2.g"].data_ptr(), self._w[f"{p}.norm2.b"].data_ptr()
-            ops.append((self.lib.wd_xattn_pair,
-                        (x_in.data_ptr(), inner, B, hw, inner, 1e-5, heads, L, g2, b2, qa.data_ptr(), oa.data_ptr(),
-                         self._w[f"{p}.a1.o.b"].data_ptr(), g2, b2, qb.data_ptr(), ob.data_ptr(),
-                         self._w[f"{p}.a2.o.b"].data_ptr(), x_out.data_ptr(), inner, self._w[f"{p}.norm3.g"].data_ptr(),
-                         self._w[f"{p}.norm3.b"].data_ptr(), 1e-5, *self._hilo(npl), inner), f"{p}.a1+a2:folded"))
+            args = (x_in.data_ptr(), inner, B, hw, inner, 1e-5, heads, L, g2, b2, qa.data_ptr(), oa.data_ptr(),
+                    self._w[f"{p}.a1.o.b"].data_ptr(), g2, b2, qb.data_ptr(), ob.data_ptr(),
+                    self._w[f"{p}.a2.o.b"].data_ptr(), x_out.data_ptr(), inner, self._w[f"{p}.norm3.g"].data_ptr(),
+                    self._w[f"{p}.norm3.b"].data_ptr(), 1e-5, *self._hilo(npl), inner)
+            if raw is not None:
+                ops.append((self.lib.wd_xattn_planes, args + (*self._hilo(raw), inner), f"{p}.a1+a2:folded + planes"))
+            else:
+                ops.append((self.lib.wd_xattn_pair, args, f"{p}.a1+a2:folded"))
             return npl
 
         for di, tb in enumerate(mod.transformer_blocks):
             p = f"{name}.tb{di}"
             scale = d ** -0.5
             n3 = None
+            last = di == len(mod.transformer_blocks) - 1
+            ffi = tb.ff.net[2].in_features
+            ff_fused = self.fuse_ff and (p + ".ff1f.w") in self._w and (M + 63) // 64 >= 192
+            tok2pl = None
+            if (last and not ff_fused and self.fold_proj and self.npass == 3 and fuse and (name + ".po32.w") in self._w and
+                    not os.environ.get("WDIFF_XATTN_VALU")):
+                tok2pl = self._planes(P, M, inner)
             if fuse and self.variant != "phosc" and self.fuse_xattn_pair:
                 tok2 = self._f32(P, M, inner)
-                n3 = folded_pair(p, tok, tok2)
+                n3 = folded_pair(p, tok, tok2, raw=tok2pl)
             tok1 = self._f32(P, M, inner) if n3 is None else None
             if n3 is not None:
                 pass
@@ -1002,7 +1047,7 @@
                 pass
             elif fuse:
                 tok2 = self._f32(P, M, inner)
-                n3 = folded("a2", p, tok1, tok2, "norm2", next_ln="norm3")
+                n3 = folded("a2", p, tok1, tok2, "norm2", next_ln="norm3", raw=tok2pl)
             else:
                 tok2 = self._f32(P, M, inner)
                 n2 = n2_pre if (self.variant == "phosc" and n2_pre is not None) else \
@@ -1028,11 +1073,17 @@
                                 resid=tok1.data_ptr(), resid_ld=inner, out_f32=tok2, out_ld=inner, ln=p + ".norm3")._ln_pl
             if n3 is None:
                 n3 = self._ln(P, ops, p + ".norm3", tok2, M, inner, p + ".norm3")
-            last = di == len(mod.transformer_blocks) - 1
+            if tok2pl is not None:
+                ffh = self._planes(P, M, ffi)
+                self._gemm(ops, p + ".ff1", [self._src(n3, inner)], p + ".ff1.w", M, hw, bias=self._w[p + ".ff1.b"],
+                           act=N.ACT_GEGLU, out_pl=ffh, tile=geglu_tile(ffi))
+                out = self._f32(P, M, c)
+                gg = self._gemm(ops, name + ".ff2 + proj_out", [self._src(ffh, ffi), self._src(tok2pl, inner)], name + ".po32.w", M, hw,
+                                bias=self._w[name + ".b32"], resid=x.t.data_ptr(), resid_ld=c, out_f32=out, out_ld=c, want_stats=True)
+                return Act(out, c, h, w, gg._stats, prod=gg)
             tok = self._f32(P, M, inner)
             xpl = self._planes(P, M, inner) if last else None
-            ffi = tb.ff.net[2].in_features
-            if self.fuse_ff and (p + ".ff1f.w") in self._w and (M + 63) // 64 >= 192:
+            if ff_fused:
                 if last and self.fuse_proj and inner == c:
                     out = self._f32(P, M, c)
                     fa = self._ff_fused(ops, p, n3, tok2, M, inner, ffi, out, None,
@@ -1057,7 +1108,7 @@
         heads, d, L = mod.heads, mod.d_head, self._ctx_len
         p = name + ".tb0"
         folds = [self._xattn_fold(P, f"{p}.{tag}", heads, d)[2:] for tag in ("a1", "a2")]
-        tok2 = self._f32(P, M, c)
+        tok2 = None if self._fold_fused(name) else self._f32(P, M, c)
         out = self._f32(P, M, c)
         part, nchunk, pc = x.stats
         pw = self._wfrag(name + ".pi.w")
@@ -1068,11 +1119,14 @@
                      mq_a=folds[0][0].data_ptr(), mot_a=folds[0][1].data_ptr(), xb_a=self._w[p + ".a1.o.b"].data_ptr(),
                      mq_b=folds[1][0].data_ptr(), mot_b=folds[1][1].data_ptr(), xb_b=self._w[p + ".a2.o.b"].data_ptr(),
                      ln3_gamma=self._w[p + ".norm3.g"].data_ptr(), ln3_beta=self._w[p + ".norm3.b"].data_ptr(), ln_eps=1e-5,
-                     heads=heads, L=L, tok2=tok2.data_ptr())
+                     heads=heads, L=L, tok2=_ptr(tok2))
         ffi = mod.transformer_blocks[0].ff.net[2].in_features
         fa = self._ff_fused(P.step, p, None, tok2, M, c, ffi, out, None, proj=(name + ".po.w", self._w[name + ".po.b"], x.t, hw),
                             front=front)
         return Act(out, c, x.h, x.w, fa._stats, prod=fa)
+
+    def _fold_fused(self, name) -> bool:
+        return self.fold_proj and self.npass == 3 and (name + ".w32.w") in self._w
 
     def _wfrag(self, wname):
         if wname not in self._wf:
@@ -1092,7 +1146,7 @@
         w1, w2 = self._wfrag(p + ".ff1f.w"), self._wfrag(p + ".ff2.w")
         a.w1_hi, a.w1_lo, a.b1 = w1[0].data_ptr(), w1[1].data_ptr(), self._w[p + ".ff1f.b"].data_ptr()
         a.w2_hi, a.w2_lo, a.b2 = w2[0].data_ptr(), w2[1].data_ptr(), self._w[p + ".ff2.b"].data_ptr()
-        a.resid, a.resid_ld = resid.data_ptr(), inner
+        a.resid, a.resid_ld = _ptr(resid), inner
         if out_f32 is not None:
             a.out_f32, a.out_ld = out_f32.data_ptr(), inner
         if out_pl is not None:
@@ -1104,6 +1158,9 @@
             w3 = self._wfrag(wname)
             a.w3_hi, a.w3_lo, a.b3 = w3[0].data_ptr(), w3[1].data_ptr(), b3.data_ptr()
             a.resid3, a.resid3_ld = x_in.data_ptr(), inner
+            if self._fold_fused(wname[:-len(".po.w")]):
+                w32 = self._wfrag(wname[:-len(".po.w")] + ".w32.w")
+                a.w32_hi, a.w32_lo, a.b32 = w32[0].data_ptr(), w32[1].data_ptr(), self._w[wname[:-len(".po.w")] + ".b32"].data_ptr()
             if self.fuse_stats and inner % 32 == 0 and hw % 64 == 0:
                 nchunk = hw // 64
                 part = torch.zeros((M // hw, nchunk, 32, 2), dtype=torch.float64, device=self.device)
diff --git a/worddiffusion_amd/train_engine.py b/worddiffusion_amd/train_engine.py
--- a/worddiffusion_amd/train_engine.py
+++ b/worddiffusion_amd/train_engine.py
@@ -53,6 +53,7 @@
         self.use_wdirect = os.environ.get("WDIFF_TRAIN_WDIRECT", "0") != "0"
         self.use_smallmap = os.environ.get("WDIFF_TRAIN_SMALLMAP", "1") != "0"
         self.fuse_ff = self.fuse_proj = False
+        self.fold_proj = False
         self.use_up_phases = False
         self.fuse_gn_in = 0
         self.use_dw = os.environ.get("WDIFF_TRAIN_DW", "1") != "0"
```

Measured after the change: 36.32 images/s, median of 6. 2.0% higher.
